# githubhjs/h264-jm-commentary

Measured on AMD Instinct MI355X. Metric: ME+transform megapixels/sec @1080p FullSearch SR=32; bit-exact vs the in-repo JM restatement (oracle); device-resident (inputs in HBM, no H2D/D2H in the timed region), higher is better.
Workload: dtype u8

## Files before the change

h264-jm-commentary_amd/csrc/jmh_analyse.hip:

```cpp
#include "jmh_common.h"
#include "jmh_launch.h"
#include "jmh_intra8.h"
#include "jmh_intra.h"
#include "jmh_i4.h"
#ifdef JMH_FLOW_TU
#include "jmh_final.h"
#endif

#define MVB_OFF 544
#define MVB_LEN 1104
#define PLS (WIN_DIM_MAX * WST + 32)
#define MAXNS 7

struct MeS {
    uint8_t org[256];
    Border bd;
    IntraNb<uint8_t> nb;
    int16_t all_mv[8][16][2];
    int motion_cost[8][4];
    unsigned red[NTA / 64][MAXNS];
    int pmv[MAXNS][2];
    uint16_t mvc[MVB_LEN];
    uint8_t planes[4 * PLS];
    union {
        int16_t h1[WIN_DIM_MAX * WST];
        uint2 sad8[NPK * NTA];
    } hs;
    unsigned long long *pst;
    int pn;
    alignas(8) IntraS<uint8_t> in;
};
union AnalyseS {
    MeS me;
    IntraS<uint8_t> in[4];
};

__device__ __forceinline__ void sstamp(MeS &s, int wave) {
    if (wave == 0 && __lane_id() == 0 && s.pst && s.pn < 44) s.pst[s.pn++] = wall_clock64();
}

struct NbMe {
    const MeS &s;
    int bt, b8, best8x8;
    __device__ bool operator()(int xN, int yN, int &ref, int &mx, int &my) const {
        if (yN > 15 || (xN > 15 && yN >= 0)) return false;
        if (xN < 0 || yN < 0) {
            int c = border_cell(xN, yN);
            if (c < 0 || s.bd.ref[c] == -2) return false;
            ref = s.bd.ref[c]; mx = s.bd.mv[c][0]; my = s.bd.mv[c][1];
            return true;
        }
        int k = (yN >> 2) * 4 + (xN >> 2), cb8 = ((yN >> 3) << 1) | (xN >> 3);
        int m = (bt <= 3 || cb8 == b8) ? bt : (best8x8 >> (4 * cb8)) & 15;
        ref = 0; mx = s.all_mv[m][k][0]; my = s.all_mv[m][k][1];
        return true;
    }
};

template <int BT, int BX, int BY>
__device__ __forceinline__ unsigned psum(const uint32_t (&r)[2]) {
    uint32_t v;
    if constexpr (BT == 1 || BT == 4) v = r[0] + r[1];
    else if constexpr (BT == 2) v = r[BY >> 1];
    else if constexpr (BT == 5) v = r[BY & 1];
    else if constexpr (BT == 3) { v = r[0] + r[1]; return (BX >> 1) ? v >> 16 : v & 0xFFFFu; }
    else if constexpr (BT == 6) { v = r[0] + r[1]; return (BX & 1) ? v >> 16 : v & 0xFFFFu; }
    else { v = r[BY & 1]; return (BX & 1) ? v >> 16 : v & 0xFFFFu; }
    return (v & 0xFFFFu) + (v >> 16);
}

struct PosState {
    uint32_t sadp[NPK][2];
    uint32_t ordk2[NPK2];
    int dx, dy0;
    int scx, scy;
};

__device__ __forceinline__ void fence_state(PosState &ps) {
#pragma unroll
    for (int k = 0; k < NPK; k++) {
#pragma unroll
        for (int q = 0; q < 2; q++) asm volatile("" : "+v"(ps.sadp[k][q]));
    }
#pragma unroll
    for (int k = 0; k < NPK2; k++) asm volatile("" : "+v"(ps.ordk2[k]));
    asm volatile("" : "+v"(ps.dx), "+v"(ps.dy0));
}

__device__ __forceinline__ uint32_t ordk_of(const PosState &ps, int k) {
    const uint32_t w = ps.ordk2[k >> 1];
    return (k & 1) ? (uint32_t)((int)w >> 16) : (uint32_t)(int)(int16_t)(w & 0xFFFFu);
}

template <int BT, int BX, int BY>
__device__ __forceinline__ unsigned eval_search(const MeS &s, const PosState &ps, const uint32_t (&sp)[NPK][2], int sr, int range, int pmx,
                                                int pmy, int scx, int scy) {
    const unsigned cxv = s.mvc[4 * (scx - sr + ps.dx) - pmx + MVB_OFF];
    const uint16_t *cy = s.mvc + 4 * (scy - sr + ps.dy0) - pmy + MVB_OFF;
    unsigned b = 0xFFFFFFFFu;
    if (range >= sr) {
#pragma unroll
        for (int k = 0; k < NPK; k++) {
            const unsigned cost = psum<BT, BX, BY>(sp[k]) + cxv + cy[4 * k];
            b = min(b, (cost << 13) | ordk_of(ps, k));
        }
    } else {
        const int rx = abs(ps.dx - sr);
#pragma unroll
        for (int k = 0; k < NPK; k++) {
            const unsigned cost = psum<BT, BX, BY>(sp[k]) + cxv + cy[4 * k];
            const uint32_t o = ordk_of(ps, k);
            const bool in = max(rx, abs(ps.dy0 + k - sr)) <= range || o == 0;
            b = min(b, in ? (cost << 13) | o : 0xFFFFFFFFu);
        }
    }
    return b;
}

__device__ __forceinline__ int search_range(const DevParams &d, int bt) { return d.restrict_sr == 0 ? d.sr / min(2, bt) : d.sr; }

struct SDesc {
    int bt, bx4, by4, mc;
    int fbt, fbx4, fby4, fslot;
};

__device__ __forceinline__ uint32_t lds_u32_at(const uint8_t *p) { return lds_u32_any(p); }
typedef short s16x2 __attribute__((ext_vector_type(2)));
__device__ __forceinline__ s16x2 as_s2(uint32_t v) { return __builtin_bit_cast(s16x2, v); }
__device__ __forceinline__ uint32_t as_u32(s16x2 v) { return __builtin_bit_cast(uint32_t, v); }
__device__ __forceinline__ s16x2 abs2(s16x2 v) { return __builtin_elementwise_max(v, (s16x2)(0) - v); }
__device__ __forceinline__ s16x2 lo16(uint32_t w) { return as_s2(__builtin_amdgcn_perm(0u, w, 0x0c010c00u)); }
__device__ __forceinline__ s16x2 hi16(uint32_t w) { return as_s2(__builtin_amdgcn_perm(0u, w, 0x0c030c02u)); }
__device__ __forceinline__ s16x2 tap6_2(s16x2 a, s16x2 b, s16x2 c, s16x2 d, s16x2 e, s16x2 f) {
    return (a + f) + (s16x2)(20) * (c + d) - (s16x2)(5) * (b + e);
}
__device__ __forceinline__ s16x2 clip5(s16x2 v) {
    return __builtin_elementwise_min(__builtin_elementwise_max((v + (s16x2)(16)) >> (s16x2)(5), (s16x2)(0)), (s16x2)(255));
}
__device__ __forceinline__ uint32_t pack4(s16x2 lo, s16x2 hi) { return __builtin_amdgcn_perm(as_u32(hi), as_u32(lo), 0x06040200u); }

template <bool HALF>
__device__ __forceinline__ int subblock_satd(const MeS &s, int wbase, int obase, int ox, int oy, int had) {
    const int off = qoff((oy & 3) * 4 + (ox & 3));
    const int xa = (off >> 12) & 15, ya = (off >> 8) & 15, xb = (off >> 4) & 15, yb = off & 15;
    const int oA = ((xa & 1) + 2 * (ya & 1)) * PLS + (ya >> 1) * WST + (xa >> 1);
    const int oB = ((xb & 1) + 2 * (yb & 1)) * PLS + (yb >> 1) * WST + (xb >> 1);
    const uint8_t *r0 = s.planes + wbase + (oy >> 2) * WST + (ox >> 2);
    uint32_t O[4], P[4];
#pragma unroll
    for (int yy = 0; yy < 4; yy++) {
        const uint32_t A = lds_u32_at(r0 + yy * WST + oA);
        if constexpr (HALF) P[yy] = A;
        else {
            const uint32_t B = lds_u32_at(r0 + yy * WST + oB);
            P[yy] = (A | B) - (((A ^ B) >> 1) & 0x7F7F7F7Fu);
        }
        O[yy] = *reinterpret_cast<const uint32_t *>(s.org + obase + 16 * yy);
    }
    if (!had) {
        uint32_t sad = 0;
#pragma unroll
        for (int yy = 0; yy < 4; yy++) sad = __builtin_amdgcn_sad_u8(O[yy], P[yy], sad);
        return (int)sad;
    }
    s16x2 r[4][2];
#pragma unroll
    for (int yy = 0; yy < 4; yy++) {
        r[yy][0] = as_s2(__builtin_amdgcn_perm(0u, O[yy], 0x0c010c00u)) - as_s2(__builtin_amdgcn_perm(0u, P[yy], 0x0c010c00u));
        r[yy][1] = as_s2(__builtin_amdgcn_perm(0u, O[yy], 0x0c030c02u)) - as_s2(__builtin_amdgcn_perm(0u, P[yy], 0x0c030c02u));
    }
    s16x2 m[4][2];
#pragma unroll
    for (int h = 0; h < 2; h++) {
        const s16x2 a0 = r[0][h] + r[3][h], a1 = r[1][h] + r[2][h], a2 = r[1][h] - r[2][h], a3 = r[0][h] - r[3][h];
        m[0][h] = a0 + a1; m[2][h] = a0 - a1; m[1][h] = a2 + a3; m[3][h] = a3 - a2;
    }
    s16x2 acc = (s16x2)(0);
#pragma unroll
    for (int p = 0; p < 2; p++) {
        const uint32_t u0 = as_u32(m[2 * p][0]), v0 = as_u32(m[2 * p + 1][0]);
        const uint32_t u1 = as_u32(m[2 * p][1]), v1 = as_u32(m[2 * p + 1][1]);
        const s16x2 x0 = as_s2(__builtin_amdgcn_perm(v0, u0, 0x05040100u)), x1 = as_s2(__builtin_amdgcn_perm(v0, u0, 0x07060302u));
        const s16x2 x2 = as_s2(__builtin_amdgcn_perm(v1, u1, 0x05040100u)), x3 = as_s2(__builtin_amdgcn_perm(v1, u1, 0x07060302u));
        const s16x2 a0 = x0 + x3, a1 = x1 + x2, a2 = x1 - x2, a3 = x0 - x3;
        acc += __builtin_elementwise_max(abs2(a0), abs2(a1)) + __builtin_elementwise_max(abs2(a2), abs2(a3));
    }
    const uint32_t t = as_u32(acc);
    return (int)((t & 0xFFFFu) + (t >> 16));
}

template <bool HALF>
__device__ __forceinline__ int quad_row_satd(const MeS &s, int wbase, int obase, int ox, int oy, int row, int had) {
    const int off = qoff((oy & 3) * 4 + (ox & 3));
    const int xa = (off >> 12) & 15, ya = (off >> 8) & 15, xb = (off >> 4) & 15, yb = off & 15;
    const int oA = ((xa & 1) + 2 * (ya & 1)) * PLS + (ya >> 1) * WST + (xa >> 1);
    const int oB = ((xb & 1) + 2 * (yb & 1)) * PLS + (yb >> 1) * WST + (xb >> 1);
    const uint8_t *rr = s.planes + wbase + (oy >> 2) * WST + (ox >> 2) + row * WST;
    const uint32_t A = lds_u32_at(rr + oA);
    uint32_t P = A;
    if constexpr (!HALF) {
        const uint32_t B = lds_u32_at(rr + oB);
        P = (A | B) - (((A ^ B) >> 1) & 0x7F7F7F7Fu);
    }
    const uint32_t O = *reinterpret_cast<const uint32_t *>(s.org + obase + 16 * row);
    if (!had) return (int)__builtin_amdgcn_sad_u8(O, P, 0u);
    s16x2 p0 = as_s2(__builtin_amdgcn_perm(0u, O, 0x0c010c00u)) - as_s2(__builtin_amdgcn_perm(0u, P, 0x0c010c00u));
    s16x2 p1 = as_s2(__builtin_amdgcn_perm(0u, O, 0x0c030c02u)) - as_s2(__builtin_amdgcn_perm(0u, P, 0x0c030c02u));
    {
        const s16x2 q0 = as_s2((uint32_t)dpp<0x1B>((int)as_u32(p0))), q1 = as_s2((uint32_t)dpp<0x1B>((int)as_u32(p1)));
        p0 = row < 2 ? p0 + q0 : q0 - p0;
        p1 = row < 2 ? p1 + q1 : q1 - p1;
    }
    {
        const s16x2 q0 = as_s2((uint32_t)dpp<0xB1>((int)as_u32(p0))), q1 = as_s2((uint32_t)dpp<0xB1>((int)as_u32(p1)));
        p0 = (row & 1) == 0 ? p0 + q0 : q0 - p0;
        p1 = (row & 1) == 0 ? p1 + q1 : q1 - p1;
    }
    const s16x2 sw = as_s2(__builtin_amdgcn_alignbit(as_u32(p1), as_u32(p1), 16));
    const uint32_t t = as_u32(abs2(p0 + sw)), u = as_u32(abs2(p0 - sw));
    return (int)(max(t & 0xFFFFu, t >> 16) + max(u & 0xFFFFu, u >> 16));
}

#define KOFF 4096
__device__ __forceinline__ void subpel_wave(const DevParams &d, MeS &s, int j, const SDesc q, int pmvx, int pmvy, int scx, int scy, int b8,
                                            int best8x8) {
    const int lane = __lane_id();
    const int sr = d.sr, lam = d.lambda_motion, had = d.use_hadamard;
    unsigned best = s.red[0][j];
#pragma unroll
    for (int w = 1; w < NTA / 64; w++) best = min(best, s.red[w][j]);
    const unsigned order = best & 8191u;
    int rx, ry;
    if (order == 0) { rx = -scx; ry = -scy; }
    else {
        const uint32_t e = d.ordtab[ORDTAB_SPOS + order - 1];
        rx = (int)(int16_t)(e & 0xFFFFu);
        ry = (int)e >> 16;
    }
    const int fmx = scx + rx, fmy = scy + ry;
    int min_mcost = had ? BIGCOST : (int)(best >> 13);
    const int lw4 = lw4_of(q.bt), lns = lw4 + lh4_of(q.bt), nsub = 1 << lns;
    const bool check0 = q.bt == 1 && fmx == 0 && fmy == 0 && had && d.slice_type == JMH_P_SLICE;
    const int wb0 = (WM + sr + ry) * WST + WM + sr + rx;
    int qx = 0, qy = 0;
#pragma unroll
    for (int pass = 0; pass < 2; pass++) {
        const int step = pass == 0 ? 2 : 1;
        const int min_pos = pass == 0 ? (had ? 0 : 1) : 1;
        unsigned kb = 0xFFFFFFFFu;
        if (lns <= 1) {
            const int row = lane & 3, c = lane >> 2;
            const bool val = c < 9 && c >= min_pos;
            const int ox = qx + step * sp9x(c), oy = qy + step * sp9y(c);
            int sat = 0;
            if (c < 9) {
                const int bxs1 = q.bx4 + lw4, bys1 = q.by4 + (lns - lw4);
                sat = pass == 0 ? quad_row_satd<true>(s, wb0 + 4 * q.by4 * WST + 4 * q.bx4, 64 * q.by4 + 4 * q.bx4, ox, oy, row, had)
                                : quad_row_satd<false>(s, wb0 + 4 * q.by4 * WST + 4 * q.bx4, 64 * q.by4 + 4 * q.bx4, ox, oy, row, had);
                if (lns)
                    sat += pass == 0 ? quad_row_satd<true>(s, wb0 + 4 * bys1 * WST + 4 * bxs1, 64 * bys1 + 4 * bxs1, ox, oy, row, had)
                                     : quad_row_satd<false>(s, wb0 + 4 * bys1 * WST + 4 * bxs1, 64 * bys1 + 4 * bxs1, ox, oy, row, had);
            }
            sat += dpp<0xB1>(sat);
            sat += dpp<0x4E>(sat);
            if (val && row == 0) {
                int cost = sat + (int)__umul24(lam, mvbits(4 * fmx + ox - pmvx) + mvbits(4 * fmy + oy - pmvy));
                if (pass == 0 && check0 && c == 0) cost -= 16 * lam;
                kb = min(kb, ((unsigned)(cost + KOFF) << 4) | (unsigned)c);
            }
        } else {
            const int g = lane & 3, c = lane >> 2, lspl = lns - 2;
            const bool val = c < 9 && c >= min_pos;
            const int ox = qx + step * sp9x(c), oy = qy + step * sp9y(c);
            int sat = 0;
            if (val) {
#pragma unroll
                for (int k = 0; k < 4; k++) {
                    if (k >= (1 << lspl)) break;
                    const int sub = (g << lspl) + k;
                    const int bxs = q.bx4 + (sub & ((1 << lw4) - 1)), bys = q.by4 + (sub >> lw4);
                    sat += pass == 0 ? subblock_satd<true>(s, wb0 + 4 * bys * WST + 4 * bxs, 64 * bys + 4 * bxs, ox, oy, had)
                                     : subblock_satd<false>(s, wb0 + 4 * bys * WST + 4 * bxs, 64 * bys + 4 * bxs, ox, oy, had);
                }
            }
            sat += dpp<0xB1>(sat);
            sat += dpp<0x4E>(sat);
            if (val && g == 0) {
                int cost = sat + (int)__umul24(lam, mvbits(4 * fmx + ox - pmvx) + mvbits(4 * fmy + oy - pmvy));
                if (pass == 0 && check0 && c == 0) cost -= 16 * lam;
                kb = min(kb, ((unsigned)(cost + KOFF) << 4) | (unsigned)c);
            }
        }
        kb = wave_min_u32(kb);
        if (kb != 0xFFFFFFFFu && (int)(kb >> 4) - KOFF < min_mcost) {
            const int c = kb & 15;
            min_mcost = (int)(kb >> 4) - KOFF;
            qx += step * sp9x(c);
            qy += step * sp9y(c);
        }
    }
    if (lane < nsub) {
        const int k = (q.by4 + (lane >> lw4)) * 4 + q.bx4 + (lane & ((1 << lw4) - 1));
        s.all_mv[q.bt][k][0] = (int16_t)(4 * fmx + qx);
        s.all_mv[q.bt][k][1] = (int16_t)(4 * fmy + qy);
    }
    if (lane == 0) s.motion_cost[q.bt][q.mc] += min_mcost;
    if (q.fbt) {
        int mx, my;
        set_mvp(NbMe{s, q.fbt, b8, best8x8}, q.fbx4, q.fby4, 4 << lw4_of(q.fbt), 4 << lh4_of(q.fbt), mx, my);
        if (lane == 0) { s.pmv[q.fslot][0] = mx; s.pmv[q.fslot][1] = my; }
    }
}

__device__ __forceinline__ constexpr int search_wave(int j) { return (0x6325410 >> (4 * j)) & 15; }

template <int NS, bool FWD, class EV, class IDLE>
__device__ __forceinline__ void me_stage(const DevParams &d, MeS &s, PosState &ps, const SDesc (&sd)[NS], int b8, int best8x8, EV ev,
                                         int islot, IDLE idle, int wave, int xdec = -1) {
    const int lane = __lane_id();
    fence_state(ps);
    int pmx[NS], pmy[NS];
    unsigned bk[NS];
    if constexpr (FWD) {
#pragma unroll
        for (int j = 0; j < NS; j++) {
            pmx[j] = __builtin_amdgcn_readfirstlane(s.pmv[j][0]);
            pmy[j] = __builtin_amdgcn_readfirstlane(s.pmv[j][1]);
        }
    } else {
#pragma unroll
        for (int j = 0; j < NS; j++)
            if (wave == search_wave(j)) {
                int mx, my;
                set_mvp(NbMe{s, sd[j].bt, b8, best8x8}, sd[j].bx4, sd[j].by4, 4 << lw4_of(sd[j].bt), 4 << lh4_of(sd[j].bt), mx, my);
                if (lane == 0) { s.pmv[j][0] = mx; s.pmv[j][1] = my; }
            }
        __syncthreads();
#pragma unroll
        for (int j = 0; j < NS; j++) {
            pmx[j] = __builtin_amdgcn_readfirstlane(s.pmv[j][0]);
            pmy[j] = __builtin_amdgcn_readfirstlane(s.pmv[j][1]);
        }
    }
    ev(bk, pmx, pmy);
#pragma unroll
    for (int j = 0; j < NS; j++) {
        const unsigned v = wave_min_u32(bk[j]);
        if (lane == 0) s.red[wave][j] = v;
    }
    __syncthreads();
    sstamp(s, wave);
#pragma unroll
    for (int j = 0; j < NS; j++)
        if (wave == search_wave(j)) subpel_wave(d, s, j, sd[j], pmx[j], pmy[j], ps.scx, ps.scy, b8, best8x8);
    if constexpr (NS <= 5) {
        if (xdec >= 0 && wave == 3) idle(11, xdec);
    }
    if constexpr (NS <= 6) {
        if (islot >= 0 && wave >= 6) idle(islot, wave - 6);
    } else {
        if (islot >= 0 && wave == 7) idle(islot, 0);
    }
    __syncthreads();
    sstamp(s, wave);
}

#define EV(J, BT, BX, BY) bk[J] = eval_search<BT, BX, BY>(s, ps, ps.sadp, sr, search_range(d, BT), pmx[J], pmy[J], ps.scx, ps.scy)

template <int N, int BT0, int BX0, int BY0, int BT1, int BX1, int BY1, int BT2 = 0, int BX2 = 0, int BY2 = 0>
__device__ __forceinline__ void eval_sad8(const MeS &s, const PosState &ps, int tid, int sr, const int (&range)[N], const int *pmx,
                                          const int *pmy, unsigned *out) {
    unsigned cxv[N];
    const uint16_t *cy[N];
    bool full = true;
#pragma unroll
    for (int j = 0; j < N; j++) {
        cxv[j] = s.mvc[4 * (ps.scx - sr + ps.dx) - pmx[j] + MVB_OFF];
        cy[j] = s.mvc + 4 * (ps.scy - sr + ps.dy0) - pmy[j] + MVB_OFF;
        out[j] = 0xFFFFFFFFu;
        full = full && range[j] >= sr;
    }
    auto loop = [&](auto restricted) {
        const int rx = abs(ps.dx - sr);
#pragma unroll
        for (int k = 0; k < NPK; k++) {
            const uint2 v = s.hs.sad8[k * NTA + tid];
            const uint32_t r[2] = {v.x, v.y};
            const uint32_t o = ordk_of(ps, k);
            unsigned c[3];
            c[0] = psum<BT0, BX0, BY0>(r);
            c[1] = psum<BT1, BX1, BY1>(r);
            if constexpr (N > 2) c[2] = psum<BT2, BX2, BY2>(r);
#pragma unroll
            for (int j = 0; j < N; j++) {
                const unsigned key = ((c[j] + cxv[j] + cy[j][4 * k]) << 13) | o;
                if constexpr (decltype(restricted)::value)
                    out[j] = min(out[j], (max(rx, abs(ps.dy0 + k - sr)) <= range[j] || o == 0) ? key : 0xFFFFFFFFu);
                else
                    out[j] = min(out[j], key);
            }
        }
    };
    if (full) loop(std::false_type{});
    else loop(std::true_type{});
}

template <bool EIGHT, int OX, int OY, int SLOT, int HI>
__device__ __forceinline__ void sad_strip(const MeS &s, PosState &ps) {
    const int wx = ps.dx + WM + OX;
    const uint32_t sel = wx & 3;
    const uint8_t *wb = s.planes + (ps.dy0 + WM + OY) * WST + (wx & ~3);
    uint32_t acc[NPK][2];
#pragma unroll
    for (int k = 0; k < NPK; k++) acc[k][0] = acc[k][1] = 0;
#pragma unroll
    for (int r = 0; r < 8 + NPK - 1; r++) {
        const uint32_t *w32 = reinterpret_cast<const uint32_t *>(wb + r * WST);
        const uint32_t a0 = w32[0], a1 = w32[1], a2 = w32[2];
        const uint32_t w0 = __builtin_amdgcn_alignbyte(a1, a0, sel), w1 = __builtin_amdgcn_alignbyte(a2, a1, sel);
#pragma unroll
        for (int k = 0; k < NPK; k++) {
            const int mr = r - k;
            if (mr < 0 || mr > 7) continue;
            const uint2 o = *reinterpret_cast<const uint2 *>(s.org + (OY + mr) * 16 + OX);
            if constexpr (EIGHT) {
                acc[k][0] = __builtin_amdgcn_sad_u8(w1, o.y, __builtin_amdgcn_sad_u8(w0, o.x, acc[k][0]));
                if (mr == 7) ps.sadp[k][SLOT] = HI ? (ps.sadp[k][SLOT] | (acc[k][0] << 16)) : acc[k][0];
            } else {
                acc[k][0] = __builtin_amdgcn_sad_u8(w0, o.x, acc[k][0]);
                acc[k][1] = __builtin_amdgcn_sad_u8(w1, o.y, acc[k][1]);
                if ((mr & 3) == 3) {
                    ps.sadp[k][mr >> 2] = acc[k][0] | (acc[k][1] << 16);
                    acc[k][0] = acc[k][1] = 0;
                }
            }
        }
    }
}

template <int B8, class IDLE>
__device__ __forceinline__ void p8x8_block(const DevParams &d, MeS &s, PosState &ps, int &best8x8, int &cost8x8, IDLE idle, int wave, int tid) {
    constexpr int X = 2 * (B8 & 1), Y = 2 * (B8 >> 1);
    constexpr int IS0 = 3 * B8 - (B8 == 3 ? 1 : 0), IS1 = IS0 + 1;
    constexpr int IS2 = B8 <= 1 ? 3 * B8 + 2 : B8 == 3 ? 10 : -1, IS3 = -1;
    constexpr int XD0 = B8 == 0 ? 1 : -1;
    const int sr = d.sr;
    fence_state(ps);
    sad_strip<false, 4 * X, 4 * Y, 0, 0>(s, ps);
#pragma unroll
    for (int k = 0; k < NPK; k++) {
        const uint32_t a = ps.sadp[k][0], b = ps.sadp[k][1];
        reinterpret_cast<uint16_t *>(&s.hs.sad8[k * NTA + tid])[B8] = (uint16_t)((a & 0xFFFFu) + (a >> 16) + (b & 0xFFFFu) + (b >> 16));
    }
    if constexpr (B8 == 3) {
        const SDesc sd[7] = {{4, X, Y, B8, 0, 0, 0, 0},
                             {5, X, Y, B8, 5, X, Y + 1, 0},
                             {6, X, Y, B8, 6, X + 1, Y, 1},
                             {7, X, Y, B8, 7, X + 1, Y, 2},
                             {1, 0, 0, 0, 0, 0, 0, 0},
                             {2, 0, 0, 0, 2, 0, 2, 3},
                             {3, 0, 0, 0, 3, 2, 0, 4}};
        me_stage<7, false>(d, s, ps, sd, B8, best8x8, [&](unsigned (&bk)[7], const int (&pmx)[7], const int (&pmy)[7]) {
            EV(0, 4, X, Y); EV(1, 5, X, Y); EV(2, 6, X, Y); EV(3, 7, X, Y);
            const int rg[3] = {search_range(d, 1), search_range(d, 2), search_range(d, 3)};
            eval_sad8<3, 1, 0, 0, 2, 0, 0, 3, 0, 0>(s, ps, tid, sr, rg, pmx + 4, pmy + 4, bk + 4);
        }, IS0, idle, wave);
        const SDesc sd1[5] = {{5, X, Y + 1, B8, 0, 0, 0, 0}, {6, X + 1, Y, B8, 0, 0, 0, 0}, {7, X + 1, Y, B8, 7, X, Y + 1, 0},
                              {2, 0, 2, 1, 0, 0, 0, 0}, {3, 2, 0, 1, 0, 0, 0, 0}};
        me_stage<5, true>(d, s, ps, sd1, B8, best8x8, [&](unsigned (&bk)[5], const int (&pmx)[5], const int (&pmy)[5]) {
            EV(0, 5, X, Y + 1); EV(1, 6, X + 1, Y); EV(2, 7, X + 1, Y);
            const int rg[2] = {search_range(d, 2), search_range(d, 3)};
            eval_sad8<2, 2, 0, 2, 3, 2, 0>(s, ps, tid, sr, rg, pmx + 3, pmy + 3, bk + 3);
        }, IS1, idle, wave, 0);
    } else {
        {
            const SDesc sd[4] = {{4, X, Y, B8, 0, 0, 0, 0},
                                 {5, X, Y, B8, 5, X, Y + 1, 0},
                                 {6, X, Y, B8, 6, X + 1, Y, 1},
                                 {7, X, Y, B8, 7, X + 1, Y, 2}};
            me_stage<4, false>(d, s, ps, sd, B8, best8x8, [&](unsigned (&bk)[4], const int (&pmx)[4], const int (&pmy)[4]) {
                EV(0, 4, X, Y); EV(1, 5, X, Y); EV(2, 6, X, Y); EV(3, 7, X, Y);
            }, IS0, idle, wave, XD0);
        }
        {
            const SDesc sd[3] = {{5, X, Y + 1, B8, 0, 0, 0, 0}, {6, X + 1, Y, B8, 0, 0, 0, 0}, {7, X + 1, Y, B8, 7, X, Y + 1, 0}};
            me_stage<3, true>(d, s, ps, sd, B8, best8x8, [&](unsigned (&bk)[3], const int (&pmx)[3], const int (&pmy)[3]) {
                EV(0, 5, X, Y + 1); EV(1, 6, X + 1, Y); EV(2, 7, X + 1, Y);
            }, IS1, idle, wave);
        }
    }
    {
        const SDesc sd[1] = {{7, X, Y + 1, B8, 7, X + 1, Y + 1, 0}};
        me_stage<1, true>(d, s, ps, sd, B8, best8x8, [&](unsigned (&bk)[1], const int (&pmx)[1], const int (&pmy)[1]) { EV(0, 7, X, Y + 1); },
                          IS2, idle, wave);
    }
    {
        const SDesc sd[1] = {{7, X + 1, Y + 1, B8, 0, 0, 0, 0}};
        me_stage<1, true>(d, s, ps, sd, B8, best8x8, [&](unsigned (&bk)[1], const int (&pmx)[1], const int (&pmy)[1]) { EV(0, 7, X + 1, Y + 1); },
                          IS3, idle, wave);
    }
    int mc8 = BIGCOST, bm = 0;
    for (int mode = 4; mode <= 7; mode++) {
        if (!inter_on(d.isr, mode)) continue;
        const int c = s.motion_cost[mode][B8];
        if (c < mc8) { mc8 = c; bm = mode; }
    }
    best8x8 = __builtin_amdgcn_readfirstlane(best8x8 | bm << (4 * B8));
    cost8x8 = __builtin_amdgcn_readfirstlane(cost8x8 + mc8);
}

template <class pel, class SC>
__device__ __forceinline__ void i16_decision(const DevParams &d, const pel *org, const IntraNb<pel> &nb, SC *scr, int lane, bool avL, bool avT,
                                             bool avTL) {
    int best, i16mode;
    i16_pick(d, org, nb, lane, avL, avT, avTL, best, i16mode);
    if (lane == 0) { scr->i16cost = best; scr->i16mode = i16mode; }
}

template <class pel, class SC>
__device__ __forceinline__ void chroma_decision(const DevParams &d, const IntraNb<pel> &nb, SC *scr, int lane, bool avL, bool avT, bool avTL) {
    int sat = 0;
    if (lane < 32) {
        const int m = lane >> 3, uv = (lane >> 2) & 1, b = lane & 3, xo = (b & 1) * 4, yo = (b >> 1) * 4;
        const pel *T = nb.ctop[uv] + 1, *L = nb.cleft[uv];
        const int Pc = nb.ctop[uv][0];
        const int dcv = chroma_dc(T, L, avT, avL, b, (d.maxv + 1) >> 1);
        int ih = 0, iv = 0;
#pragma unroll
        for (int i = 1; i <= 4; i++) {
            ih += i * (T[3 + i] - (3 - i >= 0 ? T[3 - i] : Pc));
            iv += i * (L[3 + i] - (3 - i >= 0 ? L[3 - i] : Pc));
        }
        const int ib = (34 * ih + 32) >> 6, ic = (34 * iv + 32) >> 6, iaa = 16 * (L[7] + T[7]);
        int df[16];
#pragma unroll
        for (int y = 0; y < 4; y++)
#pragma unroll
            for (int x = 0; x < 4; x++) {
                const int px = xo + x, py = yo + y;
                const int pl = clipmx((iaa + (px - 3) * ib + (py - 3) * ic + 16) >> 5, d.maxv);
                const int p = m == 0 ? dcv : m == 1 ? (int)L[py] : m == 2 ? (int)T[px] : pl;
                df[4 * y + x] = nb.orgc[uv][py * 8 + px] - p;
            }
        sat = satd4x4(df, d.use_hadamard);
    }
    int minc = BIGCOST, c_mode = 0;
#pragma unroll
    for (int m = 0; m < 4; m++) {
        int c = 0;
#pragma unroll
        for (int q = 0; q < 8; q++) c += __builtin_amdgcn_readlane(sat, 8 * m + q);
        if (chroma_mode_ok(m, avL, avT, avTL) && c < minc) { minc = c; c_mode = m; }
    }
    if (lane == 0) scr->c_mode = c_mode;
}

template <class SC>
__device__ __forceinline__ void intra_slot(const DevParams &d, IntraS<uint8_t> &s, SC *scr, int16_t (*i4lev)[16], int k, int w, int mbx, int mby);

__device__ __forceinline__ void me_prologue(const DevParams &d, MeS &s, int mbx, int mby) {
    const int tid = threadIdx.x;
    if (tid < 256) s.in.org[tid] = s.org[tid] = d.orgY[(16 * mby + (tid >> 4)) * d.W + 16 * mbx + (tid & 15)];
    else if (tid >= 472 && tid < 478) s.in.part[(tid - 472) / 3][(tid - 472) % 3] = 0;
    else if (tid >= 480 && tid < 512) s.motion_cost[(tid - 480) >> 2][tid & 3] = 0;
    for (int i = tid; i < MVB_LEN; i += NTA) s.mvc[i] = (uint16_t)__umul24(d.lambda_motion, mvbits(i - MVB_OFF));
}

template <class SC>
__device__ __forceinline__ void me_mb(const DevParams &d, MeS &s, SC *scr, int16_t (*i4lev)[16], int mbx, int mby, bool pre = false) {
    const int tid = threadIdx.x;
    const int wave = __builtin_amdgcn_readfirstlane(tid >> 6);
    const int W = d.W, sr = d.sr, side = d.side;
    const int pix_x = 16 * mbx, pix_y = 16 * mby;
    const bool prof = prof_mb_here(d, mbx, mby);
    PSTAMP(0);
    if (tid == 0) { s.pst = prof ? d.prof + 20 : nullptr; s.pn = 0; }
    if (tid < 256) { if (!pre) s.in.org[tid] = s.org[tid] = d.orgY[(pix_y + (tid >> 4)) * W + pix_x + (tid & 15)]; }
    else if (tid >= 384 && tid < 394) { load_border(d, s.bd, tid - 384, mbx, mby); load_border(d, s.in.bd, tid - 384, mbx, mby); }
    else if (!pre && tid >= 472 && tid < 478) s.in.part[(tid - 472) / 3][(tid - 472) % 3] = 0;
    else if (!pre && tid >= 480 && tid < 512) s.motion_cost[(tid - 480) >> 2][tid & 3] = 0;
    auto idle = [&](int k, int w) { intra_slot(d, s.in, scr, i4lev, k, w, mbx, mby); };
    if (!pre)
        for (int i = tid; i < MVB_LEN; i += NTA) s.mvc[i] = (uint16_t)__umul24(d.lambda_motion, mvbits(i - MVB_OFF));
    int pcx = 0, pcy = 0, scx = 0, scy = 0;
    uint8_t *G = s.planes;
    const int wdim = 2 * sr + 16 + 2 * WM;
    {
        __syncthreads();
        set_mvp(NbBorder{s.bd}, 0, 0, 16, 16, pcx, pcy);
        scx = iclip(-sr, sr, pcx / 4); scy = iclip(-sr, sr, pcy / 4);
        const int X0 = pix_x + scx - sr - WM, Y0 = pix_y + scy - sr - WM;
        constexpr int ND4 = WST / 4, NWT = (WIN_DIM_MAX * ND4 + NTA - 1) / NTA;
        uint32_t lo_[NWT], hi_[NWT];
        bool fast[NWT];
#pragma unroll
        for (int i = 0; i < NWT; i++) {
            const int task = tid + i * NTA;
            const int y = task / ND4, j = task - y * ND4, x0 = X0 + 4 * j;
            fast[i] = task < wdim * ND4 && 4 * j + 3 < wdim && x0 >= 0 && x0 + 3 < W;
            const uint32_t *p = reinterpret_cast<const uint32_t *>(d.refY + iclip(0, d.H - 1, Y0 + y) * W + (fast[i] ? (x0 & ~3) : 0));
            lo_[i] = p[0];
            hi_[i] = (fast[i] && (x0 & 3)) ? p[1] : 0u;
        }
#pragma unroll
        for (int i = 0; i < NWT; i++) {
            const int task = tid + i * NTA;
            if (task >= wdim * ND4) break;
            const int y = task / ND4, j = task - y * ND4, x0 = X0 + 4 * j;
            uint32_t v;
            if (fast[i]) v = __builtin_amdgcn_alignbyte(hi_[i], lo_[i], x0 & 3);
            else {
                const uint8_t *row = d.refY + iclip(0, d.H - 1, Y0 + y) * W;
                v = 0;
#pragma unroll
                for (int q = 0; q < 4; q++)
                    if (4 * j + q < wdim) v |= (uint32_t)row[iclip(0, W - 1, x0 + q)] << (8 * q);
            }
            *reinterpret_cast<uint32_t *>(G + y * WST + 4 * j) = v;
        }
        if (tid < 32) G[wdim * WST + tid] = 0;
        if (tid >= 128 && tid < 199) load_intra_nb(d, s.in.nb, tid - 128, mbx, mby);
    }
    __syncthreads();
    PSTAMP(1);
    {
        PosState ps;
        const int nstrips = (side + NPK - 1) / NPK;
        const bool sact = tid < side * nstrips;
        ps.dx = sact ? tid % side : 0;
        ps.dy0 = sact ? (tid / side) * NPK : 0;
        ps.scx = scx; ps.scy = scy;
        PSTAMP(8);
#pragma unroll
        for (int k2 = 0; k2 < NPK2; k2++) ps.ordk2[k2] = d.ordtab[k2 * NTA + tid];
        {
            const int k0 = sr - scy - ps.dy0;
            const bool mine = sact && ps.dx == sr - scx;
#pragma unroll
            for (int k2 = 0; k2 < NPK2; k2++)
                if (mine && (k0 >> 1) == k2) ps.ordk2[k2] &= (k0 & 1) ? 0x0000FFFFu : 0xFFFF0000u;
        }
        PSTAMP(9);
        {
            const int lo = WM - 1, n = 2 * sr + 18;
            uint8_t *PB = s.planes + PLS, *PH = s.planes + 2 * PLS, *PJ = s.planes + 3 * PLS;
            constexpr int NG = WIN_DIM_MAX / 4, NR = NTA / NG;
            const int g = tid % NG, rb = tid / NG, c0 = 4 * g;
            const int run = (n + NR - 1) / NR, y0 = lo + rb * run, y1 = rb < NR ? min(lo + n, y0 + run) : y0;
            if (y0 < y1) {
                const uint32_t *gc = reinterpret_cast<const uint32_t *>(G + c0);
                constexpr int WS4 = WST / 4;
                uint32_t w0 = gc[(y0 - 2) * WS4], w1 = gc[(y0 - 1) * WS4], w2 = gc[y0 * WS4], w3 = gc[(y0 + 1) * WS4], w4 = gc[(y0 + 2) * WS4];
                for (int y = y0; y < y1; y++) {
                    const uint32_t w5 = gc[(y + 3) * WS4];
                    const uint32_t L = gc[y * WS4 - 1], R = gc[y * WS4 + 1];
                    int hv[4];
                    uint32_t ph = 0, pb = 0;
#pragma unroll
                    for (int i = 0; i < 4; i++) {
                        const int sh = 8 * i;
                        hv[i] = tap6((int)((w0 >> sh) & 255u), (int)((w1 >> sh) & 255u), (int)((w2 >> sh) & 255u), (int)((w3 >> sh) & 255u),
                                     (int)((w4 >> sh) & 255u), (int)((w5 >> sh) & 255u));
                        ph |= (uint32_t)clip255((hv[i] + 16) >> 5) << sh;
                    }
                    const uint64_t mr = ((uint64_t)R << 32) | w2;
                    int bx[9];
                    bx[0] = (int)((L >> 16) & 255u); bx[1] = (int)(L >> 24);
#pragma unroll
                    for (int k = 0; k < 7; k++) bx[2 + k] = (int)((mr >> (8 * k)) & 255u);
#pragma unroll
                    for (int i = 0; i < 4; i++)
                        pb |= (uint32_t)clip255((tap6(bx[i], bx[i + 1], bx[i + 2], bx[i + 3], bx[i + 4], bx[i + 5]) + 16) >> 5) << (8 * i);
#pragma unroll
                    for (int i = 0; i < 4; i++) {
                        const int cx = c0 + i;
                        s.hs.h1[y * WST + cx] = (int16_t)hv[i];
                        { PH[y * WST + cx] = (uint8_t)(ph >> (8 * i)); PB[y * WST + cx] = (uint8_t)(pb >> (8 * i)); }
                    }
                    w0 = w1; w1 = w2; w2 = w3; w3 = w4; w4 = w5;
                }
            }
            __syncthreads();
            PSTAMP(10);
            for (int y = y0; y < y1; y++) {
                const uint32_t *hr = reinterpret_cast<const uint32_t *>(s.hs.h1 + y * WST + c0);
                const uint32_t q0 = hr[-1], q1 = hr[0], q2 = hr[1], q3 = hr[2], q4 = hr[3];
                const int x[9] = {(int)(int16_t)q0, (int)q0 >> 16, (int)(int16_t)q1, (int)q1 >> 16, (int)(int16_t)q2,
                                  (int)q2 >> 16, (int)(int16_t)q3, (int)q3 >> 16, (int)(int16_t)q4};
                uint32_t jv = 0;
#pragma unroll
                for (int i = 0; i < 4; i++)
                    jv |= (uint32_t)clip255((tap6(x[i], x[i + 1], x[i + 2], x[i + 3], x[i + 4], x[i + 5]) + 512) >> 10) << (8 * i);
#pragma unroll
                for (int i = 0; i < 4; i++)
                    PJ[y * WST + c0 + i] = (uint8_t)(jv >> (8 * i));
            }
        }
        __syncthreads();
        PSTAMP(2);
        {
            int best8x8 = 0, cost8x8 = 0;
            p8x8_block<0>(d, s, ps, best8x8, cost8x8, idle, wave, tid);
            PSTAMP(3);
            p8x8_block<1>(d, s, ps, best8x8, cost8x8, idle, wave, tid);
            PSTAMP(4);
            p8x8_block<2>(d, s, ps, best8x8, cost8x8, idle, wave, tid);
            PSTAMP(5);
            p8x8_block<3>(d, s, ps, best8x8, cost8x8, idle, wave, tid);
            if constexpr (scr_global<SC>) {
                if (tid < 224) {
                    const int m = 1 + tid / 32, k = (tid & 31) >> 1, c = tid & 1;
                    scr->all_mv[m][k][c] = s.all_mv[m][k][c];
                } else if (tid < 252) {
                    const int m = 1 + (tid - 224) / 4, k = tid & 3;
                    scr->motion_cost[m][k] = s.motion_cost[m][k];
                }
            }
            if (tid == 256) {
                scr->best8x8 = best8x8; scr->cost8x8 = cost8x8;
            } else if (tid == 320) {
                NbBorder nbv{s.bd};
                int ra = -1, ax = 0, ay = 0, rb = -1, bx = 0, by = 0;
                const bool aa = nbv(-1, 0, ra, ax, ay), ab = nbv(0, -1, rb, bx, by);
                const bool zl = !aa || (ra == 0 && ax == 0 && ay == 0), za = !ab || (rb == 0 && bx == 0 && by == 0);
                scr->skipx = (za || zl) ? 0 : pcx;
                scr->skipy = (za || zl) ? 0 : pcy;
            }
            PSTAMP(6);
        }
    }
}

template <class pel, class SC>
__device__ __forceinline__ void intra_role(const DevParams &d, IntraS<pel> &s, SC *scr, int16_t (*i4lev)[16], int mbx, int mby, int tid, bool act,
                                           bool i4) {
    const int wave = tid >> 6, lane = tid & 63;
    const int pix_x = 16 * mbx, pix_y = 16 * mby, W = d.W;
    const MbAvail mav = intra_avail(d, mbx, mby);
    const bool avL = mav.L, avT = mav.T, avTL = mav.TL, avTR = mav.TR;
    const bool prof = act && prof_mb_here(d, mbx, mby);
    PSTAMP(12);
    if (act) {
        const pel *orgY = spl<pel>(d.orgY);
        s.org[tid] = orgY[(pix_y + (tid >> 4)) * W + pix_x + (tid & 15)];
        s.org[tid + 128] = orgY[(pix_y + 8 + (tid >> 4)) * W + pix_x + (tid & 15)];
        load_orgc(d, s.nb, tid, mbx, mby);
        if (tid < 10) load_border(d, s.bd, tid, mbx, mby);
        else if (tid >= 16 && tid < 16 + 71) load_intra_nb(d, s.nb, tid - 16, mbx, mby);
    }
    const int q_bits = 15 + (d.qp + d.qpbd) / 6;
    const int qpk = q_round(d.qsel, q_bits);
    int tabr[2];
    i4_tabrow(lane, tabr);
    int acc[3] = {0, 0, 0};
    __syncthreads();
    for (int dg = 0; dg < 10; dg++) {
        const int by_lo = dg > 3 ? (dg - 2) >> 1 : 0;
        const int by4 = by_lo + wave, bx4 = dg - 2 * by4;
        if (act && i4 && by4 <= 3 && bx4 >= 0 && bx4 <= 3) i4_block(d, s, i4lev, wave, bx4, by4, tabr, avL, avT, avTL, avTR, qpk, acc);
        __syncthreads();
    }
    if (act && lane == 0) { s.part[wave][0] = acc[0]; s.part[wave][1] = acc[1]; s.part[wave][2] = acc[2]; }
    __syncthreads();
    if (!act) return;
    if (i4 && tid == 0) {
        scr->i4cost = 24 * d.lambda_mode + s.part[0][0] + s.part[1][0];
        scr->i4cbp = s.part[0][1] | s.part[1][1];
        scr->i4blk = s.part[0][2] | s.part[1][2];
    }
    if constexpr (scr_global<SC>) {
        if (i4 && tid < 16) scr->ipred[tid] = s.ipred_cur[tid];
        if (i4 && tid < (int)sizeof(s.rec) / 4) reinterpret_cast<uint32_t *>(scr->i4rec)[tid] = reinterpret_cast<const uint32_t *>(s.rec)[tid];
    }
    PSTAMP(13);
    if (wave == 0) i16_decision(d, s.org, s.nb, scr, lane, avL, avT, avTL);
    else chroma_decision(d, s.nb, scr, lane, avL, avT, avTL);
    PSTAMP(14);
}

template <class SC>
__device__ __forceinline__ void intra_slot(const DevParams &d, IntraS<uint8_t> &s, SC *scr, int16_t (*i4lev)[16], int k, int w, int mbx, int mby) {
    const int lane = threadIdx.x & 63;
    const MbAvail mav = intra_avail(d, mbx, mby);
    const bool avL = mav.L, avT = mav.T, avTL = mav.TL, avTR = mav.TR;
    if (k == 11) {
        if (d.i16c) {
            if (w == 0) i16_decision(d, s.org, s.nb, scr, lane, avL, avT, avTL);
            else chroma_decision(d, s.nb, scr, lane, avL, avT, avTL);
        }
    } else if (k < 10) {
        const int q_bits = 15 + d.qp / 6;
        const int qpk = q_round(d.qsel, q_bits);
        int tabr[2];
        i4_tabrow(lane, tabr);
        const int by_lo = k > 3 ? (k - 2) >> 1 : 0;
        const int by4 = by_lo + w, bx4 = k - 2 * by4;
        if (by4 <= 3 && bx4 >= 0 && bx4 <= 3) {
            int acc[3] = {s.part[w][0], s.part[w][1], s.part[w][2]};
            unsigned long long *pst = (k == 4 && w == 0 && d.prof && d.prof_mb == mby * d.mbw + mbx) ? d.prof : nullptr;
            i4_block(d, s, i4lev, w, bx4, by4, tabr, avL, avT, avTL, avTR, qpk, acc, pst);
            if (lane == 0) { s.part[w][0] = acc[0]; s.part[w][1] = acc[1]; s.part[w][2] = acc[2]; }
        }
    } else if (w == 0) {
        if (lane == 0) {
            scr->i4cost = 24 * d.lambda_mode + s.part[0][0] + s.part[1][0];
            scr->i4cbp = s.part[0][1] | s.part[1][1];
            scr->i4blk = s.part[0][2] | s.part[1][2];
        }
        if constexpr (scr_global<SC>) {
            if (lane < 16) scr->ipred[lane] = s.ipred_cur[lane];
            reinterpret_cast<uint32_t *>(scr->i4rec)[lane] = reinterpret_cast<const uint32_t *>(s.rec)[lane];
        }
    }
}

#ifndef JMH_FLOW_TU
__global__ __launch_bounds__(NTA, 4) void k_mb_analyse(const TickArgs t) {
    __shared__ AnalyseS s;
    const int nPm = t.me_in_analyse ? t.pre[t.nP] : 0, nPg = xcd_grid(nPm), tot = t.pre[t.npic], b = blockIdx.x;
    const unsigned long long t0 = t.bprof ? wall_clock64() : 0;
    const bool first_thread = threadIdx.x == 0;
    const int role = b < nPg ? 2 : 0;
    unsigned long long tag = role;
    if (role == 2) {
        const int m = xcd_block(b, nPm);
        if (m >= nPm) return;
        const int e = tick_entry(t, m);
        const DevParams d = tick_params(t, e);
        const int mby = d.y_min + (m - t.pre[e]), mbx = d.diag - 2 * mby;
        tag = 2u | (unsigned long long)(mby * d.mbw + mbx) << 4 | (unsigned long long)e << 32;
        MbScratch *scr = d.scr + mby * d.mbw + mbx;
        me_mb(d, s.me, scr, scr->i4lev, mbx, mby);
    } else {
        const int q = __builtin_amdgcn_readfirstlane(4 * (b - nPg) + (int)(threadIdx.x >> 7));
        const bool act = q < tot;
        const int e = tick_entry(t, act ? q : 0);
        const DevParams d = tick_params(t, e);
        const int mby = d.y_min + ((act ? q : t.pre[e]) - t.pre[e]), mbx = d.diag - 2 * mby;
        MbScratch *scr = d.scr + mby * d.mbw + mbx;
        intra_role(d, s.in[threadIdx.x >> 7], scr, scr->i4lev, mbx, mby, threadIdx.x & 127, act, q >= nPm);
    }
    if (t.bprof) {
        __syncthreads();
        if (first_thread) {
            t.bprof[3 * b] = t0;
            t.bprof[3 * b + 1] = wall_clock64();
            t.bprof[3 * b + 2] = tag;
        }
    }
}

#define JMH_INTRA_OCC 8
template <class pel>
__global__ __launch_bounds__(NT, JMH_INTRA_OCC) void k_mb_intra(const TickArgs t) {
    __shared__ union {
        IntraS<pel> in[2];
        I8S<pel> i8;
    } s;
    const int tot = t.pre[t.npic], nR = (tot + 1) / 2, nRg = xcd_grid(nR), b = blockIdx.x;
    if (b < nRg) {
        const int r = xcd_block(b, nR);
        if (r >= nR) return;
        const int q = __builtin_amdgcn_readfirstlane(2 * r + (int)(threadIdx.x >> 7));
        const bool act = q < tot;
        const int e = tick_entry(t, act ? q : 0);
        const DevParams d = tick_params(t, e);
        const int mby = d.y_min + ((act ? q : t.pre[e]) - t.pre[e]), mbx = d.diag - 2 * mby;
        MbScratch *scr = d.scr + mby * d.mbw + mbx;
        intra_role(d, s.in[threadIdx.x >> 7], scr, scr->i4lev, mbx, mby, threadIdx.x & 127, act, true);
    } else {
        const int mi = xcd_block(b - nRg, tot);
        if (mi >= tot) return;
        intra8_mb<pel>(t, s.i8, mi);
    }
}

hipError_t jmh_launch_intra(const TickArgs &t, hipStream_t st) {
    const int tot = t.pre[t.npic];
    const int nblocks = xcd_grid((tot + 1) / 2) + (t.t8 ? xcd_grid(tot) : 0);
    if (t.bd > 8) hipLaunchKernelGGL(k_mb_intra<uint16_t>, dim3(nblocks), dim3(NT), 0, st, t);
    else hipLaunchKernelGGL(k_mb_intra<uint8_t>, dim3(nblocks), dim3(NT), 0, st, t);
    return hipGetLastError();
}

hipError_t jmh_launch_analyse(const TickArgs &t, hipStream_t st) {
    const int nPm = t.me_in_analyse ? t.pre[t.nP] : 0;
    const int nblocks = xcd_grid(nPm) + (t.pre[t.npic] + 3) / 4;
    if (nblocks == 0) return hipSuccess;
    hipLaunchKernelGGL(k_mb_analyse, dim3(nblocks), dim3(NTA), 0, st, t);
    return hipGetLastError();
}
#endif

#ifdef JMH_FLOW_TU
__device__ __forceinline__ int own_sgpr(int v) {
    asm("" : "+s"(v));
    return v;
}

__device__ __forceinline__ DevParams flow_params(const FlowArgs &f, const PicParams &q) {
    DevParams d;
    const int W = own_sgpr(f.W), H = own_sgpr(f.H), sr = own_sgpr(f.sr);
    d.W = W; d.H = H; d.Wc = W >> 1; d.Hc = H >> 1; d.mbw = own_sgpr(f.mbw); d.mbh = own_sgpr(f.mbh);
    d.sr = sr; d.side = 2 * sr + 1; d.npos = d.side * d.side;
    d.search_mode = own_sgpr(f.search_mode); d.use_hadamard = own_sgpr(f.use_hadamard); d.restrict_sr = own_sgpr(f.restrict_sr);
    d.isr = f.isr;
    d.t8 = 0;
    d.epzs_dual = 0; d.epzs_subpel = 0; d.epzs_spts = 0; d.epzs_mints = 0; d.epzs_maxts = 0;
    d.slice_mbs = f.slice_mbs;
    d.maxv = 255; d.qpbd = 0;
    const int ls = W * H, lc = ls >> 2;
    d.orgY = q.org; d.orgU = q.org + ls; d.orgV = q.org + ls + lc;
    d.refY = q.ref; d.refU = q.ref + ls; d.refV = q.ref + ls + lc;
    d.recY = q.rec; d.recU = q.rec + ls; d.recV = q.rec + ls + lc;
    d.dbkY = q.dbk; d.dbkU = q.dbk ? q.dbk + ls : nullptr; d.dbkV = q.dbk ? q.dbk + ls + lc : nullptr;
    d.lf_disable = q.lf_disable; d.lf_offA = q.lf_offA; d.lf_offB = q.lf_offB;
    d.mv = q.mv; d.refidx = q.refidx; d.ipred = q.ipred; d.res = q.res;
    d.scr = nullptr;
    d.tmv = nullptr; d.tref = nullptr; d.ordtab = f.ordtab;
    d.prof = f.prof; d.prof_mb = f.prof_mb;
    d.slice_type = q.slice_type; d.qp = q.qp; d.lambda_motion = q.lambda_motion;
    d.lambda_mode = __builtin_amdgcn_readfirstlane(q.lambda_mode);
    d.cqp_off = q.cqp_off; d.qsel = q.qsel; d.diag = q.diag; d.y_min = q.y_min;
    d.rdo = 0; d.cavlc = 0;
    d.i16c = 1;
    d.cip = 0;
    d.lf = q.lambda_motion << 16;
    d.lambda_rd = 0;
    d.rp = nullptr;
    return d;
}

struct PlaneMC {
    uint32_t g;
    int ox, oy;
    __device__ __forceinline__ int at(int plane, int x, int y) const {
        return ((lds_cu8 *)(uintptr_t)(g + plane * PLS + y * WST + x))[0];
    }
    __device__ __forceinline__ int operator()(int X, int Y) const {
        const int x = (X >> 2) - ox, y = (Y >> 2) - oy, fx = X & 3, fy = Y & 3;
        if (fy == 0) {
            const int G = at(0, x, y);
            if (fx == 0) return G;
            const int b = at(1, x, y);
            return fx == 2 ? b : ((fx == 1 ? G : at(0, x + 1, y)) + b + 1) >> 1;
        }
        if (fx == 0) {
            const int h = at(2, x, y);
            return fy == 2 ? h : ((fy == 1 ? at(0, x, y) : at(0, x, y + 1)) + h + 1) >> 1;
        }
        if ((fx & 1) && (fy & 1)) return (at(1, x, fy == 1 ? y : y + 1) + at(2, fx == 1 ? x : x + 1, y) + 1) >> 1;
        const int j = at(3, x, y);
        if (fx == 2 && fy == 2) return j;
        const int o = fx == 2 ? at(1, x, fy == 1 ? y : y + 1) : at(2, fx == 1 ? x : x + 1, y);
        return (j + o + 1) >> 1;
    }
};

struct FlowAnalysis {
    const MeS &me;
    const IntraS<uint8_t> &in;
    const MbCarry &c;
    const int16_t (*lev)[16];
    __device__ __forceinline__ int motion_cost(int m, int k) const { return me.motion_cost[m][k]; }
    __device__ __forceinline__ int mv(int m, int k, int cc) const { return me.all_mv[m][k][cc]; }
    __device__ __forceinline__ int best8x8() const { return c.best8x8; }
    __device__ __forceinline__ int cost8x8() const { return c.cost8x8; }
    __device__ __forceinline__ int skipx() const { return c.skipx; }
    __device__ __forceinline__ int skipy() const { return c.skipy; }
    __device__ __forceinline__ int i4cost() const { return c.i4cost; }
    __device__ __forceinline__ int i4cbp() const { return c.i4cbp; }
    __device__ __forceinline__ int i4blk() const { return c.i4blk; }
    __device__ __forceinline__ int i4lev(int blk, int l) const { return lev[blk][l]; }
    __device__ __forceinline__ uint8_t i4rec(int i) const { return in.rec[i]; }
    __device__ __forceinline__ int ipred(int k) const { return in.ipred_cur[k]; }
    __device__ __forceinline__ int i16cost() const { return c.i16cost; }
    __device__ __forceinline__ int i16mode() const { return c.i16mode; }
    __device__ __forceinline__ int c_mode() const { return c.c_mode; }
    __device__ __forceinline__ int i8cost() const { return 0; }
    __device__ __forceinline__ int i8cbp() const { return 0; }
    __device__ __forceinline__ int i8modes() const { return 0; }
    __device__ __forceinline__ int i8lev(int, int) const { return 0; }
    __device__ __forceinline__ uint8_t i8rec(int) const { return 0; }
};

#define FLOW_SPIN_MAX (1 << 17)
__device__ __forceinline__ bool flow_done(const FlowArgs &f, int e, int mb, uint32_t gen) {
    return __hip_atomic_load(f.flags + (size_t)e * f.nmb + mb, __ATOMIC_RELAXED, __HIP_MEMORY_SCOPE_AGENT) >= gen;
}

__global__ __launch_bounds__(NTA, 4) void k_mb_flow(const FlowArgs f) {
    __shared__ struct {
        FinS<uint8_t> fin;
        AnalyseS a;
        MbCarry carry;
    } s;
    __shared__ int s_item;
    __shared__ unsigned s_tk;
    const int tid = threadIdx.x;
    const unsigned long long t0 = f.fprof ? wall_clock64() : 0;
    if (tid == 0) {
        const unsigned n = atomicAdd(f.head, 1u) - f.base;
        s_tk = n;
        int item = n < (unsigned)f.nitems ? (int)f.items[n] : -1;
        if (item < 0 || (item >> 24) >= f.nring || ((item >> 12) & 0xFFF) >= f.mbh || (item & 0xFFF) >= f.mbw) {
            __hip_atomic_store(f.err + 1, n, __ATOMIC_RELAXED, __HIP_MEMORY_SCOPE_SYSTEM);
            __hip_atomic_store(f.err + 2, (unsigned)item, __ATOMIC_RELAXED, __HIP_MEMORY_SCOPE_SYSTEM);
            __hip_atomic_store(f.err, 2u, __ATOMIC_RELAXED, __HIP_MEMORY_SCOPE_SYSTEM);
            item = -1;
        }
        s_item = item;
    }
    __syncthreads();
    const int item = __builtin_amdgcn_readfirstlane(s_item);
    if (item < 0) return;
    const int e = item >> 24, mby = (item >> 12) & 0xFFF, mbx = item & 0xFFF;
    const bool pslice = f.pics[e].pp.slice_type == JMH_P_SLICE;
    if (pslice) {
        const DevParams d = flow_params(f, f.pics[e].pp);
        me_prologue(d, s.a.me, mbx, mby);
        if (tid >= 256 && tid < 384) load_orgc(d, s.a.me.in.nb, tid - 256, mbx, mby);
    }
    if (tid == 0) {
        const FlowPic &P = f.pics[e];
        const uint32_t g = P.gen;
        const int mb = mby * f.mbw + mbx;
        const int re = pslice ? P.ref_entry : -1;
        const int rmb = min(mby + 5, f.mbh - 1) * f.mbw + min(mbx + 5, f.mbw - 1);
        const int tmb = mby > 0 ? (mbx + 1 < f.mbw ? mb - f.mbw + 1 : mb - f.mbw) : -1;
        int spin = 0;
        while (!((mbx == 0 || flow_done(f, e, mb - 1, g)) && (tmb < 0 || flow_done(f, e, tmb, g)) &&
                 (re < 0 || flow_done(f, re, rmb, P.ref_gen)))) {
            __builtin_amdgcn_s_sleep(2);
            if (++spin > FLOW_SPIN_MAX) { __hip_atomic_store(f.err, 1u, __ATOMIC_RELAXED, __HIP_MEMORY_SCOPE_SYSTEM); break; }
            if ((spin & 63) == 0 && __hip_atomic_load(f.err, __ATOMIC_RELAXED, __HIP_MEMORY_SCOPE_SYSTEM)) break;
        }
        __builtin_amdgcn_fence(__ATOMIC_ACQUIRE, "agent");
        asm volatile("s_waitcnt vmcnt(0)" ::: "memory");
    }
    __syncthreads();
#define FLOW_FP (f.fprof ? f.fprof + 6 * (size_t)__builtin_amdgcn_readfirstlane(s_tk) : nullptr)
    if (unsigned long long *fp = FLOW_FP; fp && tid == 0) {
        fp[0] = t0;
        fp[1] = wall_clock64();
        const unsigned hw = __builtin_amdgcn_s_getreg((4 << 0) | (0 << 6) | (15 << 11));
        const unsigned xcc = __builtin_amdgcn_s_getreg((20 << 0) | (0 << 6) | (3 << 11));
        fp[5] = (unsigned long long)(hw | xcc << 16) << 32 | (unsigned)item;
    }
    {
        const DevParams d = flow_params(f, f.pics[e].pp);
        if (pslice) me_mb(d, s.a.me, &s.carry, s.fin.lev, mbx, mby, true);
        else intra_role(d, s.a.in[tid >> 7], &s.carry, s.fin.lev, mbx, mby, tid & 127, tid < 128, true);
    }
    if (unsigned long long *fp = FLOW_FP; fp && tid == 0) fp[2] = wall_clock64();
    asm volatile("" ::: "memory");
    {
        const DevParams d = flow_params(f, f.pics[e].pp);
        const bool prof = prof_mb_here(d, mbx, mby);
        PSTAMP(56);
        __syncthreads();
        PSTAMP(58);
        int pcx = 0, pcy = 0;
        if (pslice) set_mvp(NbBorder{s.a.me.bd}, 0, 0, 16, 16, pcx, pcy);
        const int scx = iclip(-d.sr, d.sr, pcx / 4), scy = iclip(-d.sr, d.sr, pcy / 4);
        const PlaneMC mc{(uint32_t)(uintptr_t)(lds_cu8 *)s.a.me.planes, 16 * mbx + scx - d.sr - WM, 16 * mby + scy - d.sr - WM};
        IntraS<uint8_t> &in = pslice ? s.a.me.in : s.a.in[0];
        final_core<5, uint8_t, false, NTA>(d, s.fin, mbx, mby, tid, mc, FlowAnalysis{s.a.me, in, s.carry, s.fin.lev}, in.org, &in.nb);
    }
    asm volatile("s_waitcnt vmcnt(0)" ::: "memory");
    __syncthreads();
    if (tid == 0) {
        unsigned long long *fp = FLOW_FP;
        if (fp) fp[3] = wall_clock64();
        __builtin_amdgcn_fence(__ATOMIC_RELEASE, "agent");
        asm volatile("s_waitcnt vmcnt(0)" ::: "memory");
        __hip_atomic_store(f.flags + (size_t)e * f.nmb + mby * f.mbw + mbx, f.pics[e].gen, __ATOMIC_RELAXED, __HIP_MEMORY_SCOPE_AGENT);
        if (fp) fp[4] = wall_clock64();
    }
#undef FLOW_FP
}

hipError_t jmh_launch_flow(const FlowArgs &f, hipStream_t st) {
    if (f.nitems <= 0) return hipSuccess;
    hipLaunchKernelGGL(k_mb_flow, dim3(f.nitems), dim3(NTA), 0, st, f);
    return hipGetLastError();
}
#endif

#ifdef JMH_ISA_PROBE
__global__ __launch_bounds__(NTA, 4) void k_probe_subpel(const TickArgs t, int j) {
    __shared__ MeS s;
    const DevParams d = tick_params(t, 0);
    const SDesc q4 = {7, 1, 0, 0, 7, 0, 1, 0}, q8 = {4, 0, 0, 0, 0, 0, 0, 0};
    if (j) subpel_wave(d, s, 0, q4, t.W, t.H, 3, -2, 0, 0);
    else subpel_wave(d, s, 0, q8, t.W, t.H, 3, -2, 0, 0);
    __syncthreads();
    if (threadIdx.x < 64) d.mv[threadIdx.x] = s.all_mv[j ? 7 : 4][threadIdx.x & 15][threadIdx.x >> 4 & 1] + s.motion_cost[4][0] + s.pmv[0][0];
}
#endif
```

h264-jm-commentary_amd/csrc/jmh_common.h:

```cpp
#pragma once
#include "jmh_device.h"

#define MAX_VALUE 999999
#define WM 4
#define WIN_DIM_MAX (2 * SRMAX + 16 + 2 * WM)
#define WST 92

static __constant__ int c_q3[6][3] = {{13107, 5243, 8066}, {11916, 4660, 7490}, {10082, 4194, 6554},
                                      {9362, 3647, 5825},  {8192, 3355, 5243},  {7282, 2893, 4559}};
static __constant__ int c_dq3[6][3] = {{10, 16, 13}, {11, 18, 14}, {13, 20, 16}, {14, 23, 18}, {16, 25, 20}, {18, 29, 23}};
static __constant__ int c_qpc[52] = {0,  1,  2,  3,  4,  5,  6,  7,  8,  9,  10, 11, 12, 13, 14, 15, 16, 17,
                                     18, 19, 20, 21, 22, 23, 24, 25, 26, 27, 28, 29, 29, 30, 31, 32, 32, 33,
                                     34, 34, 35, 35, 36, 36, 37, 37, 37, 38, 38, 38, 39, 39, 39, 39};
static __constant__ int c_blc[8][2] = {{16, 16}, {16, 16}, {16, 8}, {8, 16}, {8, 8}, {8, 4}, {4, 8}, {4, 4}};
static __constant__ int c_sp9[9][2] = {{0, 0}, {0, -1}, {0, 1}, {-1, -1}, {1, -1}, {-1, 0}, {1, 0}, {-1, 1}, {1, 1}};
static __constant__ uint16_t c_qoff[16] = {
    0x0000, 0x0010, 0x1010, 0x2010,
    0x0001, 0x1001, 0x1011, 0x1021,
    0x0101, 0x0111, 0x1111, 0x1121,
    0x0201, 0x0112, 0x1112, 0x2112};
__device__ __forceinline__ int sp9x(int c) { return ((0x22215 >> (2 * c)) & 3) - 1; }
__device__ __forceinline__ int sp9y(int c) { return ((0x29421 >> (2 * c)) & 3) - 1; }
__device__ __forceinline__ int qoff(int ph) {
    const uint64_t q = ph < 8 ? (ph < 4 ? 0x2010101000100000ULL : 0x1021101110010001ULL)
                              : (ph < 12 ? 0x1121111101110101ULL : 0x2112111201120201ULL);
    return (int)((q >> (16 * (ph & 3))) & 0xFFFF);
}
__device__ __forceinline__ int lw4_of(int bt) { return bt <= 2 ? 2 : (bt <= 5 ? 1 : 0); }
__device__ __forceinline__ int lh4_of(int bt) { return (bt == 1 || bt == 3) ? 2 : (bt == 2 || bt == 4 || bt == 6) ? 1 : 0; }
#define SCAN_PACKED 0xFEB7ADC963258410ULL
__device__ __forceinline__ int scan_of(int k) { return (int)((SCAN_PACKED >> (4 * k)) & 15); }

__device__ __forceinline__ int iclip(int lo, int hi, int v) { return v < lo ? lo : (v > hi ? hi : v); }
__device__ __forceinline__ int clip255(int v) { return v < 0 ? 0 : (v > 255 ? 255 : v); }
__device__ __forceinline__ int clipmx(int v, int maxv) { return v < 0 ? 0 : (v > maxv ? maxv : v); }
__device__ __forceinline__ int isign(int a, int b) { return b < 0 ? -abs(a) : abs(a); }
__device__ __forceinline__ int mvbits(int v) { return v == 0 ? 1 : 2 * (31 - __clz(abs(v))) + 3; }
__device__ __forceinline__ int tap6(int a, int b, int c, int d, int e, int f) { return a - 5 * b + 20 * c + 20 * d - 5 * e + f; }
template <class T>
__device__ __forceinline__ int rpx(const T *p, int w, int h, int x, int y) { return p[iclip(0, h - 1, y) * w + iclip(0, w - 1, x)]; }
__device__ __forceinline__ int hb1(const uint8_t *p, int w, int h, int x, int y) {
    return tap6(rpx(p, w, h, x - 2, y), rpx(p, w, h, x - 1, y), rpx(p, w, h, x, y), rpx(p, w, h, x + 1, y), rpx(p, w, h, x + 2, y),
                rpx(p, w, h, x + 3, y));
}
__device__ __forceinline__ int vh1(const uint8_t *p, int w, int h, int x, int y) {
    return tap6(rpx(p, w, h, x, y - 2), rpx(p, w, h, x, y - 1), rpx(p, w, h, x, y), rpx(p, w, h, x, y + 1), rpx(p, w, h, x, y + 2),
                rpx(p, w, h, x, y + 3));
}
template <class PX, bool SERIAL_J = false>
__device__ __forceinline__ int qpel_from(PX px, int X, int Y, int maxv = 255) {
    const int x = X >> 2, y = Y >> 2, fx = X & 3, fy = Y & 3;
    auto hb1p = [&](int xx, int yy) { return tap6(px(xx - 2, yy), px(xx - 1, yy), px(xx, yy), px(xx + 1, yy), px(xx + 2, yy), px(xx + 3, yy)); };
    auto vh1p = [&](int xx, int yy) { return tap6(px(xx, yy - 2), px(xx, yy - 1), px(xx, yy), px(xx, yy + 1), px(xx, yy + 2), px(xx, yy + 3)); };
    auto hb = [&](int xx, int yy) { return iclip(0, maxv, (hb1p(xx, yy) + 16) >> 5); };
    auto vb = [&](int xx, int yy) { return iclip(0, maxv, (vh1p(xx, yy) + 16) >> 5); };
    if (fy == 0) {
        const int G = px(x, y);
        if (fx == 0) return G;
        const int b = hb(x, y);
        return fx == 2 ? b : ((fx == 1 ? G : px(x + 1, y)) + b + 1) >> 1;
    }
    if (fx == 0) {
        const int h = vb(x, y);
        return fy == 2 ? h : ((fy == 1 ? px(x, y) : px(x, y + 1)) + h + 1) >> 1;
    }
    if ((fx & 1) && (fy & 1)) return (hb(x, fy == 1 ? y : y + 1) + vb(fx == 1 ? x : x + 1, y) + 1) >> 1;
    int j1 = 0;
    if constexpr (SERIAL_J) {
#pragma unroll 1
        for (int k = 0; k < 6; k++) j1 += (k == 0 || k == 5 ? 1 : (k == 1 || k == 4 ? -5 : 20)) * vh1p(x - 2 + k, y);
    } else {
#pragma unroll
        for (int k = 0; k < 6; k++) j1 += (k == 0 || k == 5 ? 1 : (k == 1 || k == 4 ? -5 : 20)) * vh1p(x - 2 + k, y);
    }
    const int j = iclip(0, maxv, (j1 + 512) >> 10);
    if (fx == 2 && fy == 2) return j;
    const int o = fx == 2 ? hb(x, fy == 1 ? y : y + 1) : vb(fx == 1 ? x : x + 1, y);
    return (j + o + 1) >> 1;
}
template <class T, bool SERIAL_J = false>
__device__ __forceinline__ int qpel_direct(const T *ref, int W, int H, int X, int Y, int maxv = 255) {
    auto px = [&](int x, int y) { return rpx(ref, W, H, x, y); };
    return qpel_from<decltype(px), SERIAL_J>(px, X, Y, maxv);
}

__device__ __forceinline__ int spiral_index(int x, int y) {
    int ax = abs(x), ay = abs(y), l = max(ax, ay);
    if (l == 0) return 0;
    int base = (2 * l - 1) * (2 * l - 1);
    if (ay == l && ax < l) return base + 2 * (x + l - 1) + (y > 0);
    return base + 2 * (2 * l - 1) + 2 * (y + l) + (x > 0);
}
__device__ __forceinline__ void spiral_pos(int k, int &x, int &y) {
    if (k == 0) { x = y = 0; return; }
    int l = max(1, (int)((sqrtf((float)k) + 1.0f) * 0.5f));
    if ((2 * l + 1) * (2 * l + 1) <= k) l++;
    if ((2 * l - 1) * (2 * l - 1) > k) l--;
    int o = k - (2 * l - 1) * (2 * l - 1);
    if (o < 2 * (2 * l - 1)) { x = (o >> 1) - l + 1; y = (o & 1) ? l : -l; }
    else { o -= 2 * (2 * l - 1); y = (o >> 1) - l; x = (o & 1) ? l : -l; }
}
__device__ __forceinline__ int coeff_cost_run(int run) { return run == 0 ? 3 : run <= 2 ? 2 : run <= 5 ? 1 : 0; }

typedef __attribute__((address_space(3))) const uint32_t lds_cu32;
typedef __attribute__((address_space(3))) const uint8_t lds_cu8;
__device__ __forceinline__ uint32_t lds_u32_any(const void *p) {
    const uint32_t a = (uint32_t)(uintptr_t)(lds_cu8 *)p;
    lds_cu32 *q = (lds_cu32 *)(uintptr_t)(a & ~3u);
    return __builtin_amdgcn_alignbyte(q[1], q[0], a & 3);
}

template <int CTRL>
__device__ __forceinline__ int dpp(int v) {
    return __builtin_amdgcn_update_dpp(0, v, CTRL, 0xF, 0xF, true);
}
template <int CTRL>
__device__ __forceinline__ unsigned dpp_umin(unsigned v) {
    return min(v, (unsigned)__builtin_amdgcn_update_dpp(-1, (int)v, CTRL, 0xF, 0xF, false));
}
__device__ __forceinline__ int row16_sum(int v) {
    v += dpp<0xB1>(v);
    v += dpp<0x4E>(v);
    v += dpp<0x141>(v);
    v += dpp<0x140>(v);
    return v;
}
__device__ __forceinline__ int row16_had(int v, int l) {
    int p = dpp<0xB1>(v);
    v = (l & 1) ? p - v : v + p;
    p = dpp<0x4E>(v);
    v = (l & 2) ? p - v : v + p;
    p = dpp<0x1B>(dpp<0x141>(v));
    v = (l & 4) ? p - v : v + p;
    p = dpp<0x128>(v);
    v = (l & 8) ? p - v : v + p;
    return v;
}
__device__ __forceinline__ unsigned wave_min_u32(unsigned v) {
    v = dpp_umin<0xB1>(v);
    v = dpp_umin<0x4E>(v);
    v = dpp_umin<0x141>(v);
    v = dpp_umin<0x140>(v);
    unsigned a = __builtin_amdgcn_readlane(v, 0), b = __builtin_amdgcn_readlane(v, 16);
    unsigned c = __builtin_amdgcn_readlane(v, 32), e = __builtin_amdgcn_readlane(v, 48);
    return min(min(a, b), min(c, e));
}
__device__ __forceinline__ void wave_lds_sync() {
    __builtin_amdgcn_fence(__ATOMIC_RELEASE, "wavefront");
    __builtin_amdgcn_wave_barrier();
    __builtin_amdgcn_fence(__ATOMIC_ACQUIRE, "wavefront");
}

__device__ __forceinline__ int g16(int v, int src) { return __shfl(v, (int)(threadIdx.x & 48) + src, 64); }

__device__ __forceinline__ int fwd_tap(int p0, int p1, int p2, int p3, int k) {
    const int a = (k & 1) ? p3 : p0, b = (k & 1) ? p2 : p1;
    const int ca = k == 1 ? 2 : 1, cb = k < 2 ? 1 : k == 2 ? -1 : -2;
    return ca * a + cb * b;
}
__device__ __forceinline__ int inv_tap(int e0, int e1, int e2, int e3, int k) {
    const bool outer = k == 0 || k == 3;
    const int a = outer ? e0 : e1, b = outer ? e3 : e2;
    return k < 2 ? a + b : a - b;
}
__device__ __forceinline__ int lane_fwd4x4(int r, int l) {
    int y = l >> 2, x = l & 3;
    int v0 = g16(r, 4 * y), v1 = g16(r, 4 * y + 1), v2 = g16(r, 4 * y + 2), v3 = g16(r, 4 * y + 3);
    int p0 = v0 + v3, p3 = v0 - v3, p1 = v1 + v2, p2 = v1 - v2;
    const int t = fwd_tap(p0, p1, p2, p3, x);
    const int u0 = g16(t, x), u1 = g16(t, 4 + x), u2 = g16(t, 8 + x), u3 = g16(t, 12 + x);
    return fwd_tap(u0 + u3, u1 + u2, u1 - u2, u0 - u3, y);
}
__device__ __forceinline__ int lane_inv4x4(int dq, int l, int pred, int maxv = 255) {
    int y = l >> 2, x = l & 3;
    int d0 = g16(dq, 4 * y), d1 = g16(dq, 4 * y + 1), d2 = g16(dq, 4 * y + 2), d3 = g16(dq, 4 * y + 3);
    int e0 = d0 + d2, e1 = d0 - d2, e2 = (d1 >> 1) - d3, e3 = d1 + (d3 >> 1);
    const int t = inv_tap(e0, e1, e2, e3, x);
    const int f0 = g16(t, x), f1 = g16(t, 4 + x), f2 = g16(t, 8 + x), f3 = g16(t, 12 + x);
    const int o = inv_tap(f0 + f2, f0 - f2, (f1 >> 1) - f3, f1 + (f3 >> 1), y);
    return iclip(0, maxv, (o + (pred << 6) + 32) >> 6);
}
__device__ __forceinline__ int q_round(int sel, int q_bits) {
    return sel >= 2 ? (sel - 2) << (q_bits - 11) : sel ? (1 << q_bits) / 3 : (1 << q_bits) / 6;
}
__device__ __forceinline__ int q_sel16(int sel) { return sel >= 2 ? sel : 1; }
__device__ __forceinline__ unsigned lane_quant(int c, int l, int qp, int qp_const, bool ac_only, int &lev_scan, int &dq, int &cost) {
    const int qp_per = qp / 6, qp_rem = qp % 6, q_bits = 15 + qp_per;
    const int x = l & 3, y = l >> 2;
    const int cls = ((x | y) & 1) == 0 ? 0 : ((x & y) & 1) ? 1 : 2;
    const int q0 = __builtin_amdgcn_readfirstlane(c_q3[qp_rem][0]), q1 = __builtin_amdgcn_readfirstlane(c_q3[qp_rem][1]);
    const int q2 = __builtin_amdgcn_readfirstlane(c_q3[qp_rem][2]);
    const int d0 = __builtin_amdgcn_readfirstlane(c_dq3[qp_rem][0]), d1 = __builtin_amdgcn_readfirstlane(c_dq3[qp_rem][1]);
    const int d2 = __builtin_amdgcn_readfirstlane(c_dq3[qp_rem][2]);
    const int qc = cls == 0 ? q0 : cls == 1 ? q1 : q2;
    const int dqc = cls == 0 ? d0 : cls == 1 ? d1 : d2;
    int level = (abs(c) * qc + qp_const) >> q_bits;
    if (ac_only && l == 0) level = 0;
    const int dqm = level * dqc << qp_per;
    dq = c < 0 ? -dqm : dqm;
    const int sr = scan_of(l);
    const int lvs = g16(level, sr), cs = g16(c, sr);
    const unsigned long long bal = __ballot(lvs != 0);
    const unsigned m = (unsigned)(bal >> (threadIdx.x & 48)) & 0xFFFFu;
    int k = 0;
    if (lvs) {
        unsigned below = m & ((1u << l) - 1u);
        int prev = below ? 31 - __clz(below) : (ac_only ? 0 : -1);
        k = lvs > 1 ? MAX_VALUE : coeff_cost_run(l - prev - 1);
    }
    cost = row16_sum(k);
    lev_scan = lvs ? isign(lvs, cs) : 0;
    return m;
}

__device__ __forceinline__ int satd4x4(const int d[16], int had) {
    int s = 0;
    if (!had) {
#pragma unroll
        for (int k = 0; k < 16; k++) s += abs(d[k]);
        return s;
    }
    int m[16];
#pragma unroll
    for (int x = 0; x < 4; x++) {
        int a0 = d[x] + d[12 + x], a1 = d[4 + x] + d[8 + x], a2 = d[4 + x] - d[8 + x], a3 = d[x] - d[12 + x];
        m[x] = a0 + a1; m[8 + x] = a0 - a1; m[4 + x] = a2 + a3; m[12 + x] = a3 - a2;
    }
#pragma unroll
    for (int y = 0; y < 4; y++) {
        int *r = m + 4 * y;
        int a0 = r[0] + r[3], a1 = r[1] + r[2], a2 = r[1] - r[2], a3 = r[0] - r[3];
        s += abs(a0 + a1) + abs(a0 - a1) + abs(a2 + a3) + abs(a3 - a2);
    }
    return s >> 1;
}
__device__ __forceinline__ int lane_had_abs(int dv, int l) { return row16_sum(abs(row16_had(dv, l))); }
__device__ __forceinline__ int lane_satd(int dv, int l, int had) {
    return had ? lane_had_abs(dv, l) >> 1 : row16_sum(abs(dv));
}

template <class NB>
__device__ __forceinline__ void set_mvp(const NB &nb, int bx4, int by4, int bsx, int bsy, int &px, int &py) {
    int mb_x = 4 * bx4, mb_y = 4 * by4;
    int ra = -1, rb = -1, rc = -1, rd = -1, ax = 0, ay = 0, bxv = 0, byv = 0, cx = 0, cy = 0, dx = 0, dy = 0;
    bool av_a = nb(mb_x - 1, mb_y, ra, ax, ay);
    bool av_b = nb(mb_x, mb_y - 1, rb, bxv, byv);
    bool av_c = nb(mb_x + bsx, mb_y - 1, rc, cx, cy);
    bool av_d = nb(mb_x - 1, mb_y - 1, rd, dx, dy);
    if (mb_y > 0) {
        if (mb_x < 8) {
            if (mb_y == 8) { if (bsx == 16) av_c = false; }
            else if (mb_x + bsx == 8) av_c = false;
        } else if (mb_x + bsx == 16) av_c = false;
    }
    if (!av_c) { av_c = av_d; rc = rd; cx = dx; cy = dy; }
    int rL = av_a ? ra : -1, rU = av_b ? rb : -1, rUR = av_c ? rc : -1;
    int type = 0;
    if (rL == 0 && rU != 0 && rUR != 0) type = 1;
    else if (rL != 0 && rU == 0 && rUR != 0) type = 2;
    else if (rL != 0 && rU != 0 && rUR == 0) type = 3;
    if (bsx == 8 && bsy == 16) { if (mb_x == 0) { if (rL == 0) type = 1; } else if (rUR == 0) type = 3; }
    else if (bsx == 16 && bsy == 8) { if (mb_y == 0) { if (rU == 0) type = 2; } else if (rL == 0) type = 1; }
    int A[2] = {av_a ? ax : 0, av_a ? ay : 0}, B[2] = {av_b ? bxv : 0, av_b ? byv : 0}, C[2] = {av_c ? cx : 0, av_c ? cy : 0};
    int p[2];
#pragma unroll
    for (int hv = 0; hv < 2; hv++) {
        int a = A[hv], b = B[hv], c = C[hv];
        if (type == 1) p[hv] = a;
        else if (type == 2) p[hv] = b;
        else if (type == 3) p[hv] = c;
        else if (!(av_b || av_c)) p[hv] = a;
        else p[hv] = a + b + c - min(a, min(b, c)) - max(a, max(b, c));
    }
    px = p[0]; py = p[1];
}

template <class NB>
__device__ __forceinline__ bool mvp_nbr(const NB &nb, int bx4, int by4, int bsx, int k, int &ref, int &mx, int &my) {
    const int mb_x = 4 * bx4, mb_y = 4 * by4;
    if (k == 0) return nb(mb_x - 1, mb_y, ref, mx, my);
    if (k == 1) return nb(mb_x, mb_y - 1, ref, mx, my);
    bool av_c = nb(mb_x + bsx, mb_y - 1, ref, mx, my);
    if (mb_y > 0) {
        if (mb_x < 8) {
            if (mb_y == 8) { if (bsx == 16) av_c = false; }
            else if (mb_x + bsx == 8) av_c = false;
        } else if (mb_x + bsx == 16) av_c = false;
    }
    if (!av_c) av_c = nb(mb_x - 1, mb_y - 1, ref, mx, my);
    return av_c;
}

struct Border {
    int16_t mv[10][2];
    int8_t ref[10];
    int8_t ipm[10];
};
__device__ __forceinline__ int border_cell(int xN, int yN) {
    if (yN < 0) { int b = xN >> 2; return b > 4 ? -1 : b + 1; }
    if (xN < 0) return yN > 15 ? -1 : 6 + (yN >> 2);
    return -1;
}
__device__ __forceinline__ void load_border(const DevParams &d, Border &b, int t, int mbx, int mby) {
    const int W4 = d.W >> 2;
    int by4 = t < 6 ? -1 : t - 6, bx4 = t < 6 ? t - 1 : -1;
    const MbAvail m = mb_avail(d, mbx, mby);
    bool av = by4 < 0 ? (bx4 < 0 ? m.TL : bx4 > 3 ? m.TR : m.T) : m.L;
    int ref = -2, mx = 0, my = 0, ipm = -1;
    if (av) {
        int a = (4 * mby + by4) * W4 + 4 * mbx + bx4;
        ref = d.refidx[a]; mx = d.mv[2 * a]; my = d.mv[2 * a + 1]; ipm = d.ipred[a];
        if (d.cip && ref >= 0) ipm = -1;
    }
    b.ref[t] = (int8_t)ref; b.mv[t][0] = (int16_t)mx; b.mv[t][1] = (int16_t)my; b.ipm[t] = (int8_t)ipm;
}
struct NbBorder {
    const Border &b;
    __device__ __forceinline__ bool operator()(int xN, int yN, int &ref, int &mx, int &my) const {
        if (yN > 15 || (xN > 15 && yN >= 0)) return false;
        int c = border_cell(xN, yN);
        if (c < 0 || b.ref[c] == -2) return false;
        ref = b.ref[c]; mx = b.mv[c][0]; my = b.mv[c][1];
        return true;
    }
};

__device__ __forceinline__ int i4_pred_px(const int *P, int up, int left, int m, int x, int y) {
#define PT(i) P[1 + (i)]
#define PL(j) ((j) < 0 ? P[0] : P[9 + (j)])
    switch (m) {
    case 0: return PT(x);
    case 1: return PL(y);
    case 2:
        if (up && left) return (PT(0) + PT(1) + PT(2) + PT(3) + PL(0) + PL(1) + PL(2) + PL(3) + 4) >> 3;
        if (left) return (PL(0) + PL(1) + PL(2) + PL(3) + 2) >> 2;
        if (up) return (PT(0) + PT(1) + PT(2) + PT(3) + 2) >> 2;
        return 128;
    case 3: return (x == 3 && y == 3) ? (PT(6) + 3 * PT(7) + 2) >> 2 : (PT(x + y) + 2 * PT(x + y + 1) + PT(x + y + 2) + 2) >> 2;
    case 4:
        if (x > y) return (PT(x - y - 2) + 2 * PT(x - y - 1) + PT(x - y) + 2) >> 2;
        if (x < y) return (PL(y - x - 2) + 2 * PL(y - x - 1) + PL(y - x) + 2) >> 2;
        return (PT(0) + 2 * P[0] + PL(0) + 2) >> 2;
    case 5: {
        int z = 2 * x - y;
        if (z >= 0 && !(z & 1)) return (PT(x - (y >> 1) - 1) + PT(x - (y >> 1)) + 1) >> 1;
        if (z >= 0) return (PT(x - (y >> 1) - 2) + 2 * PT(x - (y >> 1) - 1) + PT(x - (y >> 1)) + 2) >> 2;
        if (z == -1) return (PL(0) + 2 * P[0] + PT(0) + 2) >> 2;
        return (PL(y - 1) + 2 * PL(y - 2) + PL(y - 3) + 2) >> 2;
    }
    case 6: {
        int z = 2 * y - x;
        if (z >= 0 && !(z & 1)) return (PL(y - (x >> 1) - 1) + PL(y - (x >> 1)) + 1) >> 1;
        if (z >= 0) return (PL(y - (x >> 1) - 2) + 2 * PL(y - (x >> 1) - 1) + PL(y - (x >> 1)) + 2) >> 2;
        if (z == -1) return (PL(0) + 2 * P[0] + PT(0) + 2) >> 2;
        return (PT(x - 1) + 2 * PT(x - 2) + PT(x - 3) + 2) >> 2;
    }
    case 7:
        return (y & 1) ? (PT(x + (y >> 1)) + 2 * PT(x + (y >> 1) + 1) + PT(x + (y >> 1) + 2) + 2) >> 2
                       : (PT(x + (y >> 1)) + PT(x + (y >> 1) + 1) + 1) >> 1;
    default: {
        int z = x + 2 * y;
        if (z > 5) return PL(3);
        if (z == 5) return (PL(2) + 3 * PL(3) + 2) >> 2;
        if (!(z & 1)) return (PL(y + (x >> 1)) + PL(y + (x >> 1) + 1) + 1) >> 1;
        return (PL(y + (x >> 1)) + 2 * PL(y + (x >> 1) + 1) + PL(y + (x >> 1) + 2) + 2) >> 2;
    }
    }
#undef PT
#undef PL
}

template <class pel>
__device__ __forceinline__ int chroma_dc(const pel *T, const pel *L, int up, int left, int b, int dcd) {
    int s0 = 0, s1 = 0, s2 = 0, s3 = 0;
    for (int i = 0; i < 4; i++) { s0 += T[i]; s1 += T[4 + i]; s2 += L[i]; s3 += L[4 + i]; }
    if (b == 0) return (up && left) ? (s0 + s2 + 4) >> 3 : up ? (s0 + 2) >> 2 : left ? (s2 + 2) >> 2 : dcd;
    if (b == 1) return up ? (s1 + 2) >> 2 : left ? (s2 + 2) >> 2 : dcd;
    if (b == 2) return left ? (s3 + 2) >> 2 : up ? (s0 + 2) >> 2 : dcd;
    return (up && left) ? (s1 + s3 + 4) >> 3 : up ? (s1 + 2) >> 2 : left ? (s3 + 2) >> 2 : dcd;
}
template <class pel>
__device__ __forceinline__ int chroma_pred_px(const pel *T, const pel *L, int Pc, int up, int left, int m, int x, int y, int maxv = 255) {
    if (m == 0) return chroma_dc(T, L, up, left, (y >> 2) * 2 + (x >> 2), (maxv + 1) >> 1);
    if (m == 1) return L[y];
    if (m == 2) return T[x];
    int ih = 0, iv = 0;
    for (int i = 1; i <= 4; i++) {
        ih += i * (T[3 + i] - (3 - i >= 0 ? T[3 - i] : Pc));
        iv += i * (L[3 + i] - (3 - i >= 0 ? L[3 - i] : Pc));
    }
    int ib = (34 * ih + 32) >> 6, ic = (34 * iv + 32) >> 6, iaa = 16 * (L[7] + T[7]);
    return clipmx((iaa + (x - 3) * ib + (y - 3) * ic + 16) >> 5, maxv);
}
struct I16Par { int dcv, ib, ic, iaa; };
template <class pel>
__device__ __forceinline__ I16Par i16_params(const pel *T, const pel *L, int up, int left, int dcd = 128) {
    int st = 0, sl = 0, ih = 0, iv = 0;
    for (int i = 0; i < 16; i++) { st += T[i]; sl += L[i]; }
    for (int i = 1; i <= 8; i++) {
        ih += i * (T[7 + i] - T[7 - i]);
        iv += i * (L[7 + i] - (7 - i >= 0 ? L[7 - i] : T[-1]));
    }
    I16Par p;
    p.dcv = (up && left) ? (st + sl + 16) >> 5 : up ? (st + 8) >> 4 : left ? (sl + 8) >> 4 : dcd;
    p.ib = (5 * ih + 32) >> 6; p.ic = (5 * iv + 32) >> 6; p.iaa = 16 * (L[15] + T[15]);
    return p;
}
template <class pel>
__device__ __forceinline__ int i16_pred(const I16Par &p, const pel *T, const pel *L, int m, int x, int y, int maxv = 255) {
    if (m == 0) return T[x];
    if (m == 1) return L[y];
    if (m == 2) return p.dcv;
    return clipmx((p.iaa + (x - 7) * p.ib + (y - 7) * p.ic + 16) >> 5, maxv);
}

__device__ __forceinline__ int class8(int x, int y) {
    if (!(x & 3) && !(y & 3)) return 0;
    if ((x & 1) && (y & 1)) return 1;
    if ((x & 3) == 2 && (y & 3) == 2) return 2;
    if ((!(x & 3) && (y & 1)) || ((x & 1) && !(y & 3))) return 3;
    if ((!(x & 3) && (y & 3) == 2) || ((x & 3) == 2 && !(y & 3))) return 4;
    return 5;
}
static __constant__ int c_q8[6][6] = {{13107, 11428, 20972, 12222, 16777, 15481}, {11916, 10826, 19174, 11058, 14980, 14290},
                                      {10082, 8943, 15978, 9675, 12710, 11985},   {9362, 8228, 14913, 8931, 11984, 11259},
                                      {8192, 7346, 13159, 7740, 10486, 9777},     {7282, 6428, 11570, 6830, 9118, 8640}};
static __constant__ int c_dq8[6][6] = {{20, 18, 32, 19, 25, 24}, {22, 19, 35, 21, 28, 26}, {26, 23, 42, 24, 33, 31},
                                       {28, 25, 45, 26, 35, 33}, {32, 28, 51, 30, 40, 38}, {36, 32, 58, 34, 46, 43}};
static __constant__ uint8_t c_scan8[64] = {0,  1,  8,  16, 9,  2,  3,  10, 17, 24, 32, 25, 18, 11, 4,  5,
                                           12, 19, 26, 33, 40, 48, 41, 34, 27, 20, 13, 6,  7,  14, 21, 28,
                                           35, 42, 49, 56, 57, 50, 43, 36, 29, 22, 15, 23, 30, 37, 44, 51,
                                           58, 59, 52, 45, 38, 31, 39, 46, 53, 60, 61, 54, 47, 55, 62, 63};
__device__ __forceinline__ int scan8_of(int l) {
    const int g = l >> 3;
    const uint64_t q = g < 4 ? (g < 2 ? (g == 0 ? 0x0a03020910080100ull : 0x05040b1219201811ull) : (g == 2 ? 0x22293028211a130cull : 0x1c150e07060d141bull))
                             : (g < 6 ? (g == 4 ? 0x242b323938312a23ull : 0x332c251e170f161dull) : (g == 6 ? 0x2e271f262d343b3aull : 0x3f3e372f363d3c35ull));
    return (int)((q >> (8 * (l & 7))) & 63);
}
__device__ __forceinline__ int pick6(const int *row, int cls) {
    const int a0 = __builtin_amdgcn_readfirstlane(row[0]), a1 = __builtin_amdgcn_readfirstlane(row[1]);
    const int a2 = __builtin_amdgcn_readfirstlane(row[2]), a3 = __builtin_amdgcn_readfirstlane(row[3]);
    const int a4 = __builtin_amdgcn_readfirstlane(row[4]), a5 = __builtin_amdgcn_readfirstlane(row[5]);
    return cls < 3 ? (cls == 0 ? a0 : cls == 1 ? a1 : a2) : (cls == 3 ? a3 : cls == 4 ? a4 : a5);
}
__device__ __forceinline__ int coeff_cost8_run(int run) { return run < 4 ? 3 : run < 12 ? 2 : run < 24 ? 1 : 0; }

__device__ __forceinline__ int wave_sum(int v) {
    v = row16_sum(v);
    return __builtin_amdgcn_readlane(v, 0) + __builtin_amdgcn_readlane(v, 16) + __builtin_amdgcn_readlane(v, 32) +
           __builtin_amdgcn_readlane(v, 48);
}
__device__ __forceinline__ int w64(int v, int src) { return __shfl(v, src, 64); }

__device__ __forceinline__ int fwd8_pick(int x0, int x1, int x2, int x3, int x4, int x5, int x6, int x7, int k) {
    const int a0 = x0 + x7, a1 = x1 + x6, a2 = x2 + x5, a3 = x3 + x4;
    const int b0 = a0 + a3, b1 = a1 + a2, b2 = a0 - a3, b3 = a1 - a2;
    const int a4 = x0 - x7, a5 = x1 - x6, a6 = x2 - x5, a7 = x3 - x4;
    const int b4 = a5 + a6 + ((a4 >> 1) + a4), b5 = a4 - a7 - ((a6 >> 1) + a6);
    const int b6 = a4 + a7 - ((a5 >> 1) + a5), b7 = a5 - a6 + ((a7 >> 1) + a7);
    switch (k) {
    case 0: return b0 + b1;
    case 1: return b4 + (b7 >> 2);
    case 2: return b2 + (b3 >> 1);
    case 3: return b5 + (b6 >> 2);
    case 4: return b0 - b1;
    case 5: return b6 - (b5 >> 2);
    case 6: return (b2 >> 1) - b3;
    default: return (b4 >> 2) - b7;
    }
}
__device__ __forceinline__ int inv8_pick(int d0, int d1, int d2, int d3, int d4, int d5, int d6, int d7, int k) {
    const int a0 = d0 + d4, a4 = d0 - d4, a2 = (d2 >> 1) - d6, a6 = d2 + (d6 >> 1);
    const int b0 = a0 + a6, b2 = a4 + a2, b4 = a4 - a2, b6 = a0 - a6;
    const int a1 = -d3 + d5 - d7 - (d7 >> 1), a3 = d1 + d7 - d3 - (d3 >> 1);
    const int a5 = -d1 + d7 + d5 + (d5 >> 1), a7 = d3 + d5 + d1 + (d1 >> 1);
    const int b1 = a1 + (a7 >> 2), b7 = a7 - (a1 >> 2), b3 = a3 + (a5 >> 2), b5 = (a3 >> 2) - a5;
    switch (k) {
    case 0: return b0 + b7;
    case 1: return b2 + b5;
    case 2: return b4 + b3;
    case 3: return b6 + b1;
    case 4: return b6 - b1;
    case 5: return b4 - b3;
    case 6: return b2 - b5;
    default: return b0 - b7;
    }
}
__device__ __forceinline__ int wave_fwd8x8(int r, int l) {
    const int x = l & 7, y = l >> 3, rb = 8 * y;
    const int t = fwd8_pick(w64(r, rb), w64(r, rb + 1), w64(r, rb + 2), w64(r, rb + 3), w64(r, rb + 4), w64(r, rb + 5),
                            w64(r, rb + 6), w64(r, rb + 7), x);
    return fwd8_pick(w64(t, x), w64(t, 8 + x), w64(t, 16 + x), w64(t, 24 + x), w64(t, 32 + x), w64(t, 40 + x), w64(t, 48 + x),
                     w64(t, 56 + x), y);
}
__device__ __forceinline__ int wave_inv8x8(int dq, int l, int pred, int maxv = 255) {
    const int x = l & 7, y = l >> 3, rb = 8 * y;
    const int t = inv8_pick(w64(dq, rb), w64(dq, rb + 1), w64(dq, rb + 2), w64(dq, rb + 3), w64(dq, rb + 4), w64(dq, rb + 5),
                            w64(dq, rb + 6), w64(dq, rb + 7), x);
    const int o = inv8_pick(w64(t, x), w64(t, 8 + x), w64(t, 16 + x), w64(t, 24 + x), w64(t, 32 + x), w64(t, 40 + x), w64(t, 48 + x),
                            w64(t, 56 + x), y);
    return iclip(0, maxv, (o + (pred << 6) + 32) >> 6);
}
__device__ __forceinline__ unsigned long long wave_quant8(int c, int l, int qp, int qp_const, int &lev_scan, int &dq, int &cost) {
    const int qp_per = qp / 6, qp_rem = qp % 6, q_bits = 16 + qp_per;
    const int cls = class8(l & 7, l >> 3);
    const int level = (abs(c) * pick6(c_q8[qp_rem], cls) + qp_const) >> q_bits;
    const int sl = c < 0 ? -level : level;
    const int ls = 16 * pick6(c_dq8[qp_rem], cls);
    dq = !level ? 0 : qp >= 36 ? sl * ls * (1 << (qp_per - 6)) : (sl * ls + (1 << (5 - qp_per))) >> (6 - qp_per);
    const int lvs = w64(sl, scan8_of(l));
    const unsigned long long m = __ballot(lvs != 0);
    int k = 0;
    if (lvs) {
        const unsigned long long below = m & ((1ull << l) - 1ull);
        const int prev = below ? 63 - __clzll(below) : -1;
        k = abs(lvs) > 1 ? MAX_VALUE : coeff_cost8_run(l - prev - 1);
    }
    cost = wave_sum(k);
    lev_scan = lvs;
    return m;
}
__device__ __forceinline__ int wave_had_abs(int v, int l, bool quad4) {
#pragma unroll
    for (int h = 1; h < 64; h <<= 1) {
        if (quad4 && (h == 4 || h == 32)) continue;
        const int p = __shfl_xor(v, h, 64);
        v = (l & h) ? p - v : v + p;
    }
    return wave_sum(abs(v));
}
__device__ __forceinline__ int wave_satd8(int dv, int l, int had) { return had ? (wave_had_abs(dv, l, false) + 2) >> 2 : wave_sum(abs(dv)); }
__device__ __forceinline__ int wave_satd4x4s(int dv, int l, int had) { return had ? wave_had_abs(dv, l, true) >> 1 : wave_sum(abs(dv)); }
__device__ __forceinline__ int il_blk(int b8, int k) { const int j = k & 3; return (2 * (b8 >> 1) + (j >> 1)) * 4 + 2 * (b8 & 1) + (j & 1); }

__device__ __forceinline__ int i8_pred_px(const int *f, int dcv, int m, int x, int y) {
#define TAP(c) ((f[(c) - 1] + 2 * f[c] + f[(c) + 1] + 2) >> 2)
    int z;
    switch (m) {
    case 0: return f[9 + x];
    case 1: return f[7 - y];
    case 2: return dcv;
    case 3: return x + y < 14 ? TAP(10 + x + y) : (f[23] + 3 * f[24] + 2) >> 2;
    case 4: return TAP(8 + x - y);
    case 5:
        z = 2 * x - y;
        if (z >= 0 && !(z & 1)) return (f[8 + x - (y >> 1)] + f[9 + x - (y >> 1)] + 1) >> 1;
        return z > 0 ? TAP(8 + x - (y >> 1)) : TAP(9 + z);
    case 6:
        z = 2 * y - x;
        if (z >= 0 && !(z & 1)) return (f[8 - y + (x >> 1)] + f[7 - y + (x >> 1)] + 1) >> 1;
        return z > 0 ? TAP(8 - y + (x >> 1)) : TAP(7 - z);
    case 7:
        return (y & 1) ? (f[9 + x + (y >> 1)] + 2 * f[10 + x + (y >> 1)] + f[11 + x + (y >> 1)] + 2) >> 2
                       : (f[9 + x + (y >> 1)] + f[10 + x + (y >> 1)] + 1) >> 1;
    default:
        z = x + 2 * y;
        if (z > 13) return f[0];
        if (z == 13) return (f[1] + 3 * f[0] + 2) >> 2;
        if (!(z & 1)) return (f[7 - y - (x >> 1)] + f[6 - y - (x >> 1)] + 1) >> 1;
        return (f[7 - y - (x >> 1)] + 2 * f[6 - y - (x >> 1)] + f[5 - y - (x >> 1)] + 2) >> 2;
    }
#undef TAP
}

__device__ __forceinline__ bool prof_mb_here(const DevParams &d, int mbx, int mby, int w = 0) {
    return d.prof && threadIdx.x == 64 * w && d.prof_mb == mby * d.mbw + mbx;
}
#define PSTAMP(k) do { if (prof) d.prof[k] = wall_clock64(); } while (0)
```

h264-jm-commentary_amd/csrc/jmh_deblock.h:

```cpp
#pragma once
#include "jmh_common.h"
#include <cstdlib>

static __constant__ uint8_t c_alpha[52] = {0,  0,  0,  0,  0,  0,  0,  0,  0,  0,  0,  0,  0,   0,   0,   0,   4,   4,
                                           5,  6,  7,  8,  9,  10, 12, 13, 15, 17, 20, 22, 25,  28,  32,  36,  40,  45,
                                           50, 56, 63, 71, 80, 90, 101, 113, 127, 144, 162, 182, 203, 226, 255, 255};
static __constant__ uint8_t c_beta[52] = {0,  0,  0,  0,  0,  0,  0,  0,  0,  0,  0,  0,  0,  0,  0,  0,  2,  2,
                                          2,  3,  3,  3,  3,  4,  4,  4,  6,  6,  7,  7,  8,  8,  9,  9,  10, 10,
                                          11, 11, 12, 12, 13, 13, 14, 14, 15, 15, 16, 16, 17, 17, 18, 18};
static __constant__ uint8_t c_tc0[52][3] = {
    {0, 0, 0}, {0, 0, 0}, {0, 0, 0}, {0, 0, 0}, {0, 0, 0}, {0, 0, 0}, {0, 0, 0}, {0, 0, 0}, {0, 0, 0},
    {0, 0, 0}, {0, 0, 0}, {0, 0, 0}, {0, 0, 0}, {0, 0, 0}, {0, 0, 0}, {0, 0, 0}, {0, 0, 0}, {0, 0, 1},
    {0, 0, 1}, {0, 0, 1}, {0, 0, 1}, {0, 1, 1}, {0, 1, 1}, {1, 1, 1}, {1, 1, 1}, {1, 1, 1}, {1, 1, 1},
    {1, 1, 2}, {1, 1, 2}, {1, 1, 2}, {1, 1, 2}, {1, 2, 3}, {1, 2, 3}, {2, 2, 3}, {2, 2, 4}, {2, 3, 4},
    {2, 3, 4}, {3, 3, 5}, {3, 4, 6}, {3, 4, 6}, {4, 5, 7}, {4, 5, 8}, {4, 6, 9}, {5, 7, 10}, {6, 8, 11},
    {6, 8, 13}, {7, 10, 14}, {8, 11, 16}, {9, 12, 18}, {10, 13, 20}, {11, 15, 23}, {13, 17, 25}};

template <class pel>
__device__ __forceinline__ void filter_line(pel *q, int step, int bS, int alpha, int beta, int tc0, bool chroma, int maxv) {
    const int p0 = q[-step], p1 = q[-2 * step], q0 = q[0], q1 = q[step];
    if (!(abs(p0 - q0) < alpha && abs(p1 - p0) < beta && abs(q1 - q0) < beta)) return;
    if (chroma) {
        if (bS < 4) {
            const int tc = tc0 + 1;
            const int dl = iclip(-tc, tc, ((q0 - p0) * 4 + (p1 - q1) + 4) >> 3);
            q[-step] = (pel)clipmx(p0 + dl, maxv);
            q[0] = (pel)clipmx(q0 - dl, maxv);
        } else {
            q[-step] = (pel)((2 * p1 + p0 + q1 + 2) >> 2);
            q[0] = (pel)((2 * q1 + q0 + p1 + 2) >> 2);
        }
        return;
    }
    const int p2 = q[-3 * step], q2 = q[2 * step];
    const int ap = abs(p2 - p0), aq = abs(q2 - q0);
    if (bS < 4) {
        const int tc = tc0 + (ap < beta) + (aq < beta);
        const int dl = iclip(-tc, tc, ((q0 - p0) * 4 + (p1 - q1) + 4) >> 3);
        q[-step] = (pel)clipmx(p0 + dl, maxv);
        q[0] = (pel)clipmx(q0 - dl, maxv);
        if (ap < beta) q[-2 * step] = (pel)(p1 + iclip(-tc0, tc0, (p2 + ((p0 + q0 + 1) >> 1) - (p1 << 1)) >> 1));
        if (aq < beta) q[step] = (pel)(q1 + iclip(-tc0, tc0, (q2 + ((p0 + q0 + 1) >> 1) - (q1 << 1)) >> 1));
    } else {
        const int p3 = q[-4 * step], q3 = q[3 * step];
        const bool small = abs(p0 - q0) < ((alpha >> 2) + 2);
        if (ap < beta && small) {
            q[-step] = (pel)((p2 + 2 * p1 + 2 * p0 + 2 * q0 + q1 + 4) >> 3);
            q[-2 * step] = (pel)((p2 + p1 + p0 + q0 + 2) >> 2);
            q[-3 * step] = (pel)((2 * p3 + 3 * p2 + p1 + p0 + q0 + 4) >> 3);
        } else q[-step] = (pel)((2 * p1 + p0 + q1 + 2) >> 2);
        if (aq < beta && small) {
            q[0] = (pel)((p1 + 2 * p0 + 2 * q0 + 2 * q1 + q2 + 4) >> 3);
            q[step] = (pel)((p0 + q0 + q1 + q2 + 2) >> 2);
            q[2 * step] = (pel)((2 * q3 + 3 * q2 + q1 + q0 + p0 + 4) >> 3);
        } else q[0] = (pel)((2 * q1 + q0 + p1 + 2) >> 2);
    }
}



template <class pel>
struct DbkS {
    pel dy[20][20];
    pel dc2[2][12][12];
    int8_t bs[2][4][4];
    int16_t nmv[2][4][2];
    int32_t nbits[2];
    int8_t nintra[2];
};

template <class pel, int NTH>
__device__ __forceinline__ void deblock_prefetch(const DevParams &d, DbkS<pel> &s, int mbx, int mby, int tid) {
    const pel *dbkY = spl<pel>(d.dbkY), *dbkU = spl<pel>(d.dbkU), *dbkV = spl<pel>(d.dbkV);
    const int pix_x = 16 * mbx, pix_y = 16 * mby, W = d.W, Wc = d.Wc;
    const bool dbL = mbx > 0, dbT = mby > 0;
    for (int i = tid; i < 256 + 16; i += NTH) {
        if (i < 128) {
            const bool top = i < 64;
            const int a = i & 63, r = top ? (a >> 4) - 4 : a >> 2, c = top ? a & 15 : (a & 3) - 4;
            s.dy[r + 4][c + 4] = (top ? dbT : dbL) ? dbkY[(pix_y + r) * W + pix_x + c] : (pel)0;
        } else if (i < 256) {
            const int j = i - 128, pl = j >> 6, a = j & 63;
            const bool top = a < 32;
            const int b = a & 31, r = top ? (b >> 3) - 4 : b >> 2, c = top ? b & 7 : (b & 3) - 4;
            s.dc2[pl][r + 4][c + 4] = (top ? dbT : dbL) ? (pl ? dbkV : dbkU)[((pix_y >> 1) + r) * Wc + (pix_x >> 1) + c] : (pel)0;
        } else {
            const int j = i - 256, dir = j >> 3, k = j & 7;
            const bool av = dir == 0 ? dbL : dbT;
            if (av) {
                const jmh_mb_result *rp = d.res + (dir == 0 ? mby * d.mbw + mbx - 1 : (mby - 1) * d.mbw + mbx);
                if (k < 4) {
                    const int bp = dir == 0 ? k * 4 + 3 : 12 + k;
                    s.nmv[dir][k][0] = rp->mv[bp][0];
                    s.nmv[dir][k][1] = rp->mv[bp][1];
                } else if (k == 4) {
                    s.nbits[dir] = rp->cbp_blk;
                } else if (k == 5) {
                    const int t = rp->mb_type;
                    s.nintra[dir] = t == JMH_I4MB || t == JMH_I16MB || t == JMH_I8MB;
                }
            }
        }
    }
}

template <class pel, int NTH = NT, bool PRE = false>
__device__ __forceinline__ void deblock_mb(const DevParams &d, DbkS<pel> &s, const pel *rec, const pel (*cfin)[64], const int16_t (*fmv)[2],
                                           bool is_intra, int cbp_blk, bool t8flag, int qpy, int qpcy, int mbx, int mby, int tid) {
    pel *dbkY = spl<pel>(d.dbkY), *dbkU = spl<pel>(d.dbkU), *dbkV = spl<pel>(d.dbkV);
    const int pix_x = 16 * mbx, pix_y = 16 * mby, W = d.W, Wc = d.Wc, maxv = d.maxv;
    const bool dbL = mbx > 0, dbT = mby > 0;
    {
        const bool filt = d.lf_disable != 1;
        __syncthreads();
        for (int i = tid; i < 400 + 288; i += NTH) {
            if (i < 400) {
                const int r = i / 20 - 4, c = i % 20 - 4;
                int v = 0;
                if (r >= 0 && c >= 0) v = rec[16 * r + c];
                else if ((r < 0) != (c < 0)) {
                    if (PRE) continue;
                    if ((r < 0 && dbT) || (c < 0 && dbL)) v = dbkY[(pix_y + r) * W + pix_x + c];
                }
                s.dy[r + 4][c + 4] = (pel)v;
            } else {
                const int j = i - 400, pl = j / 144, r = (j % 144) / 12 - 4, c = j % 12 - 4;
                int v = 0;
                if (r >= 0 && c >= 0) v = cfin[pl][8 * r + c];
                else if ((r < 0) != (c < 0)) {
                    if (PRE) continue;
                    if ((r < 0 && dbT) || (c < 0 && dbL)) v = (pl ? dbkV : dbkU)[((pix_y >> 1) + r) * Wc + (pix_x >> 1) + c];
                }
                s.dc2[pl][r + 4][c + 4] = (pel)v;
            }
        }
        if (tid < 32) {
            const int dir = tid >> 4, e = (tid >> 2) & 3, i = tid & 3;
            const bool mb_edge = e == 0;
            int bS = 0;
            if (filt && !(mb_edge && (dir == 0 ? !dbL : !dbT))) {
                const int bq = dir == 0 ? i * 4 + e : e * 4 + i;
                const int bp = dir == 0 ? (mb_edge ? i * 4 + 3 : bq - 1) : (mb_edge ? 12 + i : bq - 4);
                bool intra_p = is_intra, pcoef;
                int pref, pmx, pmy;
                const int qref = is_intra ? -1 : 0, qmx = fmv[bq][0], qmy = fmv[bq][1];
                const bool qcoef = (cbp_blk >> bq) & 1;
                if (mb_edge && PRE) {
                    intra_p = s.nintra[dir];
                    pcoef = (s.nbits[dir] >> bp) & 1;
                    pref = intra_p ? -1 : 0;
                    pmx = s.nmv[dir][i][0]; pmy = s.nmv[dir][i][1];
                } else if (mb_edge) {
                    const int nx = dir == 0 ? mbx - 1 : mbx, ny = dir == 0 ? mby : mby - 1;
                    const jmh_mb_result *rp = d.res + ny * d.mbw + nx;
                    intra_p = rp->mb_type == JMH_I4MB || rp->mb_type == JMH_I16MB || rp->mb_type == JMH_I8MB;
                    pcoef = (rp->cbp_blk >> bp) & 1;
                    pref = intra_p ? -1 : 0;
                    pmx = rp->mv[bp][0]; pmy = rp->mv[bp][1];
                } else {
                    pcoef = (cbp_blk >> bp) & 1;
                    pref = qref; pmx = fmv[bp][0]; pmy = fmv[bp][1];
                }
                if (intra_p || is_intra) bS = mb_edge ? 4 : 3;
                else if (pcoef || qcoef) bS = 2;
                else if (pref != qref || abs(pmx - qmx) >= 4 || abs(pmy - qmy) >= 4) bS = 1;
            }
            s.bs[dir][e][i] = (int8_t)bS;
        }
        __syncthreads();
        if (tid < 64 && filt) {
            const int offA = d.lf_offA, offB = d.lf_offB, bsc = 1 << (d.qpbd / 6);
            const int iA = iclip(0, 51, qpy + offA), iB = iclip(0, 51, qpy + offB);
            const int alpha = bsc * c_alpha[iA], beta = bsc * c_beta[iB];
            const int t1 = bsc * c_tc0[iA][0], t2 = bsc * c_tc0[iA][1], t3 = bsc * c_tc0[iA][2];
            const int cA = iclip(0, 51, qpcy + offA), cB = iclip(0, 51, qpcy + offB);
            const int calpha = bsc * c_alpha[cA], cbeta = bsc * c_beta[cB];
            const int u1 = bsc * c_tc0[cA][0], u2 = bsc * c_tc0[cA][1], u3 = bsc * c_tc0[cA][2];
            for (int dir = 0; dir < 2; dir++)
                for (int e = 0; e < 4; e++) {
                    if (tid < 16 && !((e & 1) && t8flag)) {
                        const int k = tid, b = s.bs[dir][e][k >> 2];
                        if (b) {
                            pel *q = dir == 0 ? &s.dy[k + 4][4 * e + 4] : &s.dy[4 * e + 4][k + 4];
                            filter_line(q, dir == 0 ? 1 : 20, b, alpha, beta, b == 1 ? t1 : b == 2 ? t2 : t3, false, maxv);
                        }
                    } else if (tid < 32 && !(e & 1)) {
                        const int pl = (tid - 16) >> 3, k = tid & 7, b = s.bs[dir][e][k >> 1];
                        if (b) {
                            pel *q = dir == 0 ? &s.dc2[pl][k + 4][2 * e + 4] : &s.dc2[pl][2 * e + 4][k + 4];
                            filter_line(q, dir == 0 ? 1 : 12, b, calpha, cbeta, b == 1 ? u1 : b == 2 ? u2 : u3, true, maxv);
                        }
                    }
                    wave_lds_sync();
                }
        }
        __syncthreads();
        for (int i = tid; i < 400 + 288; i += NTH) {
            if (i < 400) {
                const int r = i / 20 - 4, c = i % 20 - 4;
                if ((r >= 0 && c >= 0) || (r >= -3 && r < 0 && c >= 0 && dbT) || (c >= -3 && c < 0 && r >= 0 && dbL))
                    dbkY[(pix_y + r) * W + pix_x + c] = s.dy[r + 4][c + 4];
            } else {
                const int j = i - 400, pl = j / 144, r = (j % 144) / 12 - 4, c = j % 12 - 4;
                if ((r >= 0 && c >= 0) || (r == -1 && c >= 0 && c < 8 && dbT) || (c == -1 && r >= 0 && r < 8 && dbL))
                    if (r < 8 && c < 8) (pl ? dbkV : dbkU)[((pix_y >> 1) + r) * Wc + (pix_x >> 1) + c] = s.dc2[pl][r + 4][c + 4];
            }
        }
    }
}
```

h264-jm-commentary_amd/csrc/jmh_device.h:

```cpp
#pragma once
#include <hip/hip_runtime.h>
#include <stdint.h>
#include "../../include/jmhip.h"

#define SRMAX 32
#define SIDE_MAX (2 * SRMAX + 1)
#define NPOS_MAX (SIDE_MAX * SIDE_MAX)
#define QPAD 4
#define NT 256
#define NTA 512
#define NPK 10
#define NPK2 ((NPK + 1) / 2)
#define ORDTAB_SPOS (NPK2 * NTA)
#define BIGCOST (1 << 20)
#define PMAX 33
#define PIPE_LAG 16
__host__ __device__ __forceinline__ int ref_reach(int sr) { return sr <= SRMAX ? 5 : (19 + 2 * sr) / 16; }
__host__ __device__ __forceinline__ int pipe_lag(int sr) { return sr <= SRMAX ? PIPE_LAG : 3 * ref_reach(sr) + 1; }

struct MbScratch {
    int16_t all_mv[8][16][2];
    uint16_t fpc[7][16];
    int32_t motion_cost[8][4];
    int32_t best8x8;
    int32_t cost8x8;
    int32_t skipx, skipy;
    int32_t i4cost, i4cbp, i4blk;
    int32_t i16cost, i16mode, c_mode;
    int8_t ipred[16];
    int16_t i4lev[16][16];
    alignas(4) uint8_t i4rec[512];
    int32_t i8cost, i8cbp, i8modes;
    int16_t i8lev[16][16];
    alignas(4) uint8_t i8rec[512];
};

struct MbCarry {
    int32_t best8x8, cost8x8;
    int32_t skipx, skipy;
    int32_t i4cost, i4cbp, i4blk;
    int32_t i16cost, i16mode, c_mode;
};
template <class SC> struct ScrKind { static constexpr bool global = false; };
template <> struct ScrKind<MbScratch> { static constexpr bool global = true; };
template <class SC> constexpr bool scr_global = ScrKind<SC>::global;

struct jmr_mbinfo;
struct RdoPic {
    double lambda;
    int32_t lf;
    int32_t pad;
    uint8_t *cab;
    uint32_t *range;
    jmr_mbinfo *mbi;
};

__host__ __device__ __forceinline__ size_t rdo_pic_offset(size_t nmb) { return (nmb * sizeof(MbScratch) + 15) & ~(size_t)15; }

struct DevParams {
    int W, H, Wc, Hc, mbw, mbh;
    int sr, side, npos;
    int search_mode, use_hadamard, restrict_sr;
    int isr;
    int t8;
    int epzs_dual;
    int epzs_subpel;
    int epzs_spts;
    int epzs_mints, epzs_maxts;
    int slice_mbs;
    int maxv, qpbd;
    const uint8_t *orgY, *orgU, *orgV;
    const uint8_t *refY, *refU, *refV;
    uint8_t *recY, *recU, *recV;
    uint8_t *dbkY, *dbkU, *dbkV;
    int lf_disable, lf_offA, lf_offB;
    int16_t *mv;
    int8_t *refidx;
    int8_t *ipred;
    const int16_t *tmv;
    const int8_t *tref;
    const uint32_t *ordtab;
    jmh_mb_result *res;
    MbScratch *scr;
    unsigned long long *prof;
    int prof_mb;
    int slice_type, qp, lambda_mode, lambda_motion, cqp_off;
    int qsel;
    int diag, y_min;
    int rdo;
    int lf;
    double lambda_rd;
    int cavlc;
    const RdoPic *rp;
    int cip;
    int i16c;
};

struct MbAvail { bool L, T, TL, TR; };
__device__ __forceinline__ MbAvail mb_avail(const DevParams &d, int mbx, int mby) {
    const int a = mby * d.mbw + mbx, first = a - a % d.slice_mbs;
    MbAvail v;
    v.L = mbx > 0 && a - 1 >= first;
    v.T = mby > 0 && a - d.mbw >= first;
    v.TL = mbx > 0 && mby > 0 && a - d.mbw - 1 >= first;
    v.TR = mby > 0 && mbx + 1 < d.mbw && a - d.mbw + 1 >= first;
    return v;
}
__device__ __forceinline__ MbAvail intra_avail(const DevParams &d, int mbx, int mby) {
    MbAvail v = mb_avail(d, mbx, mby);
    if (d.cip && d.slice_type == JMH_P_SLICE) {
        const int W4 = d.W >> 2, a = 4 * mby * W4 + 4 * mbx;
        v.L = v.L && d.refidx[a - 1] < 0;
        v.T = v.T && d.refidx[a - W4] < 0;
        v.TL = v.TL && d.refidx[a - W4 - 1] < 0;
        v.TR = v.TR && d.refidx[a - W4 + 4] < 0;
    }
    return v;
}

struct PicParams {
    const uint8_t *org, *ref;
    uint8_t *rec, *dbk;
    int16_t *mv;
    int8_t *refidx, *ipred;
    const int16_t *tmv;
    const int8_t *tref;
    jmh_mb_result *res;
    MbScratch *scr;
    int32_t lambda_mode, lambda_motion;
    int16_t diag, y_min;
    int16_t qsel;
    int8_t slice_type, qp, cqp_off, lf_disable, lf_offA, lf_offB;
};
struct TickArgs {
    int W, H, mbw, mbh, sr, search_mode, use_hadamard, restrict_sr;
    int inter_search[8];
    unsigned long long *prof;
    int prof_mb;
    unsigned long long *bprof;
    unsigned long long *bprof_fin;
    int me_in_analyse;
    int t8;
    int epzs_dual;
    int epzs_subpel, epzs_spts;
    int epzs_mints, epzs_maxts;
    int slice_mbs;
    int cip;
    int bd;
    int rdo;
    const int32_t *sched, *soff;
    void *rscr;
    void *ffs;
    unsigned long long ffs_slot;
    const uint32_t *ordtab;
    int npic, nP;
    int pre[PMAX + 1];
    PicParams p[PMAX];
};
__host__ __device__ __forceinline__ size_t ffs_slot_bytes(int sr) {
    const size_t np = (size_t)(2 * sr + 1) * (2 * sr + 1);
    return np * 5 * 8;
}
static_assert(sizeof(TickArgs) <= 4096, "TickArgs is passed by value in the kernel argument segment");

struct FlowPic {
    PicParams pp;
    uint32_t gen;
    int32_t ref_entry;
    uint32_t ref_gen;
    int32_t pad;
};
struct FlowArgs {
    int W, H, mbw, mbh, sr, search_mode, use_hadamard, restrict_sr;
    int isr;
    int slice_mbs;
    const uint32_t *ordtab;
    unsigned long long *prof;
    int prof_mb;
    const FlowPic *pics;
    const uint32_t *items;
    int nitems;
    int nmb, nring;
    unsigned *head;
    unsigned base;
    uint32_t *flags;
    unsigned *err;
    unsigned long long *fprof;
};
#define FLOW_ITEM(e, x, y) (((uint32_t)(e) << 24) | ((uint32_t)(y) << 12) | (uint32_t)(x))

struct IngestArgs {
    const uint8_t *plane[3];
    int64_t stride[3];
    uint8_t *dst;
    int w, h, W, H;
    uint32_t maxv;
    unsigned long long *clamped;
};

#define NXCD 8
__device__ __forceinline__ int xcd_block(int b, int n) { return (b % NXCD) * ((n + NXCD - 1) / NXCD) + b / NXCD; }
__host__ __device__ __forceinline__ int xcd_grid(int n) { return NXCD * ((n + NXCD - 1) / NXCD); }

__device__ __forceinline__ int tick_entry(const TickArgs &t, int idx) {
    int e = 0;
    while (e + 1 < t.npic && t.pre[e + 1] <= idx) e++;
    return e;
}
__device__ __forceinline__ bool inter_on(int isr, int mode) { return (isr >> mode) & 1; }
__device__ __forceinline__ DevParams tick_params(const TickArgs &t, int e) {
    DevParams d;
    const PicParams &q = t.p[e];
    d.W = t.W; d.H = t.H; d.Wc = t.W >> 1; d.Hc = t.H >> 1; d.mbw = t.mbw; d.mbh = t.mbh;
    d.sr = t.sr; d.side = 2 * t.sr + 1; d.npos = d.side * d.side;
    d.search_mode = t.search_mode; d.use_hadamard = t.use_hadamard; d.restrict_sr = t.restrict_sr;
    d.isr = 0;
#pragma unroll
    for (int i = 1; i < 8; i++) d.isr |= (t.inter_search[i] != 0) << i;
    d.t8 = t.t8;
    d.epzs_dual = t.epzs_dual;
    d.epzs_subpel = t.epzs_subpel; d.epzs_spts = t.epzs_spts;
    d.epzs_mints = t.epzs_mints; d.epzs_maxts = t.epzs_maxts;
    d.slice_mbs = t.slice_mbs;
    d.maxv = (1 << t.bd) - 1; d.qpbd = 6 * (t.bd - 8);
    const int ps = t.bd > 8 ? 2 : 1, ls = t.W * t.H * ps, lc = ls >> 2;
    d.orgY = q.org; d.orgU = q.org + ls; d.orgV = q.org + ls + lc;
    d.refY = q.ref; d.refU = q.ref + ls; d.refV = q.ref + ls + lc;
    d.recY = q.rec; d.recU = q.rec + ls; d.recV = q.rec + ls + lc;
    d.dbkY = q.dbk; d.dbkU = q.dbk ? q.dbk + ls : nullptr; d.dbkV = q.dbk ? q.dbk + ls + lc : nullptr;
    d.lf_disable = q.lf_disable; d.lf_offA = q.lf_offA; d.lf_offB = q.lf_offB;
    d.mv = q.mv; d.refidx = q.refidx; d.ipred = q.ipred; d.res = q.res; d.scr = q.scr;
    d.tmv = q.tmv; d.tref = q.tref; d.ordtab = t.ordtab;
    d.prof = e == 0 ? t.prof : nullptr; d.prof_mb = t.prof_mb;
    d.slice_type = q.slice_type; d.qp = q.qp; d.lambda_mode = q.lambda_mode; d.lambda_motion = q.lambda_motion;
    d.cqp_off = q.cqp_off; d.qsel = q.qsel; d.diag = q.diag; d.y_min = q.y_min;
    d.rdo = t.rdo;
    d.cavlc = t.rdo == 2;
    d.i16c = 0;
    d.cip = t.cip;
    d.lf = q.lambda_motion << 16;
    d.lambda_rd = 0;
    d.rp = nullptr;
    if (t.rdo) {
        d.rp = reinterpret_cast<const RdoPic *>(reinterpret_cast<const uint8_t *>(q.scr) + rdo_pic_offset((size_t)t.mbw * t.mbh));
        d.lf = d.rp->lf;
        d.lambda_rd = d.rp->lambda;
    }
    return d;
}

__device__ __forceinline__ void tick_mb(const TickArgs &t, const DevParams &d, int e, int m, int &mbx, int &mby) {
    if (t.rdo) {
        const int a = t.sched[t.soff[d.diag] + (m - t.pre[e])];
        mby = a / d.mbw;
        mbx = a - mby * d.mbw;
    } else {
        mby = d.y_min + (m - t.pre[e]);
        mbx = d.diag - 2 * mby;
    }
}

template <class pel> __device__ __forceinline__ pel *spl(uint8_t *p) { return reinterpret_cast<pel *>(p); }
template <class pel> __device__ __forceinline__ const pel *spl(const uint8_t *p) { return reinterpret_cast<const pel *>(p); }
```

h264-jm-commentary_amd/csrc/jmh_final.h:

```cpp
#ifndef JMH_FINAL_H
#define JMH_FINAL_H
#include "jmh_deblock.h"
#include "jmh_intra.h"

template <class pel>
struct FinS {
    pel org[256];
    pel orgc[2][64];
    pel rec[256];
    pel pred[256];
    int tdc[4][2];
    pel rtop[24];
    pel rleft[16];
    pel ctop[2][12];
    pel cleft[2][8];
    int16_t fmv[16][2];
    int16_t lev[16][16];
    int bcost[16];
    int bnz[16];
    int dc[16];
    int dcdq[16];
    int16_t dclev[16];
    int cdcin[2][4];
    int cdcq[2][4];
    int16_t cdc[2][4];
    int16_t cac[2][4][16];
    int cbcost[2][4];
    int cbnz[2][4];
    int creset[2];
    int cdcnz[2];
    pel cfin[2][64];
    DbkS<pel> db;
};

template <class pel>
struct ScratchAnalysis {
    const MbScratch *sc;
    __device__ __forceinline__ int motion_cost(int m, int k) const { return sc->motion_cost[m][k]; }
    __device__ __forceinline__ int mv(int m, int k, int c) const { return sc->all_mv[m][k][c]; }
    __device__ __forceinline__ int best8x8() const { return sc->best8x8; }
    __device__ __forceinline__ int cost8x8() const { return sc->cost8x8; }
    __device__ __forceinline__ int skipx() const { return sc->skipx; }
    __device__ __forceinline__ int skipy() const { return sc->skipy; }
    __device__ __forceinline__ int i4cost() const { return sc->i4cost; }
    __device__ __forceinline__ int i4cbp() const { return sc->i4cbp; }
    __device__ __forceinline__ int i4blk() const { return sc->i4blk; }
    __device__ __forceinline__ int i4lev(int blk, int l) const { return sc->i4lev[blk][l]; }
    __device__ __forceinline__ pel i4rec(int i) const { return spl<pel>(sc->i4rec)[i]; }
    __device__ __forceinline__ int ipred(int k) const { return sc->ipred[k]; }
    __device__ __forceinline__ int i16cost() const { return sc->i16cost; }
    __device__ __forceinline__ int i16mode() const { return sc->i16mode; }
    __device__ __forceinline__ int c_mode() const { return sc->c_mode; }
    __device__ __forceinline__ int i8cost() const { return sc->i8cost; }
    __device__ __forceinline__ int i8cbp() const { return sc->i8cbp; }
    __device__ __forceinline__ int i8modes() const { return sc->i8modes; }
    __device__ __forceinline__ int i8lev(int blk, int l) const { return sc->i8lev[blk][l]; }
    __device__ __forceinline__ pel i8rec(int i) const { return spl<pel>(sc->i8rec)[i]; }
};

template <int OCC, class pel, bool T8, int NTH, class MC, class AV>
__device__ __forceinline__ void final_core(DevParams d, FinS<pel> &s, int mbx, int mby, int tid, MC mc, AV an, const pel *porg = nullptr,
                                           const IntraNb<pel> *pnb = nullptr) {
    constexpr bool W2 = NTH == 512;
    static_assert(NTH == 256 || NTH == 512, "final_core runs on 256 or 512 threads");
    if constexpr (!T8) d.t8 = 0;
    if constexpr (sizeof(pel) == 1) { d.maxv = 255; d.qpbd = 0; }
    const bool lu = !W2 || tid < 256;
    const int ct = W2 ? tid - 256 : tid;
    const bool chv = ct >= 0 && ct < 128;
    const int pix_x = 16 * mbx, pix_y = 16 * mby;
    const int W = d.W, Wc = d.Wc, W4 = d.W >> 2;
    const int slice_p = d.slice_type == JMH_P_SLICE;
    const int qpy = d.qp, qp = d.qp + d.qpbd, maxv = d.maxv;
    const pel *orgY = spl<pel>(d.orgY), *orgU = spl<pel>(d.orgU), *orgV = spl<pel>(d.orgV);
    const pel *refU = spl<pel>(d.refU), *refV = spl<pel>(d.refV);
    pel *recY = spl<pel>(d.recY), *recU = spl<pel>(d.recU), *recV = spl<pel>(d.recV);
    const MbAvail mav = intra_avail(d, mbx, mby);
    const bool avL = mav.L, avT = mav.T, avTL = mav.TL;
    const bool prof = prof_mb_here(d, mbx, mby);
    PSTAMP(16);

    const pel *S_org = porg ? porg : s.org;
    const pel(*S_orgc)[64] = pnb ? pnb->orgc : s.orgc;
    const pel *S_rtop = pnb ? pnb->rtop : s.rtop, *S_rleft = pnb ? pnb->rleft : s.rleft;
    const pel(*S_ctop)[12] = pnb ? pnb->ctop : s.ctop;
    const pel(*S_cleft)[8] = pnb ? pnb->cleft : s.cleft;
    if (lu && !porg) s.org[tid] = orgY[(pix_y + (tid >> 4)) * W + pix_x + (tid & 15)];
    if (d.dbkY) deblock_prefetch<pel, NTH>(d, s.db, mbx, mby, tid);
    if (!pnb && (!W2 || tid >= 256)) {
        const int u = ct;
        if (u < 128) {
            const int uv = u >> 6, k = u & 63;
            s.orgc[uv][k] = (uv ? orgV : orgU)[((pix_y >> 1) + (k >> 3)) * Wc + (pix_x >> 1) + (k & 7)];
        } else if (u >= 128 && u < 149) {
            const int x = u - 129;
            const bool av = x < 0 ? avTL : x < 16 ? avT : false;
            s.rtop[x + 1] = av ? recY[(pix_y - 1) * W + pix_x + x] : 0;
        } else if (u >= 160 && u < 176) {
            const int y = u - 160;
            s.rleft[y] = avL ? recY[(pix_y + y) * W + pix_x - 1] : 0;
        } else if (u >= 192 && u < 210) {
            const int i = u - 192, uv = i / 9, x = i - 9 * uv - 1;
            const bool av = x < 0 ? avTL : avT;
            s.ctop[uv][x + 1] = av ? (uv ? recV : recU)[((pix_y >> 1) - 1) * Wc + (pix_x >> 1) + x] : 0;
        } else if (u >= 224 && u < 240) {
            const int i = u - 224, uv = i >> 3, y = i & 7;
            s.cleft[uv][y] = avL ? (uv ? recV : recU)[((pix_y >> 1) + y) * Wc + (pix_x >> 1) - 1] : 0;
        }
    }

    int min_cost = BIGCOST, best_mode = 1, best8x8 = 0;
    if (slice_p) {
        for (int mode = 1; mode < 4; mode++) {
            if (!inter_on(d.isr, mode)) continue;
            const int cost = mode == 1 ? an.motion_cost(1, 0) : an.motion_cost(mode, 0) + an.motion_cost(mode, 1);
            if (cost < min_cost) { best_mode = mode; min_cost = cost; }
        }
        if (inter_on(d.isr, 4) || inter_on(d.isr, 5) || inter_on(d.isr, 6) || inter_on(d.isr, 7)) {
            best8x8 = an.best8x8();
            if (an.cost8x8() < min_cost) { best_mode = JMH_P8x8; min_cost = an.cost8x8(); }
        }
    }
    if (d.t8 && an.i8cost() <= min_cost) { min_cost = an.i8cost(); best_mode = JMH_I8MB; }
    if (an.i4cost() <= min_cost) { min_cost = an.i4cost(); best_mode = JMH_I4MB; }
    const int i16mode = an.i16mode();
    if (an.i16cost() < min_cost) { min_cost = an.i16cost(); best_mode = JMH_I16MB; }
    const int is_intra = best_mode == JMH_I4MB || best_mode == JMH_I16MB || best_mode == JMH_I8MB;
    int b8mode[4];
    for (int b = 0; b < 4; b++)
        b8mode[b] = best_mode == JMH_P8x8 ? (best8x8 >> (4 * b)) & 15 : best_mode == JMH_I4MB ? JMH_IBLOCK : best_mode == JMH_I16MB ? 0
                  : best_mode == JMH_I8MB ? JMH_I8MB : best_mode;
    if (tid < 32) {
        const int k = tid >> 1, c = tid & 1, b8 = ((k >> 3) << 1) + ((k & 3) >> 1);
        const int bm = best_mode == JMH_P8x8 ? (best8x8 >> (4 * b8)) & 15 : best_mode;
        s.fmv[k][c] = is_intra ? 0 : an.mv(bm, k, c);
    }
    __syncthreads();

    const int c_mode = is_intra ? an.c_mode() : 0;
    const int l = tid & 15;
    const int cuv = (ct >> 4) >> 2, cb = (ct >> 4) & 3;
    const int cxo = (cb & 1) * 4 + (ct & 3), cyo = (cb >> 1) * 4 + ((ct & 15) >> 2);
    int cpredv = 0;
    if (chv) {
        if (is_intra) {
            cpredv = chroma_pred_px(S_ctop[cuv] + 1, S_cleft[cuv], S_ctop[cuv][0], avT, avL, c_mode, cxo, cyo, maxv);
        } else {
            const pel *R = cuv ? refV : refU;
            const int vx = s.fmv[(cyo >> 1) * 4 + (cxo >> 1)][0], vy = s.fmv[(cyo >> 1) * 4 + (cxo >> 1)][1];
            const int ii = ((pix_x >> 1) + cxo) * 8 + vx, jj = ((pix_y >> 1) + cyo) * 8 + vy;
            const int x0 = iclip(0, Wc - 1, ii >> 3), y0 = iclip(0, d.Hc - 1, jj >> 3);
            const int x1 = iclip(0, Wc - 1, (ii + 7) >> 3), y1 = iclip(0, d.Hc - 1, (jj + 7) >> 3);
            const int fx = ii & 7, fy = jj & 7;
            cpredv = ((8 - fx) * (8 - fy) * R[y0 * Wc + x0] + fx * (8 - fy) * R[y0 * Wc + x1] + (8 - fx) * fy * R[y1 * Wc + x0] +
                      fx * fy * R[y1 * Wc + x1] + 32) >> 6;
        }
    }
    const int qpi = iclip(-d.qpbd, 51, qpy + d.cqp_off), qpcy = qpi < 0 ? qpi : c_qpc[qpi], qpc = qpcy + d.qpbd;
    const int cq_bits = 15 + qpc / 6;
    const int cqp_const = q_round(d.qsel, cq_bits);
    int cdq = 0;
    auto chroma_a = [&]() {
        if (chv) {
            const int c = lane_fwd4x4(S_orgc[cuv][cyo * 8 + cxo] - cpredv, l);
            if (l == 0) s.cdcin[cuv][cb] = c;
            int lev, cc;
            unsigned nz = lane_quant(c, l, qpc, cqp_const, true, lev, cdq, cc);
            s.cac[cuv][cb][l] = (int16_t)lev;
            if (l == 0) { s.cbcost[cuv][cb] = cc; s.cbnz[cuv][cb] = nz != 0; }
        }
    };
    auto chroma_b = [&]() {
        if (ct >= 0 && ct < 2) {
            const int uv = ct, qp_per = qpc / 6, qp_rem = qpc % 6;
            const int *m = s.cdcin[uv];
            int m1[4] = {m[0] + m[1] + m[2] + m[3], m[0] - m[1] + m[2] - m[3], m[0] + m[1] - m[2] - m[3], m[0] - m[1] - m[2] + m[3]};
            int dcnz = 0;
            for (int k = 0; k < 4; k++) {
                int level = (abs(m1[k]) * c_q3[qp_rem][0] + 2 * cqp_const) >> (cq_bits + 1);
                if (level) dcnz = 1;
                s.cdc[uv][k] = (int16_t)isign(level, m1[k]);
            }
            int c0 = s.cdc[uv][0], c1 = s.cdc[uv][1], c2 = s.cdc[uv][2], c3 = s.cdc[uv][3];
            int fv[4] = {c0 + c1 + c2 + c3, c0 - c1 + c2 - c3, c0 + c1 - c2 - c3, c0 - c1 - c2 + c3};
            int v00 = c_dq3[qp_rem][0];
            for (int k = 0; k < 4; k++) s.cdcq[uv][k] = (fv[k] * 16 * v00 * (1 << qp_per)) >> 5;
            int cost = s.cbcost[uv][0] + s.cbcost[uv][1] + s.cbcost[uv][2] + s.cbcost[uv][3];
            int acany = s.cbnz[uv][0] | s.cbnz[uv][1] | s.cbnz[uv][2] | s.cbnz[uv][3];
            s.creset[uv] = cost < 4;
            s.cdcnz[uv] = (dcnz ? 1 : 0) | (acany && cost >= 4 ? 2 : 0);
        }
    };
    auto chroma_c = [&]() {
        if (chv) {
            if (s.creset[cuv]) { cdq = 0; s.cac[cuv][cb][l] = 0; }
            if (l == 0) cdq = s.cdcq[cuv][cb];
            s.cfin[cuv][cyo * 8 + cxo] = (pel)lane_inv4x4(cdq, l, cpredv, maxv);
        }
    };
    if constexpr (W2) chroma_a();

    int cbp = 0, cbp_blk = 0;
    bool tr8 = false;
    const int blk = tid >> 4, lx = l & 3, ly = l >> 2;
    const int px4 = 4 * (blk & 3) + lx, py4 = 4 * (blk >> 2) + ly;
    const int w8 = tid >> 6, l8 = tid & 63;
    const int qx = 8 * (w8 & 1) + (l8 & 7), qy = 8 * (w8 >> 1) + (l8 >> 3);
    if (best_mode == JMH_I8MB) {
        cbp = an.i8cbp(); tr8 = true;
        for (int b = 0; b < 4; b++)
            if ((cbp >> b) & 1) cbp_blk |= 0x33 << ((b >> 1) * 8 + (b & 1) * 2);
        if (lu) {
            s.lev[blk][l] = (int16_t)an.i8lev(blk, l);
            s.rec[tid] = an.i8rec(tid);
        }
    } else if (best_mode == JMH_I4MB) {
        cbp = an.i4cbp(); cbp_blk = an.i4blk();
        if (lu) {
            s.lev[blk][l] = (int16_t)an.i4lev(blk, l);
            s.rec[tid] = an.i4rec(tid);
        }
    } else if (best_mode == JMH_I16MB) {
        int p = 0, org = 0;
        if (lu) {
            const pel *T = S_rtop + 1, *L = S_rleft;
            const I16Par par = i16_params(T, L, avT, avL, (maxv + 1) >> 1);
            p = i16_pred(par, T, L, i16mode, px4, py4, maxv);
            org = (int)S_org[py4 * 16 + px4];
        }
        int lev, rv;
        i16_code(p, org, qp, q_round(q_sel16(d.qsel), 15 + qp / 6), s.dc, s.dcdq, s.dclev, s.bnz, tid, maxv, lev, rv, lu);
        if (lu) {
            s.lev[blk][l] = (int16_t)lev;
            s.rec[py4 * 16 + px4] = (pel)rv;
        }
        __syncthreads();
        for (int b = 0; b < 16; b++)
            if (s.bnz[b]) { cbp = 15; cbp_blk |= 1 << b; }
    } else {
        const int p = lu ? mc(4 * (pix_x + px4) + s.fmv[blk][0], 4 * (pix_y + py4) + s.fmv[blk][1]) : 0;
        if (d.t8 && (best_mode <= 3 || best8x8 == 0x4444)) {
            if (lu) s.pred[py4 * 16 + px4] = (pel)p;
            __syncthreads();
            if (lu) {
                const int dv = S_org[qy * 16 + qx] - s.pred[qy * 16 + qx];
                const int c4 = wave_satd4x4s(dv, l8, d.use_hadamard), c8 = wave_satd8(dv, l8, d.use_hadamard);
                if (l8 == 0) { s.tdc[w8][0] = c4; s.tdc[w8][1] = c8; }
            }
            __syncthreads();
            tr8 = s.tdc[0][1] + s.tdc[1][1] + s.tdc[2][1] + s.tdc[3][1] < s.tdc[0][0] + s.tdc[1][0] + s.tdc[2][0] + s.tdc[3][0];
        }
        if (tr8) {
            int lev = 0, rv = 0, pv = 0;
            if (lu) {
                pv = s.pred[qy * 16 + qx];
                const int q8 = 16 + qp / 6;
                const int c = wave_fwd8x8(S_org[qy * 16 + qx] - pv, l8);
                int dq, cc;
                const unsigned long long nz = wave_quant8(c, l8, qp, q_round(d.qsel, q8), lev, dq, cc);
                rv = wave_inv8x8(dq, l8, pv, maxv);
                if (l8 == 0) { s.bcost[w8] = cc; s.bnz[w8] = nz != 0; }
            }
            __syncthreads();
            int sum_cnt = 0, keep8 = 0;
            for (int b8 = 0; b8 < 4; b8++) {
                int c8 = s.bcost[b8];
                if (c8 <= 4) c8 = 0;
                else {
                    keep8 |= 1 << b8;
                    if (s.bnz[b8]) { cbp |= 1 << b8; cbp_blk |= 0x33 << ((b8 >> 1) * 8 + (b8 & 1) * 2); }
                }
                sum_cnt += c8;
            }
            if (sum_cnt <= 5) { keep8 = 0; cbp = 0; cbp_blk = 0; }
            if (lu) {
                const bool keep = (keep8 >> w8) & 1;
                s.lev[il_blk(w8, l8)][l8 >> 2] = keep ? (int16_t)lev : 0;
                s.rec[qy * 16 + qx] = (pel)(keep ? rv : pv);
            }
        } else {
        int lev = 0, rv = 0;
        if (lu) {
            const int c = lane_fwd4x4(S_org[py4 * 16 + px4] - p, l);
            int dq, cc;
            const int q_bits = 15 + qp / 6;
            unsigned nz = lane_quant(c, l, qp, q_round(d.qsel, q_bits), false, lev, dq, cc);
            rv = lane_inv4x4(dq, l, p, maxv);
            if (l == 0) { s.bcost[blk] = cc; s.bnz[blk] = nz != 0; }
        }
        __syncthreads();
        int sum_cnt = 0, keep8 = 0;
        for (int b8 = 0; b8 < 4; b8++) {
            int base = (b8 >> 1) * 8 + (b8 & 1) * 2;
            int c8 = s.bcost[base] + s.bcost[base + 1] + s.bcost[base + 4] + s.bcost[base + 5];
            int nz8 = s.bnz[base] | s.bnz[base + 1] | s.bnz[base + 4] | s.bnz[base + 5];
            if (c8 <= 4) c8 = 0;
            else {
                keep8 |= 1 << b8;
                if (nz8) cbp |= 1 << b8;
                for (int q = 0; q < 4; q++) {
                    int k = base + (q & 1) + (q >> 1) * 4;
                    if (s.bnz[k]) cbp_blk |= 1 << k;
                }
            }
            sum_cnt += c8;
        }
        if (sum_cnt <= 5) { keep8 = 0; cbp = 0; cbp_blk = 0; }
        if (lu) {
            const int mb8 = ((blk >> 3) << 1) + ((blk & 3) >> 1);
            const bool keep = (keep8 >> mb8) & 1;
            s.lev[blk][l] = keep ? (int16_t)lev : 0;
            s.rec[py4 * 16 + px4] = (pel)(keep ? rv : p);
        }
        }
    }
    const bool t8flag = tr8 && (best_mode == JMH_I8MB || (cbp & 15));
    PSTAMP(17);

    if constexpr (!W2) chroma_a();
    __syncthreads();
    chroma_b();
    __syncthreads();
    chroma_c();
    __syncthreads();
    PSTAMP(18);
    int cr = 0;
    for (int uv = 0; uv < 2; uv++) {
        if (s.cdcnz[uv] & 1) cr = max(cr, 1);
        if (s.cdcnz[uv] & 2) cr = 2;
    }
    cbp |= cr << 4;

    jmh_mb_result *res = d.res + mby * d.mbw + mbx;
    int mb_type = best_mode;
    if (slice_p && best_mode == 1 && cbp == 0 && s.fmv[0][0] == an.skipx() && s.fmv[0][1] == an.skipy()) mb_type = JMH_PSKIP;
    if (tid == 0) {
        res->mb_type = (int16_t)mb_type;
        res->cbp = (int16_t)cbp;
        res->cbp_blk = cbp_blk;
        for (int b = 0; b < 4; b++) {
            res->b8mode[b] = (int8_t)(mb_type == JMH_PSKIP ? 0 : b8mode[b]);
            res->ref_idx[b] = (int8_t)(is_intra ? -1 : 0);
        }
        res->i16mode = (int8_t)(best_mode == JMH_I16MB ? i16mode : 0);
        res->c_ipred_mode = (int8_t)c_mode;
        res->transform_8x8 = (int8_t)t8flag; res->pad0 = 0;
        res->min_cost = min_cost;
        res->reserved = 0;
    }
    if (lu) res->luma[blk][l] = s.lev[blk][l];
    if (tid < 16) {
        const int k = tid;
        const int ip = best_mode == JMH_I4MB ? an.ipred(k)
                     : best_mode == JMH_I8MB ? (an.i8modes() >> (4 * (((k >> 3) << 1) + ((k & 3) >> 1)))) & 15 : 2;
        res->ipred[k] = (int8_t)ip;
        res->mv[k][0] = s.fmv[k][0]; res->mv[k][1] = s.fmv[k][1];
        res->luma_dc[k] = best_mode == JMH_I16MB ? s.dclev[k] : 0;
        const int a = ((pix_y >> 2) + (k >> 2)) * W4 + (pix_x >> 2) + (k & 3);
        d.mv[2 * a] = s.fmv[k][0]; d.mv[2 * a + 1] = s.fmv[k][1];
        d.refidx[a] = (int8_t)(is_intra ? -1 : 0);
        d.ipred[a] = (int8_t)ip;
    }
    if (tid < 8) { const int uv = tid >> 2, k = tid & 3; res->chroma_dc[uv][k] = s.cdc[uv][k]; }
    if (chv) {
        const int uv = ct >> 6, b = (ct >> 4) & 3, q = ct & 15;
        res->chroma_ac[uv][b][q] = s.cac[uv][b][q];
        const int k = ct & 63;
        (uv ? recV : recU)[((pix_y >> 1) + (k >> 3)) * Wc + (pix_x >> 1) + (k & 7)] = s.cfin[uv][k];
    }
    if (lu) recY[(pix_y + (tid >> 4)) * W + pix_x + (tid & 15)] = s.rec[tid];

    if (d.dbkY) deblock_mb<pel, NTH, true>(d, s.db, s.rec, s.cfin, s.fmv, is_intra, cbp_blk, t8flag, qpy, qpcy, mbx, mby, tid);
    PSTAMP(19);
}

template <int OCC, class pel, bool T8, int NTH = NT>
__device__ __forceinline__ void final_mb(const TickArgs &t, FinS<pel> &s, int m, int tid, int hwb, unsigned long long bt0) {
    const int e = tick_entry(t, m);
    const DevParams d = tick_params(t, e);
    const int mby = d.y_min + (m - t.pre[e]), mbx = d.diag - 2 * mby;
    const pel *refY = spl<pel>(d.refY);
    const int W = d.W, H = d.H, maxv = sizeof(pel) == 1 ? 255 : d.maxv;
    auto mc = [=](int X, int Y) { return qpel_direct<pel, OCC == 8>(refY, W, H, X, Y, maxv); };
    final_core<OCC, pel, T8, NTH>(d, s, mbx, mby, tid, mc, ScratchAnalysis<pel>{d.scr + mby * d.mbw + mbx});
    if (t.bprof_fin && tid == 0) {
        t.bprof_fin[3 * hwb] = bt0;
        t.bprof_fin[3 * hwb + 1] = wall_clock64();
        t.bprof_fin[3 * hwb + 2] = 3;
    }
}

#endif
```

h264-jm-commentary_amd/csrc/jmh_i4.h:

```cpp
#pragma once
#include "jmh_common.h"
#include "jmh_intra.h"

template <class pel>
struct IntraS {
    alignas(4) pel org[256];
    alignas(4) pel rec[256];
    Border bd;
    IntraNb<pel> nb;
    int8_t ipred_cur[16];
    int part[2][4];
};

__device__ __forceinline__ int quad_fwd4x4(int r, int l) {
    const int y = l >> 2, x = l & 3;
    const int v0 = dpp<0x00>(r), v1 = dpp<0x55>(r), v2 = dpp<0xAA>(r), v3 = dpp<0xFF>(r);
    const int t = fwd_tap(v0 + v3, v1 + v2, v1 - v2, v0 - v3, x);
    const int u0 = g16(t, x), u1 = g16(t, 4 + x), u2 = g16(t, 8 + x), u3 = g16(t, 12 + x);
    return fwd_tap(u0 + u3, u1 + u2, u1 - u2, u0 - u3, y);
}
__device__ __forceinline__ int quad_inv4x4(int dq, int l, int pred, int maxv) {
    const int y = l >> 2, x = l & 3;
    const int d0 = dpp<0x00>(dq), d1 = dpp<0x55>(dq), d2 = dpp<0xAA>(dq), d3 = dpp<0xFF>(dq);
    const int t = inv_tap(d0 + d2, d0 - d2, (d1 >> 1) - d3, d1 + (d3 >> 1), x);
    const int f0 = g16(t, x), f1 = g16(t, 4 + x), f2 = g16(t, 8 + x), f3 = g16(t, 12 + x);
    const int o = inv_tap(f0 + f2, f0 - f2, (f1 >> 1) - f3, f1 + (f3 >> 1), y);
    return iclip(0, maxv, (o + (pred << 6) + 32) >> 6);
}

__device__ __forceinline__ void i4_tabrow(int lane, int (&tabr)[2]) {
    const int m = lane >> 2, y = lane & 3;
    tabr[0] = m < 9 ? (int)(c_i4tab[m][4 * y] | (uint32_t)c_i4tab[m][4 * y + 1] << 16) : 0;
    tabr[1] = m < 9 ? (int)(c_i4tab[m][4 * y + 2] | (uint32_t)c_i4tab[m][4 * y + 3] << 16) : 0;
}

template <class pel>
__device__ __forceinline__ void i4_block(const DevParams &d, IntraS<pel> &s, int16_t (*i4lev)[16], int w, int bx4, int by4, const int (&tabr)[2],
                                         bool avL, bool avT, bool avTL, bool avTR, int qpk, int (&acc)[3],
                                         unsigned long long *pst = nullptr) {
#define I4ST(k, v) do { if (pst) { asm volatile("" ::"v"(v)); if (__lane_id() == 0) pst[k] = wall_clock64(); } } while (0)
    I4ST(52, bx4);
    const int lane = threadIdx.x & 63, l = lane & 15;
    const int bx = 4 * bx4, by = 4 * by4, blk = 4 * by4 + bx4;
    const int lambda = d.lambda_mode, qp = d.qp + d.qpbd, had = d.use_hadamard;
    const bool up = by > 0 || avT, left = bx > 0 || avL;
    const bool ul = (bx > 0 && by > 0) || (bx == 0 && by > 0 && avL) || (bx > 0 && by == 0 && avT) || (bx == 0 && by == 0 && avTL);
    bool ur = by == 0 ? (bx + 4 <= 15 ? avT : avTR) : (bx + 4 <= 15);
    if ((bx == 4 || bx == 12) && (by == 4 || by == 12)) ur = false;
    (void)w;
    const int mtop = -(int)(lane >= 1 && lane <= 8), mleft = -(int)(lane >= 9);
    const int lx = (lane <= 4 || ur) ? lane - 1 : 3;
    const int px = bx + ((lx & mtop) | (-1 & ~mtop)), py = by + (((lane - 9) & mleft) | (-1 & ~mleft));
    const bool pav = lane < 13 && (lane == 0 ? ul : lane <= 8 ? up : left);
    const int mT = -(int)(py < 0), mL = ~mT & -(int)(px < 0);
    const int ofs = (((int)(s.nb.rtop - s.rec) + px + 1) & mT) | (((int)(s.nb.rleft - s.rec) + py) & mL) | ((16 * py + px) & ~(mT | mL));
    const int raw = s.rec[pav ? ofs : 0];
    const int v = pav ? raw : 0;
    const int upM = by > 0 ? s.ipred_cur[blk - 4] : s.bd.ipm[1 + bx4];
    const int leftM = bx > 0 ? s.ipred_cur[blk - 1] : s.bd.ipm[6 + by4];
    const int mpm = intra_mpm(upM, leftM);
    const int m = lane >> 2, y = lane & 3;
    int o[4];
    if constexpr (sizeof(pel) == 1) {
        const uint32_t ow = *reinterpret_cast<const uint32_t *>(s.org + (by + y) * 16 + bx);
#pragma unroll
        for (int x = 0; x < 4; x++) o[x] = (int)((ow >> (8 * x)) & 255u);
    } else {
        const uint2 ow = *reinterpret_cast<const uint2 *>(s.org + (by + y) * 16 + bx);
        o[0] = (int)(ow.x & 0xFFFFu); o[1] = (int)(ow.x >> 16); o[2] = (int)(ow.y & 0xFFFFu); o[3] = (int)(ow.y >> 16);
    }
    const int org = s.org[(by + (l >> 2)) * 16 + bx + (l & 3)];
    int st = 0, sl = 0;
#pragma unroll
    for (int i = 0; i < 4; i++) { st += __builtin_amdgcn_readlane(v, 1 + i); sl += __builtin_amdgcn_readlane(v, 9 + i); }
    const int dc = (up && left) ? (st + sl + 4) >> 3 : left ? (sl + 2) >> 2 : up ? (st + 2) >> 2 : (d.maxv + 1) >> 1;
    I4ST(53, mpm);
    int pr[4], dd[4];
#pragma unroll
    for (int x = 0; x < 4; x++) {
        const int e = (int)(((uint32_t)tabr[x >> 1] >> (16 * (x & 1))) & 0xFFFFu), ty = e & 3;
        const int a = __shfl(v, (e >> 2) & 15, 64), b = __shfl(v, (e >> 6) & 15, 64), c = __shfl(v, (e >> 10) & 15, 64);
        const int f1 = (a + b + 1) >> 1, f2 = (a + 2 * b + c + 2) >> 2;
        const int m1 = -(int)(ty == 1), m2 = -(int)(ty == 2);
        pr[x] = (f1 & m1) | (f2 & m2) | (dc & ~(m1 | m2));
        dd[x] = o[x] - pr[x];
    }
    int t;
    if (had) {
        const int h0 = dd[0] + dd[1], h1 = dd[0] - dd[1], h2 = dd[2] + dd[3], h3 = dd[2] - dd[3];
        int g[4] = {h0 + h2, h1 + h3, h0 - h2, h1 - h3};
#pragma unroll
        for (int x = 0; x < 4; x++) { const int q = dpp<0xB1>(g[x]); g[x] = (y & 1) ? q - g[x] : g[x] + q; }
#pragma unroll
        for (int x = 0; x < 4; x++) { const int q = dpp<0x4E>(g[x]); g[x] = (y & 2) ? q - g[x] : g[x] + q; }
        t = abs(g[0]) + abs(g[1]) + abs(g[2]) + abs(g[3]);
    } else {
        t = abs(dd[0]) + abs(dd[1]) + abs(dd[2]) + abs(dd[3]);
    }
    t += dpp<0xB1>(t);
    t += dpp<0x4E>(t);
    const int sat = had ? t >> 1 : t;
    const int cst = (m < 9 && intra_mode_ok(m, up, left, ul)) ? (m == mpm ? 0 : 4 * lambda) + sat : BIGCOST;
    const unsigned key = wave_min_u32((y == 0 && cst < BIGCOST) ? ((unsigned)cst << 4) | (unsigned)m : 0xFFFFFFFFu);
    I4ST(54, key);
    const int best = key == 0xFFFFFFFFu ? 0 : (int)(key & 15u), bc = key == 0xFFFFFFFFu ? BIGCOST : (int)(key >> 4);
    const int srcl = 4 * best + (l >> 2);
    const int q01 = __shfl((pr[0] & 0xFFFF) | (pr[1] << 16), srcl, 64), q23 = __shfl((pr[2] & 0xFFFF) | (pr[3] << 16), srcl, 64);
    const int qx = (l & 2) ? q23 : q01;
    const int pp = (l & 1) ? (int)((uint32_t)qx >> 16) : (qx & 0xFFFF);
    I4ST(55, pp);
    const int c = quad_fwd4x4(org - pp, l);
    int lev, dq, cc;
    unsigned nz = lane_quant(c, l, qp, qpk, false, lev, dq, cc);
    I4ST(56, dq);
    const int rc = quad_inv4x4(dq, l, pp, d.maxv);
    if (lane < 16) {
        i4lev[blk][l] = (int16_t)lev;
        s.rec[(by + (l >> 2)) * 16 + bx + (l & 3)] = (pel)rc;
        if (l == 0) s.ipred_cur[blk] = (int8_t)best;
    }
    nz = __builtin_amdgcn_readlane(nz, 0);
    I4ST(57, nz);
#undef I4ST
    acc[0] += bc;
    if (nz) { acc[1] |= 1 << ((by4 >> 1) * 2 + (bx4 >> 1)); acc[2] |= 1 << blk; }
}
```

h264-jm-commentary_amd/csrc/jmh_intra.h:

```cpp
#pragma once
#include "jmh_common.h"

static __constant__ uint16_t c_i4tab[9][16] = {
    {0x0446, 0x088A, 0x0CCE, 0x1112, 0x0446, 0x088A, 0x0CCE, 0x1112, 0x0446, 0x088A, 0x0CCE, 0x1112, 0x0446, 0x088A, 0x0CCE, 0x1112},
    {0x2666, 0x2666, 0x2666, 0x2666, 0x2AAA, 0x2AAA, 0x2AAA, 0x2AAA, 0x2EEE, 0x2EEE, 0x2EEE, 0x2EEE, 0x3332, 0x3332, 0x3332, 0x3332},
    {0x0003, 0x0003, 0x0003, 0x0003, 0x0003, 0x0003, 0x0003, 0x0003, 0x0003, 0x0003, 0x0003, 0x0003, 0x0003, 0x0003, 0x0003, 0x0003},
    {0x0C86, 0x10CA, 0x150E, 0x1952, 0x10CA, 0x150E, 0x1952, 0x1D96, 0x150E, 0x1952, 0x1D96, 0x21DA, 0x1952, 0x1D96, 0x21DA, 0x221E},
    {0x2406, 0x0842, 0x0C86, 0x10CA, 0x2A42, 0x2406, 0x0842, 0x0C86, 0x2EA6, 0x2A42, 0x2406, 0x0842, 0x32EA, 0x2EA6, 0x2A42, 0x2406},
    {0x0041, 0x0085, 0x00C9, 0x010D, 0x0426, 0x0842, 0x0C86, 0x10CA, 0x026A, 0x0041, 0x0085, 0x00C9, 0x26AE, 0x0426, 0x0842, 0x0C86},
    {0x0241, 0x0426, 0x004A, 0x048E, 0x02A5, 0x2A42, 0x0241, 0x0426, 0x02E9, 0x2EA6, 0x02A5, 0x2A42, 0x032D, 0x32EA, 0x02E9, 0x2EA6},
    {0x0085, 0x00C9, 0x010D, 0x0151, 0x0C86, 0x10CA, 0x150E, 0x1952, 0x00C9, 0x010D, 0x0151, 0x0195, 0x10CA, 0x150E, 0x1952, 0x1D96},
    {0x02A5, 0x2EA6, 0x02E9, 0x32EA, 0x02E9, 0x32EA, 0x032D, 0x332E, 0x032D, 0x332E, 0x3332, 0x3332, 0x3332, 0x3332, 0x3332, 0x3332}};

template <class pel>
struct IntraNb {
    pel orgc[2][64];
    pel rtop[24];
    pel rleft[16];
    pel ctop[2][12];
    pel cleft[2][8];
};
template <class pel>
__device__ __forceinline__ void load_intra_nb(const DevParams &d, IntraNb<pel> &nb, int t, int mbx, int mby) {
    const pel *recY = spl<pel>(d.recY), *recU = spl<pel>(d.recU), *recV = spl<pel>(d.recV);
    const int pix_x = 16 * mbx, pix_y = 16 * mby, W = d.W, Wc = d.Wc;
    const MbAvail mav = intra_avail(d, mbx, mby);
    const bool avL = mav.L, avT = mav.T, avTL = mav.TL, avTR = mav.TR;
    if (t < 21) {
        const int x = t - 1;
        const bool av = x < 0 ? avTL : x < 16 ? avT : avTR;
        nb.rtop[x + 1] = av ? recY[(pix_y - 1) * W + pix_x + x] : 0;
    } else if (t < 37) {
        const int y = t - 21;
        nb.rleft[y] = avL ? recY[(pix_y + y) * W + pix_x - 1] : 0;
    } else if (t < 55) {
        const int i = t - 37, uv = i / 9, x = i - 9 * uv - 1;
        const bool av = x < 0 ? avTL : avT;
        nb.ctop[uv][x + 1] = av ? (uv ? recV : recU)[((pix_y >> 1) - 1) * Wc + (pix_x >> 1) + x] : 0;
    } else if (t < 71) {
        const int i = t - 55, uv = i >> 3, y = i & 7;
        nb.cleft[uv][y] = avL ? (uv ? recV : recU)[((pix_y >> 1) + y) * Wc + (pix_x >> 1) - 1] : 0;
    }
}
template <class pel>
__device__ __forceinline__ void load_orgc(const DevParams &d, IntraNb<pel> &nb, int t, int mbx, int mby) {
    const int uv = t >> 6, k = t & 63;
    nb.orgc[uv][k] = spl<pel>(uv ? d.orgV : d.orgU)[((8 * mby) + (k >> 3)) * d.Wc + 8 * mbx + (k & 7)];
}

__host__ __device__ constexpr bool intra_mode_ok(int m, bool up, bool left, bool ul) {
    return m == 2 || ((m == 0 || m == 3 || m == 7) && up) || ((m == 1 || m == 8) && left) || (up && left && ul);
}
__host__ __device__ constexpr bool chroma_mode_ok(int m, bool avL, bool avT, bool avTL) { return m == 0 || (m == 1 ? avL : m == 2 ? avT : avT && avL && avTL); }
__host__ __device__ constexpr bool i16_mode_ok(int m, bool avL, bool avT, bool avTL) { return m == 2 || (m == 0 ? avT : m == 1 ? avL : avT && avL && avTL); }
__host__ __device__ constexpr int intra_mpm(int a, int b) { return (a < 0 || b < 0) ? 2 : a < b ? a : b; }
__host__ __device__ constexpr int intra_rem(int m, int mpm) { return m == mpm ? -1 : m < mpm ? m : m - 1; }

struct BlkAvail { bool up, left, ul, ur; };
__host__ __device__ constexpr BlkAvail i4_avail(int bx, int by, const MbAvail &mav) {
    return {by > 0 || mav.T, bx > 0 || mav.L,
            (bx > 0 && by > 0) || (bx == 0 && by > 0 && mav.L) || (bx > 0 && by == 0 && mav.T) || (bx == 0 && by == 0 && mav.TL),
            (by == 0 ? (bx + 4 <= 15 ? mav.T : mav.TR) : (bx + 4 <= 15)) && !((bx == 4 || bx == 12) && (by == 4 || by == 12))};
}
__host__ __device__ constexpr BlkAvail i8_avail(int b8, const MbAvail &mav) {
    return {(b8 & 2) ? true : mav.T, (b8 & 1) ? true : mav.L, b8 == 3 ? true : b8 == 1 ? mav.T : b8 == 2 ? mav.L : mav.TL,
            b8 == 0 ? mav.T : b8 == 1 ? mav.TR : b8 == 2};
}

namespace intra_rules_check {
constexpr bool mode_ok_all() {
    for (int m = 0; m < 9; m++)
        for (int f = 0; f < 8; f++) {
            const bool up = f & 1, left = f & 2, ul = f & 4, dir = ((m == 0 || m == 3 || m == 7) && up) || ((m == 1 || m == 8) && left);
            if (intra_mode_ok(m, up, left, ul) != (m == 2 || dir || (up && left && ul)) ||
                intra_mode_ok(m, up, left, ul) != (m == 2 || dir || ((m == 4 || m == 5 || m == 6) && up && left && ul)))
                return false;
        }
    return true;
}
constexpr bool mpm_rem_all() {
    for (int a = -1; a < 9; a++)
        for (int b = -1; b < 9; b++) {
            const int p = intra_mpm(a, b), r = intra_rem(b, a);
            if (p != ((a < 0 || b < 0) ? 2 : (a < b ? a : b))) return false;
            if (a >= 0 && b >= 0 && (a == b ? r != -1 : (r < 0 || r > 7 || (r < a ? r : r + 1) != b))) return false;
        }
    return true;
}
constexpr bool i4_ur_all() {
    for (int k = 0; k < 16; k++)
        if (i4_avail(4 * (k & 3), 4 * (k >> 2), MbAvail{false, true, false, true}).ur != (((0x575F >> k) & 1) != 0)) return false;
    return true;
}
static_assert(mode_ok_all(), "intra_mode_ok differs from the Intra4x4 / Intra8x8 spellings on m in [0, 9)");
static_assert(mpm_rem_all(), "intra_mpm / intra_rem over modes -1..8");
static_assert(i4_ur_all(), "i4_avail: the upper-right flags");
}

template <class S>
__device__ __forceinline__ int lpix(const S &s, int x, int y) {
    if (y < 0) return s.nb.rtop[x + 1];
    if (x < 0) return s.nb.rleft[y];
    return s.rec[16 * y + x];
}

struct I8Edge { int raw[25], av[25], f[25]; };
template <class pel>
__device__ __forceinline__ void i8_edge_load(I8Edge &e, int t, int b8, const BlkAvail &v, const pel *rec, const pel *recY, int pix_x, int pix_y, int W) {
    if (t >= 25) return;
    const int bx = 8 * (b8 & 1), by = 8 * (b8 >> 1);
    int xm, ym;
    bool a;
    if (t < 8) { xm = bx - 1; ym = by + 7 - t; a = v.left; }
    else if (t == 8) { xm = bx - 1; ym = by - 1; a = v.ul; }
    else { const int xx = t - 9; xm = bx + (xx < 8 || v.ur ? xx : 7); ym = by - 1; a = v.up; }
    int s = 0;
    if (a) s = (xm >= 0 && xm < 16 && ym >= 0) ? rec[ym * 16 + xm] : recY[(pix_y + ym) * W + pix_x + xm];
    e.raw[t] = s; e.av[t] = a;
}
__device__ __forceinline__ void i8_edge_filter(I8Edge &e, int t) {
    if (t >= 25 || !e.av[t]) return;
    const int c = e.raw[t];
    const int lo = t > 0 && e.av[t - 1] ? e.raw[t - 1] : c, hi = t < 24 && e.av[t + 1] ? e.raw[t + 1] : c;
    e.f[t] = (lo + 2 * c + hi + 2) >> 2;
}
__device__ __forceinline__ int i8_edge_dc(const I8Edge &e, bool up, bool left, int maxv) {
    int st = 0, sl = 0;
    for (int i = 0; i < 8; i++) { st += up ? e.f[9 + i] : 0; sl += left ? e.f[i] : 0; }
    return up && left ? (st + sl + 8) >> 4 : up ? (st + 4) >> 3 : left ? (sl + 4) >> 3 : (maxv + 1) >> 1;
}

template <class pel>
__device__ __forceinline__ void i16_pick(const DevParams &d, const pel *org, const IntraNb<pel> &nb, int lane, bool avL, bool avT, bool avTL,
                                         int &cost16, int &mode16) {
    const int m = lane >> 4, b = lane & 15, ox = (b & 3) * 4, oy = (b >> 2) * 4;
    const pel *T = nb.rtop + 1, *L = nb.rleft;
    const int k = lane & 15, nv = lane < 16 ? (int)T[k] : (int)L[k];
    const int s1 = row16_sum(nv), s2 = row16_sum((k - 7) * nv);
    const int st = __builtin_amdgcn_readlane(s1, 0), sl = __builtin_amdgcn_readlane(s1, 16);
    const int corner = T[-1];
    const int ih = __builtin_amdgcn_readlane(s2, 0) - 8 * corner, iv = __builtin_amdgcn_readlane(s2, 16) - 8 * corner;
    const int dcv = (avT && avL) ? (st + sl + 16) >> 5 : avT ? (st + 8) >> 4 : avL ? (sl + 8) >> 4 : (d.maxv + 1) >> 1;
    const int ib = (5 * ih + 32) >> 6, ic = (5 * iv + 32) >> 6, iaa = 16 * (L[15] + T[15]);
    int tx[4], ly[4];
#pragma unroll
    for (int i = 0; i < 4; i++) { tx[i] = T[ox + i]; ly[i] = L[oy + i]; }
    int mm[16], t[16];
#pragma unroll
    for (int yy = 0; yy < 4; yy++) {
        int o[4];
        if constexpr (sizeof(pel) == 1) {
            const uint32_t w = *reinterpret_cast<const uint32_t *>(org + (oy + yy) * 16 + ox);
#pragma unroll
            for (int xx = 0; xx < 4; xx++) o[xx] = (int)((w >> (8 * xx)) & 255u);
        } else {
#pragma unroll
            for (int xx = 0; xx < 4; xx++) o[xx] = org[(oy + yy) * 16 + ox + xx];
        }
#pragma unroll
        for (int xx = 0; xx < 4; xx++) {
            const int pl = clipmx((iaa + (ox + xx - 7) * ib + (oy + yy - 7) * ic + 16) >> 5, d.maxv);
            const int p = m == 0 ? tx[xx] : m == 1 ? ly[yy] : m == 2 ? dcv : pl;
            mm[4 * yy + xx] = o[xx] - p;
        }
    }
    for (int yy = 0; yy < 4; yy++) {
        int *r = mm + 4 * yy;
        int a0 = r[0] + r[3], a1 = r[1] + r[2], a2 = r[1] - r[2], a3 = r[0] - r[3];
        t[4 * yy] = a0 + a1; t[4 * yy + 2] = a0 - a1; t[4 * yy + 1] = a2 + a3; t[4 * yy + 3] = a3 - a2;
    }
    int acs = 0, dcc = 0;
    for (int xx = 0; xx < 4; xx++) {
        int a0 = t[xx] + t[12 + xx], a1 = t[4 + xx] + t[8 + xx], a2 = t[4 + xx] - t[8 + xx], a3 = t[xx] - t[12 + xx];
        int o0 = a0 + a1, o2 = a0 - a1, o1 = a2 + a3, o3 = a3 - a2;
        if (xx == 0) dcc = o0; else acs += abs(o0);
        acs += abs(o1) + abs(o2) + abs(o3);
    }
    const int cost = row16_sum(acs) + lane_had_abs(dcc / 4, b);
    int best = MAX_VALUE, i16mode = 2;
#pragma unroll
    for (int k2 = 0; k2 < 4; k2++) {
        const int c = __builtin_amdgcn_readlane(cost, 16 * k2);
        if (i16_mode_ok(k2, avL, avT, avTL) && c < best) { best = c; i16mode = k2; }
    }
    cost16 = best / 2;
    mode16 = i16mode;
}

__device__ __forceinline__ void i16_dc(int *dc, int16_t *dclev, int *dcdq, int qp, int qp_const) {
    const int qp_per = qp / 6, qp_rem = qp % 6, q_bits = 15 + qp_per, qp_const2 = qp_const << 1;
    for (int yy = 0; yy < 4; yy++) {
        int *r = dc + 4 * yy;
        int a0 = r[0] + r[3], a3 = r[0] - r[3], a1 = r[1] + r[2], a2 = r[1] - r[2];
        r[0] = a0 + a1; r[2] = a0 - a1; r[1] = a3 + a2; r[3] = a3 - a2;
    }
    for (int xx = 0; xx < 4; xx++) {
        int a0 = dc[xx] + dc[12 + xx], a3 = dc[xx] - dc[12 + xx], a1 = dc[4 + xx] + dc[8 + xx], a2 = dc[4 + xx] - dc[8 + xx];
        dc[xx] = (a0 + a1) >> 1; dc[8 + xx] = (a0 - a1) >> 1; dc[4 + xx] = (a3 + a2) >> 1; dc[12 + xx] = (a3 - a2) >> 1;
    }
    int lev[16];
    for (int k = 0; k < 16; k++) {
        int pos = scan_of(k);
        int level = (abs(dc[pos]) * c_q3[qp_rem][0] + qp_const2) >> (q_bits + 1);
        dclev[k] = (int16_t)isign(level, dc[pos]);
        lev[pos] = dclev[k];
    }
    int t[16];
    for (int yy = 0; yy < 4; yy++) {
        const int *cc = lev + 4 * yy;
        int e0 = cc[0] + cc[2], e1 = cc[0] - cc[2], e2 = cc[1] - cc[3], e3 = cc[1] + cc[3];
        t[4 * yy] = e0 + e3; t[4 * yy + 3] = e0 - e3; t[4 * yy + 1] = e1 + e2; t[4 * yy + 2] = e1 - e2;
    }
    int v00 = c_dq3[qp_rem][0];
    for (int xx = 0; xx < 4; xx++) {
        int e0 = t[xx] + t[8 + xx], e1 = t[xx] - t[8 + xx], e2 = t[4 + xx] - t[12 + xx], e3 = t[4 + xx] + t[12 + xx];
        int fv[4] = {e0 + e3, e1 + e2, e1 - e2, e0 - e3};
        for (int yy = 0; yy < 4; yy++) dcdq[4 * yy + xx] = (fv[yy] * v00 * (1 << qp_per) + 2) >> 2;
    }
}

__device__ __forceinline__ void i16_code(int p, int org, int qp, int qp_const, int *dc, int *dcdq, int16_t *dclev, int *bnz, int tid,
                                         int maxv, int &lev_out, int &rec_out, bool act = true) {
    if (!act) { __syncthreads(); __syncthreads(); lev_out = rec_out = 0; return; }
    const int blk = tid >> 4, l = tid & 15;
    const int c = lane_fwd4x4(org - p, l);
    if (l == 0) dc[blk] = c;
    __syncthreads();
    if (tid == 0) i16_dc(dc, dclev, dcdq, qp, qp_const);
    __syncthreads();
    int lev, dq, cc;
    unsigned nz = lane_quant(c, l, qp, qp_const, true, lev, dq, cc);
    if (l == 0) { dq = dcdq[blk]; bnz[blk] = nz != 0; }
    lev_out = lev;
    rec_out = lane_inv4x4(dq, l, p, maxv);
}
```

Before: 1470.

## Type device pointers as global address space and restructure border, window and deblock fetches

Device pointers in DevParams and the kernels are retyped as address_space(1) global pointers in the flow TU, so the compiler can emit global rather than flat loads. The reference-window fetch now always does clamped aligned word loads and builds edge pixels from the loaded words instead of separate byte loads. The deblock neighbour fetch is split into a register-staged fetch issued early and an LDS stage done after chroma prediction, so its latency overlaps other work. Border loads now write both copies from one read, and intra-neighbour loads are moved earlier on the pre path. The change touches many load paths and adds register pressure from the staged deblock words.

```diff
diff --git a/h264-jm-commentary_amd/csrc/jmh_analyse.hip b/h264-jm-commentary_amd/csrc/jmh_analyse.hip
--- a/h264-jm-commentary_amd/csrc/jmh_analyse.hip
+++ b/h264-jm-commentary_amd/csrc/jmh_analyse.hip
@@ -26,7 +26,7 @@
         int16_t h1[WIN_DIM_MAX * WST];
         uint2 sad8[NPK * NTA];
     } hs;
-    unsigned long long *pst;
+    gptr<unsigned long long> pst;
     int pn;
     alignas(8) IntraS<uint8_t> in;
 };
@@ -575,8 +575,11 @@
     const bool prof = prof_mb_here(d, mbx, mby);
     PSTAMP(0);
     if (tid == 0) { s.pst = prof ? d.prof + 20 : nullptr; s.pn = 0; }
-    if (tid < 256) { if (!pre) s.in.org[tid] = s.org[tid] = d.orgY[(pix_y + (tid >> 4)) * W + pix_x + (tid & 15)]; }
-    else if (tid >= 384 && tid < 394) { load_border(d, s.bd, tid - 384, mbx, mby); load_border(d, s.in.bd, tid - 384, mbx, mby); }
+    if (tid < 256) {
+        if (!pre) s.in.org[tid] = s.org[tid] = d.orgY[(pix_y + (tid >> 4)) * W + pix_x + (tid & 15)];
+        else if (tid >= 128 && tid < 199) load_intra_nb_batch(d, s.in.nb, tid - 128, mbx, mby);
+    }
+    else if (tid >= 384 && tid < 394) load_border(d, s.bd, tid - 384, mbx, mby, &s.in.bd);
     else if (!pre && tid >= 472 && tid < 478) s.in.part[(tid - 472) / 3][(tid - 472) % 3] = 0;
     else if (!pre && tid >= 480 && tid < 512) s.motion_cost[(tid - 480) >> 2][tid & 3] = 0;
     auto idle = [&](int k, int w) { intra_slot(d, s.in, scr, i4lev, k, w, mbx, mby); };
@@ -598,9 +601,10 @@
             const int task = tid + i * NTA;
             const int y = task / ND4, j = task - y * ND4, x0 = X0 + 4 * j;
             fast[i] = task < wdim * ND4 && 4 * j + 3 < wdim && x0 >= 0 && x0 + 3 < W;
-            const uint32_t *p = reinterpret_cast<const uint32_t *>(d.refY + iclip(0, d.H - 1, Y0 + y) * W + (fast[i] ? (x0 & ~3) : 0));
+            const int bx = iclip(0, W - 4, x0 & ~3);
+            const gptr<const uint32_t> p = reinterpret_cast<gptr<const uint32_t>>(d.refY + iclip(0, d.H - 1, Y0 + y) * W + bx);
             lo_[i] = p[0];
-            hi_[i] = (fast[i] && (x0 & 3)) ? p[1] : 0u;
+            hi_[i] = ((x0 & 3) && bx + 4 < W) ? p[1] : 0u;
         }
 #pragma unroll
         for (int i = 0; i < NWT; i++) {
@@ -610,16 +614,18 @@
             uint32_t v;
             if (fast[i]) v = __builtin_amdgcn_alignbyte(hi_[i], lo_[i], x0 & 3);
             else {
-                const uint8_t *row = d.refY + iclip(0, d.H - 1, Y0 + y) * W;
+                const int bx = iclip(0, W - 4, x0 & ~3);
                 v = 0;
 #pragma unroll
-                for (int q = 0; q < 4; q++)
-                    if (4 * j + q < wdim) v |= (uint32_t)row[iclip(0, W - 1, x0 + q)] << (8 * q);
+                for (int q = 0; q < 4; q++) {
+                    const int c = iclip(0, W - 1, x0 + q) - bx;
+                    if (4 * j + q < wdim) v |= (((c < 4 ? lo_[i] : hi_[i]) >> (8 * (c & 3))) & 255u) << (8 * q);
+                }
             }
             *reinterpret_cast<uint32_t *>(G + y * WST + 4 * j) = v;
         }
         if (tid < 32) G[wdim * WST + tid] = 0;
-        if (tid >= 128 && tid < 199) load_intra_nb(d, s.in.nb, tid - 128, mbx, mby);
+        if (!pre && tid >= 128 && tid < 199) load_intra_nb(d, s.in.nb, tid - 128, mbx, mby);
     }
     __syncthreads();
     PSTAMP(1);
@@ -741,7 +747,7 @@
     const bool prof = act && prof_mb_here(d, mbx, mby);
     PSTAMP(12);
     if (act) {
-        const pel *orgY = spl<pel>(d.orgY);
+        const gptr<const pel> orgY = spl<pel>(d.orgY);
         s.org[tid] = orgY[(pix_y + (tid >> 4)) * W + pix_x + (tid & 15)];
         s.org[tid + 128] = orgY[(pix_y + 8 + (tid >> 4)) * W + pix_x + (tid & 15)];
         load_orgc(d, s.nb, tid, mbx, mby);
@@ -797,7 +803,7 @@
         const int by4 = by_lo + w, bx4 = k - 2 * by4;
         if (by4 <= 3 && bx4 >= 0 && bx4 <= 3) {
             int acc[3] = {s.part[w][0], s.part[w][1], s.part[w][2]};
-            unsigned long long *pst = (k == 4 && w == 0 && d.prof && d.prof_mb == mby * d.mbw + mbx) ? d.prof : nullptr;
+            const gptr<unsigned long long> pst = (k == 4 && w == 0 && d.prof && d.prof_mb == mby * d.mbw + mbx) ? d.prof : nullptr;
             i4_block(d, s, i4lev, w, bx4, by4, tabr, avL, avT, avTL, avTR, qpk, acc, pst);
             if (lane == 0) { s.part[w][0] = acc[0]; s.part[w][1] = acc[1]; s.part[w][2] = acc[2]; }
         }
@@ -910,15 +916,11 @@
     d.slice_mbs = f.slice_mbs;
     d.maxv = 255; d.qpbd = 0;
     const int ls = W * H, lc = ls >> 2;
-    d.orgY = q.org; d.orgU = q.org + ls; d.orgV = q.org + ls + lc;
-    d.refY = q.ref; d.refU = q.ref + ls; d.refV = q.ref + ls + lc;
-    d.recY = q.rec; d.recU = q.rec + ls; d.recV = q.rec + ls + lc;
-    d.dbkY = q.dbk; d.dbkU = q.dbk ? q.dbk + ls : nullptr; d.dbkV = q.dbk ? q.dbk + ls + lc : nullptr;
+    set_pic_pointers(d, q, ls, lc);
     d.lf_disable = q.lf_disable; d.lf_offA = q.lf_offA; d.lf_offB = q.lf_offB;
-    d.mv = q.mv; d.refidx = q.refidx; d.ipred = q.ipred; d.res = q.res;
     d.scr = nullptr;
     d.tmv = nullptr; d.tref = nullptr; d.ordtab = f.ordtab;
-    d.prof = f.prof; d.prof_mb = f.prof_mb;
+    d.prof = to_global(f.prof); d.prof_mb = f.prof_mb;
     d.slice_type = q.slice_type; d.qp = q.qp; d.lambda_motion = q.lambda_motion;
     d.lambda_mode = __builtin_amdgcn_readfirstlane(q.lambda_mode);
     d.cqp_off = q.cqp_off; d.qsel = q.qsel; d.diag = q.diag; d.y_min = q.y_min;
@@ -958,6 +960,7 @@
 };
 
 struct FlowAnalysis {
+    static constexpr bool in_lds = true;
     const MeS &me;
     const IntraS<uint8_t> &in;
     const MbCarry &c;
diff --git a/h264-jm-commentary_amd/csrc/jmh_common.h b/h264-jm-commentary_amd/csrc/jmh_common.h
--- a/h264-jm-commentary_amd/csrc/jmh_common.h
+++ b/h264-jm-commentary_amd/csrc/jmh_common.h
@@ -301,18 +301,20 @@
     if (xN < 0) return yN > 15 ? -1 : 6 + (yN >> 2);
     return -1;
 }
-__device__ __forceinline__ void load_border(const DevParams &d, Border &b, int t, int mbx, int mby) {
+__device__ __forceinline__ void load_border(const DevParams &d, Border &b, int t, int mbx, int mby, Border *b2 = nullptr) {
     const int W4 = d.W >> 2;
     int by4 = t < 6 ? -1 : t - 6, bx4 = t < 6 ? t - 1 : -1;
     const MbAvail m = mb_avail(d, mbx, mby);
     bool av = by4 < 0 ? (bx4 < 0 ? m.TL : bx4 > 3 ? m.TR : m.T) : m.L;
-    int ref = -2, mx = 0, my = 0, ipm = -1;
+    int ref = -2, ipm = -1;
+    uint32_t mvw = 0;
     if (av) {
         int a = (4 * mby + by4) * W4 + 4 * mbx + bx4;
-        ref = d.refidx[a]; mx = d.mv[2 * a]; my = d.mv[2 * a + 1]; ipm = d.ipred[a];
+        ref = d.refidx[a]; mvw = *reinterpret_cast<gptr<const uint32_t>>(d.mv + 2 * a); ipm = d.ipred[a];
         if (d.cip && ref >= 0) ipm = -1;
     }
-    b.ref[t] = (int8_t)ref; b.mv[t][0] = (int16_t)mx; b.mv[t][1] = (int16_t)my; b.ipm[t] = (int8_t)ipm;
+    b.ref[t] = (int8_t)ref; b.mv[t][0] = (int16_t)(mvw & 0xFFFF); b.mv[t][1] = (int16_t)(mvw >> 16); b.ipm[t] = (int8_t)ipm;
+    if (b2) { b2->ref[t] = (int8_t)ref; b2->mv[t][0] = (int16_t)(mvw & 0xFFFF); b2->mv[t][1] = (int16_t)(mvw >> 16); b2->ipm[t] = (int8_t)ipm; }
 }
 struct NbBorder {
     const Border &b;
diff --git a/h264-jm-commentary_amd/csrc/jmh_deblock.h b/h264-jm-commentary_amd/csrc/jmh_deblock.h
--- a/h264-jm-commentary_amd/csrc/jmh_deblock.h
+++ b/h264-jm-commentary_amd/csrc/jmh_deblock.h
@@ -71,7 +71,7 @@
 
 template <class pel, int NTH>
 __device__ __forceinline__ void deblock_prefetch(const DevParams &d, DbkS<pel> &s, int mbx, int mby, int tid) {
-    const pel *dbkY = spl<pel>(d.dbkY), *dbkU = spl<pel>(d.dbkU), *dbkV = spl<pel>(d.dbkV);
+    const gptr<const pel> dbkY = spl<pel>(d.dbkY), dbkU = spl<pel>(d.dbkU), dbkV = spl<pel>(d.dbkV);
     const int pix_x = 16 * mbx, pix_y = 16 * mby, W = d.W, Wc = d.Wc;
     const bool dbL = mbx > 0, dbT = mby > 0;
     for (int i = tid; i < 256 + 16; i += NTH) {
@@ -88,7 +88,7 @@
             const int j = i - 256, dir = j >> 3, k = j & 7;
             const bool av = dir == 0 ? dbL : dbT;
             if (av) {
-                const jmh_mb_result *rp = d.res + (dir == 0 ? mby * d.mbw + mbx - 1 : (mby - 1) * d.mbw + mbx);
+                const gptr<const jmh_mb_result> rp = d.res + (dir == 0 ? mby * d.mbw + mbx - 1 : (mby - 1) * d.mbw + mbx);
                 if (k < 4) {
                     const int bp = dir == 0 ? k * 4 + 3 : 12 + k;
                     s.nmv[dir][k][0] = rp->mv[bp][0];
@@ -103,11 +103,79 @@
         }
     }
 }
+template <class pel> __device__ __forceinline__ unsigned dbk_byte(int c) { return ((unsigned)sizeof(pel) * (unsigned)c) & 3u; }
+template <int NTH> struct DbkFetch { uint32_t v[(256 + 16 + NTH - 1) / NTH]; };
+static_assert(offsetof(jmh_mb_result, mv) % 4 == 0 && offsetof(jmh_mb_result, cbp_blk) % 4 == 0 && offsetof(jmh_mb_result, mb_type) == 0 &&
+              sizeof(jmh_mb_result) % 4 == 0, "deblock_fetch reads the neighbour's results by aligned words");
+template <class pel, int NTH>
+__device__ __forceinline__ DbkFetch<NTH> deblock_fetch(const DevParams &d, int mbx, int mby, int tid) {
+    const gptr<const pel> dbkY = spl<pel>(d.dbkY), dbkU = spl<pel>(d.dbkU), dbkV = spl<pel>(d.dbkV);
+    const int pix_x = 16 * mbx, pix_y = 16 * mby, W = d.W, Wc = d.Wc;
+    const bool dbL = mbx > 0, dbT = mby > 0;
+    DbkFetch<NTH> f;
+#pragma unroll
+    for (int n = 0; n * NTH < 256 + 16; n++) {
+        const int i = tid + n * NTH;
+        gptr<const uint8_t> p = nullptr;
+        if (i < 128) {
+            const bool top = i < 64;
+            const int a = i & 63, r = top ? (a >> 4) - 4 : a >> 2, c = top ? a & 15 : (a & 3) - 4;
+            if (top ? dbT : dbL) p = reinterpret_cast<gptr<const uint8_t>>(dbkY + (pix_y + r) * W + pix_x + c);
+        } else if (i < 256) {
+            const int j = i - 128, pl = j >> 6, a = j & 63;
+            const bool top = a < 32;
+            const int b = a & 31, r = top ? (b >> 3) - 4 : b >> 2, c = top ? b & 7 : (b & 3) - 4;
+            if (top ? dbT : dbL) p = reinterpret_cast<gptr<const uint8_t>>((pl ? dbkV : dbkU) + ((pix_y >> 1) + r) * Wc + (pix_x >> 1) + c);
+        } else if (i < 256 + 16) {
+            const int j = i - 256, dir = j >> 3, k = j & 7;
+            if ((dir == 0 ? dbL : dbT) && k < 6) {
+                const gptr<const jmh_mb_result> rp = d.res + (dir == 0 ? mby * d.mbw + mbx - 1 : (mby - 1) * d.mbw + mbx);
+                const int bp = dir == 0 ? k * 4 + 3 : 12 + k;
+                const int off = k < 4 ? (int)offsetof(jmh_mb_result, mv) + 4 * bp : k == 4 ? (int)offsetof(jmh_mb_result, cbp_blk) : 0;
+                p = reinterpret_cast<gptr<const uint8_t>>(rp) + off;
+            }
+        }
+        f.v[n] = p ? *reinterpret_cast<gptr<const uint32_t>>(p - ((unsigned)(uintptr_t)p & 3u)) : 0u;
+    }
+    return f;
+}
+template <class pel, int NTH>
+__device__ __forceinline__ void deblock_stage(DbkS<pel> &s, const DbkFetch<NTH> &f, int mbx, int mby, int tid) {
+    const bool dbL = mbx > 0, dbT = mby > 0;
+#pragma unroll
+    for (int n = 0; n * NTH < 256 + 16; n++) {
+        const int i = tid + n * NTH;
+        const uint32_t v = f.v[n];
+        if (i < 128) {
+            const bool top = i < 64;
+            const int a = i & 63, r = top ? (a >> 4) - 4 : a >> 2, c = top ? a & 15 : (a & 3) - 4;
+            s.dy[r + 4][c + 4] = (pel)(v >> (8 * dbk_byte<pel>(c)));
+        } else if (i < 256) {
+            const int j = i - 128, pl = j >> 6, a = j & 63;
+            const bool top = a < 32;
+            const int b = a & 31, r = top ? (b >> 3) - 4 : b >> 2, c = top ? b & 7 : (b & 3) - 4;
+            s.dc2[pl][r + 4][c + 4] = (pel)(v >> (8 * dbk_byte<pel>(c)));
+        } else if (i < 256 + 16) {
+            const int j = i - 256, dir = j >> 3, k = j & 7;
+            if (dir == 0 ? dbL : dbT) {
+                if (k < 4) {
+                    s.nmv[dir][k][0] = (int16_t)(v & 0xFFFF);
+                    s.nmv[dir][k][1] = (int16_t)(v >> 16);
+                } else if (k == 4) {
+                    s.nbits[dir] = (int32_t)v;
+                } else if (k == 5) {
+                    const int t = (int16_t)(v & 0xFFFF);
+                    s.nintra[dir] = t == JMH_I4MB || t == JMH_I16MB || t == JMH_I8MB;
+                }
+            }
+        }
+    }
+}
 
 template <class pel, int NTH = NT, bool PRE = false>
 __device__ __forceinline__ void deblock_mb(const DevParams &d, DbkS<pel> &s, const pel *rec, const pel (*cfin)[64], const int16_t (*fmv)[2],
                                            bool is_intra, int cbp_blk, bool t8flag, int qpy, int qpcy, int mbx, int mby, int tid) {
-    pel *dbkY = spl<pel>(d.dbkY), *dbkU = spl<pel>(d.dbkU), *dbkV = spl<pel>(d.dbkV);
+    const gptr<pel> dbkY = spl<pel>(d.dbkY), dbkU = spl<pel>(d.dbkU), dbkV = spl<pel>(d.dbkV);
     const int pix_x = 16 * mbx, pix_y = 16 * mby, W = d.W, Wc = d.Wc, maxv = d.maxv;
     const bool dbL = mbx > 0, dbT = mby > 0;
     {
@@ -152,7 +220,7 @@
                     pmx = s.nmv[dir][i][0]; pmy = s.nmv[dir][i][1];
                 } else if (mb_edge) {
                     const int nx = dir == 0 ? mbx - 1 : mbx, ny = dir == 0 ? mby : mby - 1;
-                    const jmh_mb_result *rp = d.res + ny * d.mbw + nx;
+                    const gptr<const jmh_mb_result> rp = d.res + ny * d.mbw + nx;
                     intra_p = rp->mb_type == JMH_I4MB || rp->mb_type == JMH_I16MB || rp->mb_type == JMH_I8MB;
                     pcoef = (rp->cbp_blk >> bp) & 1;
                     pref = intra_p ? -1 : 0;
diff --git a/h264-jm-commentary_amd/csrc/jmh_device.h b/h264-jm-commentary_amd/csrc/jmh_device.h
--- a/h264-jm-commentary_amd/csrc/jmh_device.h
+++ b/h264-jm-commentary_amd/csrc/jmh_device.h
@@ -57,6 +57,14 @@
 
 __host__ __device__ __forceinline__ size_t rdo_pic_offset(size_t nmb) { return (nmb * sizeof(MbScratch) + 15) & ~(size_t)15; }
 
+#if defined(__HIP_DEVICE_COMPILE__) && defined(JMH_FLOW_TU)
+template <class T> using gptr = __attribute__((address_space(1))) T *;
+#define JMH_TYPED_GPTR 1
+#else
+template <class T> using gptr = T *;
+#endif
+template <class T> __host__ __device__ __forceinline__ gptr<T> to_global(T *p) { return (gptr<T>)p; }
+
 struct DevParams {
     int W, H, Wc, Hc, mbw, mbh;
     int sr, side, npos;
@@ -69,20 +77,20 @@
     int epzs_mints, epzs_maxts;
     int slice_mbs;
     int maxv, qpbd;
-    const uint8_t *orgY, *orgU, *orgV;
-    const uint8_t *refY, *refU, *refV;
-    uint8_t *recY, *recU, *recV;
-    uint8_t *dbkY, *dbkU, *dbkV;
+    gptr<const uint8_t> orgY, orgU, orgV;
+    gptr<const uint8_t> refY, refU, refV;
+    gptr<uint8_t> recY, recU, recV;
+    gptr<uint8_t> dbkY, dbkU, dbkV;
     int lf_disable, lf_offA, lf_offB;
-    int16_t *mv;
-    int8_t *refidx;
-    int8_t *ipred;
+    gptr<int16_t> mv;
+    gptr<int8_t> refidx;
+    gptr<int8_t> ipred;
     const int16_t *tmv;
     const int8_t *tref;
     const uint32_t *ordtab;
-    jmh_mb_result *res;
+    gptr<jmh_mb_result> res;
     MbScratch *scr;
-    unsigned long long *prof;
+    gptr<unsigned long long> prof;
     int prof_mb;
     int slice_type, qp, lambda_mode, lambda_motion, cqp_off;
     int qsel;
@@ -207,6 +215,15 @@
     while (e + 1 < t.npic && t.pre[e + 1] <= idx) e++;
     return e;
 }
+__device__ __forceinline__ void set_pic_pointers(DevParams &d, const PicParams &q, int ls, int lc) {
+    const gptr<const uint8_t> org = to_global(q.org), ref = to_global(q.ref);
+    const gptr<uint8_t> rec = to_global(q.rec), dbk = to_global(q.dbk);
+    d.orgY = org; d.orgU = org + ls; d.orgV = org + ls + lc;
+    d.refY = ref; d.refU = ref + ls; d.refV = ref + ls + lc;
+    d.recY = rec; d.recU = rec + ls; d.recV = rec + ls + lc;
+    d.dbkY = dbk; d.dbkU = dbk ? dbk + ls : nullptr; d.dbkV = dbk ? dbk + ls + lc : nullptr;
+    d.mv = to_global(q.mv); d.refidx = to_global(q.refidx); d.ipred = to_global(q.ipred); d.res = to_global(q.res);
+}
 __device__ __forceinline__ bool inter_on(int isr, int mode) { return (isr >> mode) & 1; }
 __device__ __forceinline__ DevParams tick_params(const TickArgs &t, int e) {
     DevParams d;
@@ -224,14 +241,11 @@
     d.slice_mbs = t.slice_mbs;
     d.maxv = (1 << t.bd) - 1; d.qpbd = 6 * (t.bd - 8);
     const int ps = t.bd > 8 ? 2 : 1, ls = t.W * t.H * ps, lc = ls >> 2;
-    d.orgY = q.org; d.orgU = q.org + ls; d.orgV = q.org + ls + lc;
-    d.refY = q.ref; d.refU = q.ref + ls; d.refV = q.ref + ls + lc;
-    d.recY = q.rec; d.recU = q.rec + ls; d.recV = q.rec + ls + lc;
-    d.dbkY = q.dbk; d.dbkU = q.dbk ? q.dbk + ls : nullptr; d.dbkV = q.dbk ? q.dbk + ls + lc : nullptr;
+    set_pic_pointers(d, q, ls, lc);
     d.lf_disable = q.lf_disable; d.lf_offA = q.lf_offA; d.lf_offB = q.lf_offB;
-    d.mv = q.mv; d.refidx = q.refidx; d.ipred = q.ipred; d.res = q.res; d.scr = q.scr;
+    d.scr = q.scr;
     d.tmv = q.tmv; d.tref = q.tref; d.ordtab = t.ordtab;
-    d.prof = e == 0 ? t.prof : nullptr; d.prof_mb = t.prof_mb;
+    d.prof = e == 0 ? to_global(t.prof) : nullptr; d.prof_mb = t.prof_mb;
     d.slice_type = q.slice_type; d.qp = q.qp; d.lambda_mode = q.lambda_mode; d.lambda_motion = q.lambda_motion;
     d.cqp_off = q.cqp_off; d.qsel = q.qsel; d.diag = q.diag; d.y_min = q.y_min;
     d.rdo = t.rdo;
@@ -262,3 +276,7 @@
 
 template <class pel> __device__ __forceinline__ pel *spl(uint8_t *p) { return reinterpret_cast<pel *>(p); }
 template <class pel> __device__ __forceinline__ const pel *spl(const uint8_t *p) { return reinterpret_cast<const pel *>(p); }
+#ifdef JMH_TYPED_GPTR
+template <class pel> __device__ __forceinline__ gptr<pel> spl(gptr<uint8_t> p) { return (gptr<pel>)p; }
+template <class pel> __device__ __forceinline__ gptr<const pel> spl(gptr<const uint8_t> p) { return (gptr<const pel>)p; }
+#endif
diff --git a/h264-jm-commentary_amd/csrc/jmh_final.h b/h264-jm-commentary_amd/csrc/jmh_final.h
--- a/h264-jm-commentary_amd/csrc/jmh_final.h
+++ b/h264-jm-commentary_amd/csrc/jmh_final.h
@@ -35,6 +35,7 @@
 
 template <class pel>
 struct ScratchAnalysis {
+    static constexpr bool in_lds = false;
     const MbScratch *sc;
     __device__ __forceinline__ int motion_cost(int m, int k) const { return sc->motion_cost[m][k]; }
     __device__ __forceinline__ int mv(int m, int k, int c) const { return sc->all_mv[m][k][c]; }
@@ -72,9 +73,9 @@
     const int W = d.W, Wc = d.Wc, W4 = d.W >> 2;
     const int slice_p = d.slice_type == JMH_P_SLICE;
     const int qpy = d.qp, qp = d.qp + d.qpbd, maxv = d.maxv;
-    const pel *orgY = spl<pel>(d.orgY), *orgU = spl<pel>(d.orgU), *orgV = spl<pel>(d.orgV);
-    const pel *refU = spl<pel>(d.refU), *refV = spl<pel>(d.refV);
-    pel *recY = spl<pel>(d.recY), *recU = spl<pel>(d.recU), *recV = spl<pel>(d.recV);
+    const gptr<const pel> orgY = spl<pel>(d.orgY), orgU = spl<pel>(d.orgU), orgV = spl<pel>(d.orgV);
+    const gptr<const pel> refU = spl<pel>(d.refU), refV = spl<pel>(d.refV);
+    const gptr<pel> recY = spl<pel>(d.recY), recU = spl<pel>(d.recU), recV = spl<pel>(d.recV);
     const MbAvail mav = intra_avail(d, mbx, mby);
     const bool avL = mav.L, avT = mav.T, avTL = mav.TL;
     const bool prof = prof_mb_here(d, mbx, mby);
@@ -86,7 +87,12 @@
     const pel(*S_ctop)[12] = pnb ? pnb->ctop : s.ctop;
     const pel(*S_cleft)[8] = pnb ? pnb->cleft : s.cleft;
     if (lu && !porg) s.org[tid] = orgY[(pix_y + (tid >> 4)) * W + pix_x + (tid & 15)];
-    if (d.dbkY) deblock_prefetch<pel, NTH>(d, s.db, mbx, mby, tid);
+    constexpr bool LATE = AV::in_lds;
+    DbkFetch<NTH> dbf = {};
+    if (d.dbkY) {
+        if constexpr (LATE) dbf = deblock_fetch<pel, NTH>(d, mbx, mby, tid);
+        else deblock_prefetch<pel, NTH>(d, s.db, mbx, mby, tid);
+    }
     if (!pnb && (!W2 || tid >= 256)) {
         const int u = ct;
         if (u < 128) {
@@ -146,7 +152,7 @@
         if (is_intra) {
             cpredv = chroma_pred_px(S_ctop[cuv] + 1, S_cleft[cuv], S_ctop[cuv][0], avT, avL, c_mode, cxo, cyo, maxv);
         } else {
-            const pel *R = cuv ? refV : refU;
+            const gptr<const pel> R = cuv ? refV : refU;
             const int vx = s.fmv[(cyo >> 1) * 4 + (cxo >> 1)][0], vy = s.fmv[(cyo >> 1) * 4 + (cxo >> 1)][1];
             const int ii = ((pix_x >> 1) + cxo) * 8 + vx, jj = ((pix_y >> 1) + cyo) * 8 + vy;
             const int x0 = iclip(0, Wc - 1, ii >> 3), y0 = iclip(0, d.Hc - 1, jj >> 3);
@@ -156,6 +162,8 @@
                       fx * fy * R[y1 * Wc + x1] + 32) >> 6;
         }
     }
+    if constexpr (LATE)
+        if (d.dbkY) deblock_stage<pel, NTH>(s.db, dbf, mbx, mby, tid);
     const int qpi = iclip(-d.qpbd, 51, qpy + d.cqp_off), qpcy = qpi < 0 ? qpi : c_qpc[qpi], qpc = qpcy + d.qpbd;
     const int cq_bits = 15 + qpc / 6;
     const int cqp_const = q_round(d.qsel, cq_bits);
@@ -331,7 +339,7 @@
     }
     cbp |= cr << 4;
 
-    jmh_mb_result *res = d.res + mby * d.mbw + mbx;
+    const gptr<jmh_mb_result> res = d.res + mby * d.mbw + mbx;
     int mb_type = best_mode;
     if (slice_p && best_mode == 1 && cbp == 0 && s.fmv[0][0] == an.skipx() && s.fmv[0][1] == an.skipy()) mb_type = JMH_PSKIP;
     if (tid == 0) {
diff --git a/h264-jm-commentary_amd/csrc/jmh_i4.h b/h264-jm-commentary_amd/csrc/jmh_i4.h
--- a/h264-jm-commentary_amd/csrc/jmh_i4.h
+++ b/h264-jm-commentary_amd/csrc/jmh_i4.h
@@ -37,7 +37,7 @@
 template <class pel>
 __device__ __forceinline__ void i4_block(const DevParams &d, IntraS<pel> &s, int16_t (*i4lev)[16], int w, int bx4, int by4, const int (&tabr)[2],
                                          bool avL, bool avT, bool avTL, bool avTR, int qpk, int (&acc)[3],
-                                         unsigned long long *pst = nullptr) {
+                                         gptr<unsigned long long> pst = nullptr) {
 #define I4ST(k, v) do { if (pst) { asm volatile("" ::"v"(v)); if (__lane_id() == 0) pst[k] = wall_clock64(); } } while (0)
     I4ST(52, bx4);
     const int lane = threadIdx.x & 63, l = lane & 15;
diff --git a/h264-jm-commentary_amd/csrc/jmh_intra.h b/h264-jm-commentary_amd/csrc/jmh_intra.h
--- a/h264-jm-commentary_amd/csrc/jmh_intra.h
+++ b/h264-jm-commentary_amd/csrc/jmh_intra.h
@@ -22,7 +22,7 @@
 };
 template <class pel>
 __device__ __forceinline__ void load_intra_nb(const DevParams &d, IntraNb<pel> &nb, int t, int mbx, int mby) {
-    const pel *recY = spl<pel>(d.recY), *recU = spl<pel>(d.recU), *recV = spl<pel>(d.recV);
+    const gptr<const pel> recY = spl<pel>(d.recY), recU = spl<pel>(d.recU), recV = spl<pel>(d.recV);
     const int pix_x = 16 * mbx, pix_y = 16 * mby, W = d.W, Wc = d.Wc;
     const MbAvail mav = intra_avail(d, mbx, mby);
     const bool avL = mav.L, avT = mav.T, avTL = mav.TL, avTR = mav.TR;
@@ -43,6 +43,34 @@
     }
 }
 template <class pel>
+__device__ __forceinline__ void load_intra_nb_batch(const DevParams &d, IntraNb<pel> &nb, int t, int mbx, int mby) {
+    const gptr<const pel> recY = spl<pel>(d.recY), recU = spl<pel>(d.recU), recV = spl<pel>(d.recV);
+    const int pix_x = 16 * mbx, pix_y = 16 * mby, W = d.W, Wc = d.Wc;
+    const MbAvail mav = intra_avail(d, mbx, mby);
+    const bool avL = mav.L, avT = mav.T, avTL = mav.TL, avTR = mav.TR;
+    gptr<const pel> src = recY;
+    pel *dst = nullptr;
+    bool av = false;
+    if (t < 21) {
+        const int x = t - 1;
+        av = x < 0 ? avTL : x < 16 ? avT : avTR;
+        src = recY + (pix_y - 1) * W + pix_x + x; dst = &nb.rtop[x + 1];
+    } else if (t < 37) {
+        const int y = t - 21;
+        av = avL;
+        src = recY + (pix_y + y) * W + pix_x - 1; dst = &nb.rleft[y];
+    } else if (t < 55) {
+        const int i = t - 37, uv = i / 9, x = i - 9 * uv - 1;
+        av = x < 0 ? avTL : avT;
+        src = (uv ? recV : recU) + ((pix_y >> 1) - 1) * Wc + (pix_x >> 1) + x; dst = &nb.ctop[uv][x + 1];
+    } else if (t < 71) {
+        const int i = t - 55, uv = i >> 3, y = i & 7;
+        av = avL;
+        src = (uv ? recV : recU) + ((pix_y >> 1) + y) * Wc + (pix_x >> 1) - 1; dst = &nb.cleft[uv][y];
+    }
+    if (dst) *dst = av ? *src : (pel)0;
+}
+template <class pel>
 __device__ __forceinline__ void load_orgc(const DevParams &d, IntraNb<pel> &nb, int t, int mbx, int mby) {
     const int uv = t >> 6, k = t & 63;
     nb.orgc[uv][k] = spl<pel>(uv ? d.orgV : d.orgU)[((8 * mby) + (k >> 3)) * d.Wc + 8 * mbx + (k & 7)];
```

Result: faster. 1502, median of 6 (+2.2%).
